# 0xWOLAND/halo2-prover

Hardware: AMD Instinct MI355X
Metric: MSM+NTT field-ops/s (higher is better)
Workload: dtype u32 limbs (256-bit modular)

## Files before the change

### halo2_prover_amd/csrc/h2_capi.hip

```cpp
#include "h2_internal.hpp"

#include <algorithm>
#include <cstdio>
#include <cstring>
#include <optional>

#include "h2_expr_program.hpp"
#include "h2_host.hpp"
#include "h2_ipa.hpp"
#include "h2_lookup.hpp"
#include "h2_ntt.hpp"
#include "h2_permutation.hpp"
#include "h2_poly.hpp"

using namespace h2;

namespace h2 {

Global g_h2;
std::recursive_mutex g_h2_mu;
TestKnobs g_knobs;
TestCounters g_counts;

int dev_fail(hipError_t e, const char* where) {
  char buf[256];
  snprintf(buf, sizeof buf, "%s: %s", where, hipGetErrorString(e));
  g_h2.last_error = buf;
  return H2_EDEVICE;
}

bool curve_ok(int c) { return c == H2_BN254 || c == H2_PALLAS || c == H2_VESTA; }

const CurveOps* ops_of(int curve) {
  switch (curve) {
    case H2_BN254: return curve_ops_bn254();
    case H2_PALLAS: return curve_ops_pallas();
    case H2_VESTA: return curve_ops_vesta();
  }
  return nullptr;
}

DevCtx* ctx_current() {
  if (!g_h2.ready || g_h2.ctx.empty()) return nullptr;
  if (g_h2.ctx.size() == 1) return &g_h2.ctx[0];
  int dev = -1;
  if (hipGetDevice(&dev) != hipSuccess) return nullptr;
  for (auto& c : g_h2.ctx)
    if (c.device == dev) return &c;
  return nullptr;
}
size_t ctx_index(const DevCtx* c) { return (size_t)(c - &g_h2.ctx[0]); }

int device_alloc(void** p, size_t bytes, const char* what) {
  hipError_t e = hipMalloc(p, bytes);
  if (e == hipSuccess) return H2_OK;
  (void)hipGetLastError();
  *p = nullptr;
  g_h2.last_error = std::string("hipMalloc(") + what + "): " + hipGetErrorString(e);
  return H2_ENOMEM;
}

ArenaLease::ArenaLease(Arena& arena, size_t want, hipStream_t stream) : a(arena), s(stream) { rc = acquire(want); }
int ArenaLease::acquire(size_t want) {
  clean_bytes = a.bytes < want ? 0 : a.clean_bytes;
  a.clean_bytes = 0;
  if (a.bytes < want) {
    g_counts.arena_growths++;
    if (a.p) {
      H2_TRY(hipDeviceSynchronize());
      (void)hipFree(a.p);
      a.p = nullptr;
      a.bytes = 0;
      a.used = false;
    }
    const size_t sz = want + (want >> 3);
    if (int st = device_alloc(&a.p, sz, "arena"); st != H2_OK) return st;
    a.bytes = sz;
  }
  if (!a.ev) H2_TRY(hipEventCreateWithFlags(&a.ev, hipEventDisableTiming));
  if (a.used && a.last != s) {
    g_counts.arena_waits++;
    H2_TRY(hipStreamWaitEvent(s, a.ev, 0));
  }
  return H2_OK;
}
int ArenaLease::release() {
  released = true;
  H2_TRY(hipEventRecord(a.ev, s));
  a.last = s;
  a.used = true;
  return H2_OK;
}
int ArenaLease::wait() {
  H2_TRY(hipStreamSynchronize(s));
  released = true;
  return H2_OK;
}
ArenaLease::~ArenaLease() noexcept {
  if (rc != H2_OK || released) return;
  if (hipEventRecord(a.ev, s) == hipSuccess) {
    a.last = s;
    a.used = true;
  } else {
    (void)hipGetLastError();
  }
}
static void arena_free(Arena& a) {
  if (a.p) (void)hipFree(a.p);
  if (a.ev) (void)hipEventDestroy(a.ev);
  a = Arena{};
}

static int register_device(DevCtx& src, int curve, const void* d_affine, size_t n, uint64_t* handle_out) {
  if (!curve_ok(curve) || !d_affine || !handle_out || n == 0) return H2_EINVAL;
  const CurveOps* ops = ops_of(curve);
  MsmGeom g = msm_geometry(n, ops->scalar_bits);
  if ((uint64_t)g.W * n >= (1ull << 31)) return H2_EINVAL;
  BasesEntry be{};
  be.curve = curve;
  be.n = n;
  be.geom = g;
  be.table_bytes = (size_t)g.W * n * 64;
  be.table.assign(g_h2.ctx.size(), nullptr);
  auto fail = [&](int rc) {
    for (size_t i = 0; i < be.table.size(); i++)
      if (be.table[i]) {
        DeviceGuard dg(g_h2.ctx[i].device);
        (void)hipFree(be.table[i]);
      }
    return rc;
  };
  for (size_t i = 0; i < g_h2.ctx.size(); i++) {
    DeviceGuard dg(g_h2.ctx[i].device);
    if (int rc = device_alloc(&be.table[i], be.table_bytes, "table"); rc != H2_OK) return fail(rc);
  }
  const size_t si = ctx_index(&src);
  {
    DeviceGuard dg(src.device);
    ArenaLease scan_ws(src.div_ws, sizeof(uint32_t), src.stream);
    if (scan_ws.rc != H2_OK) return fail(scan_ws.rc);
    uint32_t* d_bad = (uint32_t*)scan_ws.a.p;
    uint32_t bad = 0;
    ArenaLease table_ws(src.msm_ws.of(src.stream), be.table_bytes / 64 * MSM_TABLE_SCRATCH, src.stream);
    if (table_ws.rc != H2_OK) return fail(table_ws.rc);
    hipError_t e = hipMemsetAsync(d_bad, 0, 4, src.stream);
    if (e == hipSuccess) e = ops->table_build(d_affine, be.table[si], table_ws.a.p, (uint32_t)n, g, d_bad, src.stream);
    if (e == hipSuccess) e = hipMemcpyAsync(&bad, d_bad, 4, hipMemcpyDeviceToHost, src.stream);
    if (e == hipSuccess) e = hipStreamSynchronize(src.stream);
    if (e != hipSuccess) return fail(dev_fail(e, "msm_table_kernel"));
    (void)scan_ws.release();
    (void)table_ws.release();
    if (bad) {
      g_h2.last_error = "bases: " + std::to_string(bad) + " point(s) not on the curve";
      return fail(H2_EINVAL);
    }
    for (size_t i = 0; i < g_h2.ctx.size(); i++) {
      if (i == si) continue;
      e = hipMemcpyPeer(be.table[i], g_h2.ctx[i].device, be.table[si], src.device, be.table_bytes);
      if (e != hipSuccess) return fail(dev_fail(e, "hipMemcpyPeer(table)"));
    }
  }
  uint64_t h = g_h2.next_handle++;
  g_h2.bases[h] = be;
  *handle_out = h;
  return H2_OK;
}

int msm_common_checks(int curve, uint64_t handle, size_t first, size_t n, size_t m, const BasesEntry** be) {
  if (!g_h2.ready) return H2_ENOTINIT;
  if (!curve_ok(curve) || m == 0) return H2_EINVAL;
  auto it = g_h2.bases.find(handle);
  if (it == g_h2.bases.end()) return H2_EHANDLE;
  if (it->second.curve != curve) return H2_EINVAL;
  if (first > it->second.n || n > it->second.n - first) return H2_EINVAL;
  *be = &it->second;
  return H2_OK;
}

size_t msm_cols_per_launch(const MsmGeom& geom, size_t n) {
  const uint64_t per_col = (uint64_t)geom.W * n;
  const uint64_t by_entries = g_knobs.msm_max_entries / per_col;
  uint64_t by_keys = ((1ull << 31) - 1) / geom.B;
  if (geom.B > 4096) {
    const uint64_t by_bins = S2_MAX_H / msm_sort2_geom(n, geom).Hc;
    if (by_bins >= 1 && by_bins < by_keys) by_keys = by_bins;
  }
  return (size_t)(by_entries < by_keys ? by_entries : by_keys);
}

static int msm_guard_inspect(const MsmWorkspace& ws, char* ws_base, hipStream_t stream, size_t m, const char* what) {
  void* d_bad = nullptr;
  if (int rc = device_alloc(&d_bad, ws.n_regions * 4, "guard"); rc != H2_OK) return rc;
  DeviceBuffer owner(d_bad);
  std::vector<uint32_t> bad(ws.n_regions, 0);
  H2_TRY(hipMemsetAsync(d_bad, 0, ws.n_regions * 4, stream));
  if (g_knobs.msm_guard_poke)
    H2_TRY(hipMemsetAsync(ws_base + ws.regions[1].off + ws.regions[1].bytes, 0, 1, stream));
  hipLaunchKernelGGL(msm_guard_check_kernel, dim3(ws.n_regions), dim3(256), 0, stream, (const uint8_t*)ws_base, ws, (uint32_t*)d_bad);
  H2_TRY(hipMemcpyAsync(bad.data(), d_bad, ws.n_regions * 4, hipMemcpyDeviceToHost, stream));
  H2_TRY(hipStreamSynchronize(stream));
  g_counts.guard_launches++;
  for (uint32_t r = 0; r < ws.n_regions; r++)
    if (bad[r]) {
      if (!g_counts.guard_violations)
        g_counts.guard_first = std::string(ws.regions[r].name) + ": " + std::to_string(bad[r]) + " byte(s) behind the region, n=" +
                               std::to_string(ws.n) + " m=" + std::to_string(m) + what;
      g_counts.guard_violations++;
    }
  return H2_OK;
}

template <class Launch, class Finish>
static int msm_run_group(DevCtx& c, hipStream_t stream, const MsmGroupPlan& plan, const char* route, const char* label, size_t m,
                         const char* guard_what, Launch&& launch, Finish&& finish) {
  const MsmWorkspace& ws = plan.ws;
  ArenaLease lease(c.msm_ws.of(stream), ws.total, stream);
  if (lease.rc != H2_OK) return lease.rc;
  Arena& A = lease.a;
  if (const char* broken = plan.broken ? plan.broken : ws.total <= A.bytes ? nullptr : "ws.total <= arena_bytes") {
    g_h2.last_error = std::string(route) + " launch geometry: " + broken;
    return H2_EDEVICE;
  }
  const bool guard = g_knobs.msm_guard;
  if (guard) H2_TRY(hipMemsetAsync(A.p, MSM_GUARD_BYTE, ws.total, stream));
  const bool zeroed = !guard && lease.clean_bytes >= ws.zero_bytes && A.clean_off == ws.off_misc;
  if (int rc = launched(launch((char*)A.p, zeroed), label); rc != H2_OK) return rc;
  if (guard) {
    if (int rc = msm_guard_inspect(ws, (char*)A.p, stream, m, guard_what); rc != H2_OK) return rc;
  } else {
    A.clean_off = ws.off_misc;
    A.clean_bytes = ws.zero_bytes;
  }
  if (int rc = finish((char*)A.p); rc != H2_OK) return rc;
  return lease.release();
}

static std::pair<hipEvent_t, hipEvent_t> msm_prof_events(DevCtx& c, size_t n, size_t m) {
  if (!g_h2.profiling) return {nullptr, nullptr};
  if (c.prof_used == c.prof_events.size()) {
    hipEvent_t a, b;
    if (hipEventCreate(&a) == hipSuccess && hipEventCreate(&b) == hipSuccess) c.prof_events.push_back({a, b});
  }
  if (c.prof_used == c.prof_events.size()) return {nullptr, nullptr};
  c.prof_alg_bytes += (double)m * (double)n * 96.0 + (double)m * 96.0;
  return c.prof_events[c.prof_used++];
}

int msm_device_run(DevCtx& c, int curve, const BasesEntry& be, const void* d_scalars, size_t first_base, size_t n,
                   size_t col_stride, size_t m, void* d_out, bool affine_out, hipStream_t stream,
                   const BasesEntry* const* per_column) {
  if (msm_cols_per_launch(be.geom, n) == 0) return H2_EINVAL;
  const void* col_tables[MSM_MAX_MULTI];
  if (per_column) {
    if (m > MSM_MAX_MULTI) return H2_EINVAL;
    for (size_t j = 0; j < m; j++) {
      if (per_column[j]->n != be.n || per_column[j]->curve != be.curve) return H2_EINVAL;
      col_tables[j] = (const char*)per_column[j]->table[ctx_index(&c)] + first_base * 64;
    }
  }
  const size_t out_sz = affine_out ? 64 : 96;
  const CurveOps* ops = ops_of(curve);
  const char* table = (const char*)be.table[ctx_index(&c)] + first_base * 64;
  for (size_t j0 = 0; j0 < m;) {
    const MsmGroupPlan plan = msm_plan_group(be.geom, be.n, n, m - j0, col_stride, g_knobs.msm_guard, g_knobs.sort2_pack);
    const MsmWorkspace& ws = plan.ws;
    const size_t mm = plan.cols;
    if (per_column && mm < m) return H2_EINVAL;
    if (ws.E >= (1ull << 31) || ws.K >= (1ull << 31)) return H2_EINVAL;
    if (c.tail_wanted && !c.tail_event) H2_TRY(hipEventCreateWithFlags(&c.tail_event, hipEventDisableTiming));
    void* dst = (char*)d_out + j0 * out_sz;
    int rc = msm_run_group(
        c, stream, plan, "msm", "msm_launch", mm, ws.sort2 ? " two-level sort" : ws.staged ? " staged scatter" : " direct scatter",
        [&](char* ws_base, bool zeroed) {
          const auto [ev0, ev1] = msm_prof_events(c, n, mm);
          hipError_t e = ops->msm_launch(table, per_column ? col_tables : nullptr, (uint32_t)be.n,
                                         (const char*)d_scalars + j0 * col_stride * 32, n, col_stride, mm, be.geom, ws_base, ws, stream,
                                         ev0, ev1, (c.tail_wanted && !ev1) ? c.tail_event : nullptr, affine_out ? nullptr : dst, zeroed);
          c.tail_recorded = c.tail_wanted;
          c.tail_wait = ev1 ? ev1 : c.tail_event;
          return e;
        },
        [&](char* ws_base) {
          return affine_out ? launched(ops->to_affine(ws_base + ws.off_tree2, dst, (uint32_t)mm, stream), "msm finish kernel") : H2_OK;
        });
    if (rc != H2_OK) return rc;
    j0 += mm;
  }
  return H2_OK;
}

static int msm_points_run(DevCtx& c, int curve, const void* d_points, const void* d_scalars, size_t n, size_t col_stride,
                          size_t m, void* d_out, hipStream_t stream) {
  const CurveOps* ops = ops_of(curve);
  if (n < g_knobs.points_small_max) {
    const size_t blocks = (n + 15) / 16, work = MSM_SMALL_MAX * (blocks * (XYZZ29_WORDS * 4) + 4);
    for (size_t j0 = 0; j0 < m; j0 += MSM_SMALL_MAX) {
      const uint32_t count = (uint32_t)std::min<size_t>(MSM_SMALL_MAX, m - j0);
      ArenaLease lease(c.msm_ws.of(stream), work, stream);
      if (lease.rc != H2_OK) return lease.rc;
      const void* pts[MSM_SMALL_MAX];
      const void* sc[MSM_SMALL_MAX];
      uint32_t len[MSM_SMALL_MAX];
      for (uint32_t j = 0; j < count; j++) {
        pts[j] = d_points;
        sc[j] = (const char*)d_scalars + (j0 + j) * col_stride * 32;
        len[j] = (uint32_t)n;
      }
      if (int rc = launched(ops->msm_small(pts, sc, len, count, lease.a.p, (char*)d_out + j0 * 96, stream), "msm_small_kernel"); rc != H2_OK)
        return rc;
      if (int rc = lease.release(); rc != H2_OK) return rc;
    }
    return H2_OK;
  }
  const MsmGeom g = msm_points_geometry(n, ops->scalar_bits);
  for (size_t j0 = 0; j0 < m;) {
    const MsmGroupPlan plan = msm_points_plan_group(g, n, m - j0, col_stride, g_knobs.msm_guard);
    const size_t mm = plan.cols;
    if (mm == 0) return H2_EINVAL;
    int rc = msm_run_group(
        c, stream, plan, "msm points", "msm_points_launch", mm, " points front",
        [&](char* ws_base, bool zeroed) {
          return ops->msm_points_launch(d_points, (const char*)d_scalars + j0 * col_stride * 32, n, col_stride, mm, g, ws_base, plan.ws,
                                        stream, (char*)d_out + j0 * 96, zeroed);
        },
        [](char*) { return (int)H2_OK; });
    if (rc != H2_OK) return rc;
    j0 += mm;
  }
  return H2_OK;
}

static int get_twiddles(DevCtx& c, const CurveOps* ops, const uint64_t omega[4], uint32_t log_n, const uint64_t* scale,
                        const void** out) {
  for (auto& t : c.twiddles) {
    if (t.field == ops->scalar_field_id && t.log_n == log_n && memcmp(t.omega, omega, 32) == 0 && t.scaled == (scale != nullptr) &&
        (!scale || memcmp(t.scale, scale, 32) == 0)) {
      t.stamp = ++c.stamp;
      *out = t.tw;
      return H2_OK;
    }
  }
  if (c.twiddles.size() >= 16) {
    size_t victim = 0;
    for (size_t i = 1; i < c.twiddles.size(); i++)
      if (c.twiddles[i].stamp < c.twiddles[victim].stamp) victim = i;
    H2_TRY(hipDeviceSynchronize());
    (void)hipFree(c.twiddles[victim].tw);
    c.twiddles.erase(c.twiddles.begin() + victim);
  }
  TwiddleEntry te{};
  te.field = ops->scalar_field_id;
  te.log_n = log_n;
  memcpy(te.omega, omega, 32);
  te.scaled = scale != nullptr;
  if (scale) memcpy(te.scale, scale, 32);
  if (int rc = device_alloc(&te.tw, ops->ntt_table_bytes(log_n), "twiddles"); rc != H2_OK) return rc;
  DeviceBuffer owner(te.tw);
  hipError_t e = ops->ntt_twiddles(te.tw, omega, log_n, c.stream, scale);
  if (e == hipSuccess) e = hipStreamSynchronize(c.stream);
  if (e != hipSuccess) return dev_fail(e, "ntt_build_tables");
  (void)owner.release();
  te.stamp = ++c.stamp;
  c.twiddles.push_back(te);
  *out = te.tw;
  return H2_OK;
}

template <class Launch>
static int ntt_run(DevCtx& c, const CurveOps* ops, const uint64_t omega[4], uint32_t log_n, const uint64_t* table_scale, size_t m,
                   hipStream_t stream, const char* what, Launch&& launch) {
  const void* tw = nullptr;
  if (log_n > 0)
    if (int rc = get_twiddles(c, ops, omega, log_n, table_scale, &tw); rc != H2_OK) return rc;
  std::optional<ArenaLease> A;
  if (ntt_make_plan(log_n).npass > 1) {
    A.emplace(c.ntt_ws.of(stream), m * ((size_t)32 << log_n), stream);
    if (A->rc != H2_OK) return A->rc;
  }
  if (int rc = launched(launch(tw, A ? A->a.p : nullptr), what); rc != H2_OK) return rc;
  return A ? A->release() : H2_OK;
}

int ntt_enqueue(DevCtx& c, int curve, void* d_a, size_t m, const uint64_t omega[4], uint32_t log_n, hipStream_t stream,
                const uint64_t* scale) {
  const CurveOps* ops = ops_of(curve);
  if (!ops) return H2_EINVAL;
  return ntt_run(c, ops, omega, log_n, (scale && ops->ntt_scale_in_table(log_n)) ? scale : nullptr, m, stream, "ntt_launch",
                 [&](const void* tw, void* scratch) { return ops->ntt_launch(d_a, scratch, tw, log_n, m, stream, scale); });
}

int coeff_to_extended_enqueue(DevCtx& c, int curve, const void* d_coeff, size_t col_stride, uint32_t log_n, size_t m,
                              const uint64_t zeta[4], const uint64_t ext_omega[4], uint32_t ext_log_n, void* d_out,
                              hipStream_t stream) {
  const CurveOps* ops = ops_of(curve);
  if (!ops) return H2_EINVAL;
  return ntt_run(c, ops, ext_omega, ext_log_n, nullptr, m, stream, "ntt_extend_launch", [&](const void* tw, void* scratch) {
    return ops->ntt_extend_launch(d_coeff, col_stride, log_n, zeta, d_out, scratch, tw, ext_log_n, m, stream);
  });
}

int extended_to_coeff_enqueue(DevCtx& c, int curve, const void* d_ext, uint32_t ext_log_n, size_t m,
                              const uint64_t ext_omega_inv[4], const uint64_t scale[4], const uint64_t zeta_inv[4], const void* d_t,
                              size_t t_period, void* d_out, size_t out_len, size_t out_stride, hipStream_t stream) {
  const CurveOps* ops = ops_of(curve);
  if (!ops) return H2_EINVAL;
  if (m == 0 || out_len == 0) return H2_OK;
  return ntt_run(c, ops, ext_omega_inv, ext_log_n, ops->ntt_scale_in_table(ext_log_n) ? scale : nullptr, m, stream, "ntt_coeff_launch",
                 [&](const void* tw, void* scratch) {
                   return ops->ntt_coeff_launch(d_ext, d_t, t_period, scale, zeta_inv, d_out, out_len, out_stride, scratch, tw, ext_log_n,
                                                m, stream);
                 });
}

int poly_eval_enqueue(DevCtx& c, int curve, const void* const* d_polys, size_t n, const uint64_t* points, size_t q, void* d_out,
                      hipStream_t stream) {
  const CurveOps* ops = ops_of(curve);
  if (!ops || n == 0 || n > POLY_EVAL_MAX_N || q == 0) return H2_EINVAL;
  const size_t per_job = poly_eval_ws_bytes(1, n);
  const size_t group = std::min<size_t>({q, (size_t)65535, std::max<size_t>(1, POLY_EVAL_WS_CAP / per_job)});
  const size_t table_bytes = h2_align256(q * sizeof(PolyEvalJob));
  ArenaLease A(c.div_ws, table_bytes + poly_eval_ws_bytes(group, n), stream);
  if (A.rc != H2_OK) return A.rc;
  std::vector<PolyEvalJob> table(q);
  for (size_t t = 0; t < q; t++) {
    table[t].poly = d_polys[t];
    memcpy(table[t].point, points + 4 * t, 32);
  }
  H2_TRY(hipMemcpyAsync(A.a.p, table.data(), q * sizeof(PolyEvalJob), hipMemcpyHostToDevice, stream));
  const PolyEvalJob* d_jobs = (const PolyEvalJob*)A.a.p;
  void* ws = (char*)A.a.p + table_bytes;
  for (size_t t0 = 0; t0 < q; t0 += group) {
    const size_t cnt = std::min(group, q - t0);
    if (int rc = launched(ops->poly_eval(d_jobs + t0, (uint32_t)cnt, n, ws, (char*)d_out + 32 * t0, stream), "poly_eval kernels"); rc != H2_OK)
      return rc;
  }
  return A.release();
}

#define H2_BY_SCALAR_FIELD(curve, call)                          \
  ((curve) == H2_BN254    ? call<BN254_CURVE::Scalar>            \
   : (curve) == H2_PALLAS ? call<PALLAS_CURVE::Scalar>           \
                          : call<VESTA_CURVE::Scalar>)

template <class FP>
static void perm_fill_tables(const PermWorkspace& w, const void* const* d_values, const void* const* d_sigma, size_t n_cols, size_t m,
                             const uint64_t* beta, const uint64_t* gamma, const uint64_t omega[4], const uint64_t delta[4], char* out) {
  using H = HF<FP>;
  PermColumn* cols = (PermColumn*)(out + w.off_columns);
  PermChallenge* ch = (PermChallenge*)(out + w.off_challenges);
  const H d = H::from_mont_limbs(delta);
  for (size_t p = 0; p < m; p++) {
    H bd = H::from_mont_limbs(beta + 4 * p);
    memcpy(ch[p].beta, beta + 4 * p, 32);
    memcpy(ch[p].gamma, gamma + 4 * p, 32);
    for (size_t j = 0; j < n_cols; j++) {
      PermColumn& c = cols[p * n_cols + j];
      c.value = d_values[p * n_cols + j];
      c.sigma = d_sigma[j];
      uint64_t limbs[4];
      bd.mont_limbs(limbs);
      memcpy(c.beta_delta, limbs, 32);
      bd = bd * d;
    }
  }
  H pw = H::from_mont_limbs(omega);
  for (int r = 1; r < perm_run(); r <<= 1) pw = pw.sqr();
  for (int b = 0; b < PERM_POW_BITS; b++) {
    uint64_t limbs[4];
    pw.mont_limbs(limbs);
    memcpy(out + w.off_powers + 32 * (size_t)b, limbs, 32);
    pw = pw.sqr();
  }
}

int permutation_product_enqueue(DevCtx& c, int curve, const void* const* d_values, const void* const* d_sigma, size_t n_cols, size_t chunk_len,
                                size_t u, size_t m, const uint64_t* beta, const uint64_t* gamma, const uint64_t omega[4],
                                const uint64_t delta[4], void* d_z, size_t col_stride, hipStream_t stream) {
  const CurveOps* ops = ops_of(curve);
  if (!ops || n_cols == 0 || chunk_len == 0 || m == 0) return H2_EINVAL;
  const size_t S = (n_cols - 1) / chunk_len + 1;
  const size_t scan_group = std::min(m, PERM_SCAN_GROUP);
  const PermWorkspace ws = perm_workspace(u, n_cols, S, m, scan_group);
  if (const char* broken = perm_check(ws, u, n_cols, chunk_len, S, m, scan_group, col_stride, ws.total)) {
    g_h2.last_error = std::string("permutation launch geometry: ") + broken;
    return H2_EDEVICE;
  }
  ArenaLease A(c.div_ws, ws.total, stream);
  if (A.rc != H2_OK) return A.rc;
  if (const char* broken = perm_check(ws, u, n_cols, chunk_len, S, m, scan_group, col_stride, A.a.bytes)) {
    g_h2.last_error = std::string("permutation launch geometry: ") + broken;
    return H2_EDEVICE;
  }
  std::vector<char> tables(ws.off_scan);
  H2_BY_SCALAR_FIELD(curve, perm_fill_tables)(ws, d_values, d_sigma, n_cols, m, beta, gamma, omega, delta, tables.data());
  H2_TRY(hipMemcpyAsync(A.a.p, tables.data(), tables.size(), hipMemcpyHostToDevice, stream));
  for (size_t p0 = 0; p0 < m; p0 += PERM_RATIO_GROUP)
    if (int rc = launched(ops->perm_ratio(ws, (char*)A.a.p, p0, std::min(PERM_RATIO_GROUP, m - p0), u, n_cols, chunk_len, S, omega, d_z,
                                          col_stride, stream),
                          "perm_ratio_kernel");
        rc != H2_OK)
      return rc;
  for (size_t p0 = 0; u && p0 < m; p0 += scan_group)
    if (int rc = launched(ops->perm_scan(ws, (char*)A.a.p, p0, std::min(scan_group, m - p0), u, S, d_z, col_stride, stream),
                          "permutation scan kernels");
        rc != H2_OK)
      return rc;
  return A.release();
}

}

namespace {

struct Call {
  std::lock_guard<std::recursive_mutex> lk{g_h2_mu};
  DevCtx* c = nullptr;
  hipStream_t stream = nullptr;
  int rc = H2_OK;
  Call(void* stream_) {
    if (!g_h2.ready) { rc = H2_ENOTINIT; return; }
    c = ctx_current();
    if (!c) { rc = H2_EINVAL; g_h2.last_error = "no h2 context on the current HIP device"; return; }
    stream = stream_ ? (hipStream_t)stream_ : c->stream;
  }
};

int init_devices(int n, const int* ids) {
  if (g_h2.ready) {
    if ((size_t)n != g_h2.ctx.size()) return H2_EINVAL;
    for (int i = 0; i < n; i++)
      if (g_h2.ctx[i].device != ids[i]) return H2_EINVAL;
    return H2_OK;
  }
  int count = 0;
  hipError_t e = hipGetDeviceCount(&count);
  if (e != hipSuccess || count == 0) {
    (void)hipGetLastError();
    g_h2.last_error = "no HIP device available";
    return H2_EDEVICE;
  }
  for (int i = 0; i < n; i++)
    if (ids[i] < 0 || ids[i] >= count) return H2_EINVAL;
  int prev = 0;
  (void)hipGetDevice(&prev);
  g_h2.ctx.assign((size_t)n, DevCtx{});
  for (int i = 0; i < n; i++) {
    DevCtx& c = g_h2.ctx[i];
    c.device = ids[i];
    H2_TRY(hipSetDevice(ids[i]));
    H2_TRY(hipStreamCreateWithFlags(&c.stream, hipStreamDefault));
    for (int cv = 0; cv < 3; cv++) H2_TRY(ops_of(cv)->kernel_setup());
  }
  H2_TRY(hipSetDevice(n == 1 ? ids[0] : prev));
  g_h2.ready = true;
  return H2_OK;
}

template <class FP>
void jac_to_affine_host(const uint8_t* jac, size_t m, uint8_t* out) {
  using H = HF<FP>;
  std::vector<H> z(m), pre(m);
  H acc = H::one();
  for (size_t j = 0; j < m; j++) {
    z[j] = H::from_mont_limbs(jac + 96 * j + 64);
    pre[j] = acc;
    if (!z[j].is_zero()) acc *= z[j];
  }
  H inv = acc.inv();
  for (size_t j = m; j-- > 0;) {
    uint8_t* o = out + 64 * j;
    if (z[j].is_zero()) {
      memset(o, 0, 64);
      continue;
    }
    const H zi = inv * pre[j], zi2 = zi.sqr();
    inv *= z[j];
    const H x = H::from_mont_limbs(jac + 96 * j) * zi2, y = H::from_mont_limbs(jac + 96 * j + 32) * zi2 * zi;
    memcpy(o, x.v.v, 32);
    memcpy(o + 32, y.v.v, 32);
  }
}
void jac_to_affine_host(int curve, const uint8_t* jac, size_t m, uint8_t* out) {
  if (curve == H2_BN254) jac_to_affine_host<BN254_FQ>(jac, m, out);
  else if (curve == H2_PALLAS) jac_to_affine_host<PASTA_FP>(jac, m, out);
  else jac_to_affine_host<PASTA_FQ>(jac, m, out);
}

int msm_host(h2_curve_t curve, uint64_t handle, const uint64_t* const* cols, size_t n, size_t m, uint64_t* out,
                    bool affine_out) {
  const BasesEntry* be = nullptr;
  int rc = msm_common_checks((int)curve, handle, 0, n, m, &be);
  if (rc != H2_OK) return rc;
  if (!out || !cols) return H2_EINVAL;
  const size_t out_sz = affine_out ? 64 : 96;
  if (n == 0) {
    memset(out, 0, m * out_sz);
    return H2_OK;
  }
  for (size_t j = 0; j < m; j++)
    if (!cols[j]) return H2_EINVAL;
  const size_t G = g_h2.ctx.size();
  const size_t col_bytes = n * 32;
  if (m == 1 && G > 1 && n >= 4096 * G) {
    std::vector<uint64_t> partial(G * 12);
    std::vector<std::optional<ArenaLease>> stages(G);
    for (size_t g = 0; g < G; g++) {
      DevCtx& c = g_h2.ctx[g];
      DeviceGuard dg(c.device);
      const size_t lo = n * g / G, hi = n * (g + 1) / G, cnt = hi - lo;
      const size_t res_off = h2_align256(cnt * 32);
      if (int st = stages[g].emplace(c.stage, res_off + 96, c.stream).rc; st != H2_OK) return st;
      H2_TRY(hipMemcpyAsync(c.stage.p, (const char*)cols[0] + lo * 32, cnt * 32, hipMemcpyHostToDevice, c.stream));
      void* d_res = (char*)c.stage.p + res_off;
      rc = msm_device_run(c, (int)curve, *be, c.stage.p, lo, cnt, cnt, 1, d_res, false, c.stream);
      if (rc != H2_OK) return rc;
      H2_TRY(hipMemcpyAsync(&partial[12 * g], d_res, 96, hipMemcpyDeviceToHost, c.stream));
    }
    for (size_t g = 0; g < G; g++) {
      DeviceGuard dg(g_h2.ctx[g].device);
      if (int st = stages[g]->wait(); st != H2_OK) return st;
    }
    DevCtx& c = g_h2.ctx[0];
    DeviceGuard dg(c.device);
    const size_t res_off = h2_align256(G * 96);
    ArenaLease stage(c.stage, res_off + 96, c.stream);
    if (stage.rc != H2_OK) return stage.rc;
    H2_TRY(hipMemcpyAsync(c.stage.p, partial.data(), G * 96, hipMemcpyHostToDevice, c.stream));
    void* d_res = (char*)c.stage.p + res_off;
    if (int st = launched(ops_of((int)curve)->points_sum(c.stage.p, d_res, (uint32_t)G, 1, c.stream), "points_sum_kernel"); st != H2_OK)
      return st;
    if (affine_out) return H2_EINVAL;
    H2_TRY(hipMemcpyAsync(out, d_res, 96, hipMemcpyDeviceToHost, c.stream));
    return stage.wait();
  }
  std::vector<uint8_t> jac(affine_out ? m * 96 : 0);
  uint8_t* dst = affine_out ? jac.data() : (uint8_t*)out;
  std::vector<std::optional<ArenaLease>> stages(G);
  for (size_t g = 0; g < G && g < m; g++) {
    DevCtx& c = g_h2.ctx[g];
    DeviceGuard dg(c.device);
    const size_t mine = (m - g + G - 1) / G;
    const size_t res_off = h2_align256(mine * col_bytes);
    if (int st = stages[g].emplace(c.stage, res_off + mine * 96, c.stream).rc; st != H2_OK) return st;
    for (size_t i = 0; i < mine; i++)
      H2_TRY(hipMemcpyAsync((char*)c.stage.p + i * col_bytes, cols[g + i * G], col_bytes, hipMemcpyHostToDevice,
                            c.stream));
    void* d_res = (char*)c.stage.p + res_off;
    rc = msm_device_run(c, (int)curve, *be, c.stage.p, 0, n, n, mine, d_res, false, c.stream);
    if (rc != H2_OK) return rc;
    if (G == 1) {
      H2_TRY(hipMemcpyAsync(dst, d_res, mine * 96, hipMemcpyDeviceToHost, c.stream));
    } else {
      for (size_t i = 0; i < mine; i++)
        H2_TRY(hipMemcpyAsync(dst + (g + i * G) * 96, (char*)d_res + i * 96, 96, hipMemcpyDeviceToHost, c.stream));
    }
  }
  for (size_t g = 0; g < G && g < m; g++) {
    DeviceGuard dg(g_h2.ctx[g].device);
    if (int st = stages[g]->wait(); st != H2_OK) return st;
  }
  if (affine_out) jac_to_affine_host((int)curve, jac.data(), m, (uint8_t*)out);
  return H2_OK;
}

constexpr size_t EXPR_TABLE_CAP = (size_t)256 << 20;
constexpr size_t EXPR_MAX_COUNT = (size_t)1 << 20;
constexpr size_t EXPR_MAX_INSTANCES = (size_t)1 << 30;

template <class FP>
bool mont_canonical(const uint64_t* v) {
  for (int i = 3; i >= 0; i--) {
    const uint64_t pw = (uint64_t)FP::P(2 * i) | ((uint64_t)FP::P(2 * i + 1) << 32);
    if (v[i] != pw) return v[i] < pw;
  }
  return false;
}
template <class FP>
void expr_working_form(const uint64_t* api, uint64_t* out) {
  HF<FP> c = HF<FP>::from_mont_limbs(api);
// ... 387 lines not shown
  }
  return ntt_enqueue(*k.c, (int)curve, d_a, m, omega, log_n, k.stream, scale);
}

int h2_coeff_to_extended_device(h2_curve_t curve, const void* d_coeff, size_t col_stride, uint32_t log_n, size_t m,
                                const uint64_t zeta[4], const uint64_t ext_omega[4], uint32_t ext_log_n, void* d_out,
                                void* stream_) {
  Call k(stream_);
  if (k.rc != H2_OK) return k.rc;
  if (!curve_ok((int)curve) || !zeta || !ext_omega || ext_log_n > 30 || ext_log_n < log_n) return H2_EINVAL;
  const size_t n = (size_t)1 << log_n, en = (size_t)1 << ext_log_n;
  if (col_stride < n) return H2_EINVAL;
  if (m == 0) return H2_OK;
  if (!d_coeff || !d_out || m > 65535) return H2_EINVAL;
  const uintptr_t s0 = (uintptr_t)d_coeff, s1 = s0 + ((m - 1) * col_stride + n) * 32;
  const uintptr_t o0 = (uintptr_t)d_out, o1 = o0 + m * en * 32;
  if (s0 < o1 && o0 < s1) return H2_EINVAL;
  if (ext_log_n == 0) {
    H2_TRY(hipMemcpy2DAsync(d_out, 32, d_coeff, col_stride * 32, 32, m, hipMemcpyDeviceToDevice, k.stream));
    return H2_OK;
  }
  return coeff_to_extended_enqueue(*k.c, (int)curve, d_coeff, col_stride, log_n, m, zeta, ext_omega, ext_log_n, d_out, k.stream);
}

int h2_extended_to_coeff_device(h2_curve_t curve, const void* d_ext, uint32_t ext_log_n, size_t m, const uint64_t ext_omega_inv[4],
                                const uint64_t scale[4], const uint64_t zeta_inv[4], const void* d_t, size_t t_period, void* d_out,
                                size_t out_len, size_t out_stride, void* stream_) {
  Call k(stream_);
  if (k.rc != H2_OK) return k.rc;
  if (!curve_ok((int)curve) || ext_log_n > 30 || m > 65535) return H2_EINVAL;
  const size_t en = (size_t)1 << ext_log_n;
  if (out_len > en || out_stride < out_len || out_stride > ((size_t)1 << 40)) return H2_EINVAL;
  if (d_t && (t_period == 0 || (t_period & (t_period - 1)) || t_period > en)) return H2_EINVAL;
  if ((((uintptr_t)d_ext | (uintptr_t)d_out | (uintptr_t)d_t) & 15) != 0) return H2_EINVAL;
  if (m == 0 || out_len == 0) return H2_OK;
  if (!d_ext || !d_out || !ext_omega_inv || !scale || !zeta_inv) return H2_EINVAL;
  const uintptr_t s0 = (uintptr_t)d_ext, s1 = s0 + m * en * 32;
  const uintptr_t o0 = (uintptr_t)d_out, o1 = o0 + ((m - 1) * out_stride + out_len) * 32;
  if (s0 < o1 && o0 < s1) return H2_EINVAL;
  return extended_to_coeff_enqueue(*k.c, (int)curve, d_ext, ext_log_n, m, ext_omega_inv, scale, zeta_inv, d_t, t_period, d_out,
                                   out_len, out_stride, k.stream);
}

int h2_poly_scale_device(h2_curve_t curve, void* d_a, size_t n, size_t m, const uint64_t c[4], void* stream_) {
  Call k(stream_);
  if (k.rc != H2_OK) return k.rc;
  if (!curve_ok((int)curve) || !d_a || !c) return H2_EINVAL;
  if (n * m == 0) return H2_OK;
  return launched(ops_of((int)curve)->poly_scale(d_a, n * m, c, k.stream), "poly_scale_kernel");
}

int h2_poly_coset_device(h2_curve_t curve, void* d_a, size_t n, size_t m, const uint64_t g[4], void* stream_) {
  Call k(stream_);
  if (k.rc != H2_OK) return k.rc;
  if (!curve_ok((int)curve) || !d_a || !g) return H2_EINVAL;
  if (n * m == 0) return H2_OK;
  return launched(ops_of((int)curve)->poly_powers(d_a, n, m, g, k.stream), "poly_powers_kernel");
}

int h2_poly_mul_periodic_device(h2_curve_t curve, void* d_a, size_t n, size_t m, const void* d_t, size_t period,
                                void* stream_) {
  Call k(stream_);
  if (k.rc != H2_OK) return k.rc;
  if (!curve_ok((int)curve) || !d_a || !d_t || period == 0 || (period & (period - 1))) return H2_EINVAL;
  if (n * m == 0) return H2_OK;
  return launched(ops_of((int)curve)->poly_mul_periodic(d_a, n * m, d_t, period, k.stream), "poly_mul_periodic_kernel");
}

int h2_poly_inverse_device(h2_curve_t curve, void* d_a, size_t n, void* stream_) {
  Call k(stream_);
  if (k.rc != H2_OK) return k.rc;
  if (!curve_ok((int)curve) || !d_a) return H2_EINVAL;
  if (n == 0) return H2_OK;
  return launched(ops_of((int)curve)->poly_inverse(d_a, n, k.stream), "poly_inverse_kernel");
}

int h2_poly_divide_linear_device(h2_curve_t curve, const void* d_a, size_t n, const uint64_t z[4], void* d_q,
                                 void* stream_) {
  Call k(stream_);
  if (k.rc != H2_OK) return k.rc;
  if (!curve_ok((int)curve) || !d_a || !d_q || !z || d_a == d_q) return H2_EINVAL;
  if (n == 0) return H2_OK;
  ArenaLease A(k.c->div_ws, SCAN_WS_BYTES, k.stream);
  if (A.rc != H2_OK) return A.rc;
  if (int rc = launched(ops_of((int)curve)->poly_scan(0, &d_a, &d_q, z, 1, n, A.a.p, k.stream), "poly_scan kernels"); rc != H2_OK) return rc;
  return A.release();
}

int h2_poly_prefix_product_device(h2_curve_t curve, const void* d_a, size_t n, void* d_out, void* stream_) {
  Call k(stream_);
  if (k.rc != H2_OK) return k.rc;
  if (!curve_ok((int)curve) || !d_a || !d_out) return H2_EINVAL;
  if (n == 0) return H2_OK;
  ArenaLease A(k.c->div_ws, SCAN_WS_BYTES, k.stream);
  if (A.rc != H2_OK) return A.rc;
  if (int rc = launched(ops_of((int)curve)->poly_scan(1, &d_a, &d_out, nullptr, 1, n, A.a.p, k.stream), "poly_scan kernels"); rc != H2_OK) return rc;
  return A.release();
}

int h2_poly_eval_tile(void) { return POLY_EVAL_TILE; }

int h2_poly_eval_device(h2_curve_t curve, const void* const* d_polys, size_t n, const uint64_t* points, size_t q, void* d_out,
                        void* stream_) {
  Call k(stream_);
  if (k.rc != H2_OK) return k.rc;
  if (!curve_ok((int)curve) || n > POLY_EVAL_MAX_N) return H2_EINVAL;
  if (q == 0) return H2_OK;
  if (!d_polys || !points || !d_out) return H2_EINVAL;
  if (n == 0) {
    H2_TRY(hipMemsetAsync(d_out, 0, q * 32, k.stream));
    return H2_OK;
  }
  for (size_t t = 0; t < q; t++)
    if (!d_polys[t] || ((uintptr_t)d_polys[t] & 15)) return H2_EINVAL;
  return poly_eval_enqueue(*k.c, (int)curve, d_polys, n, points, q, d_out, k.stream);
}

int h2_poly_eval(h2_curve_t curve, const uint64_t* coeffs, size_t n, const uint64_t point[4], uint64_t out[4]) {
  Call k(nullptr);
  if (k.rc != H2_OK) return k.rc;
  if (!curve_ok((int)curve) || n > POLY_EVAL_MAX_N || !point || !out || (n > 0 && !coeffs)) return H2_EINVAL;
  if (n == 0) {
    memset(out, 0, 32);
    return H2_OK;
  }
  DevCtx& c = *k.c;
  const size_t off_res = h2_align256(n * 32);
  ArenaLease stage(c.stage, off_res + 32, c.stream);
  if (stage.rc != H2_OK) return stage.rc;
  char* base = (char*)c.stage.p;
  H2_TRY(hipMemcpyAsync(base, coeffs, n * 32, hipMemcpyHostToDevice, c.stream));
  const void* poly = base;
  if (int rc = poly_eval_enqueue(c, (int)curve, &poly, n, point, 1, base + off_res, c.stream); rc != H2_OK) return rc;
  H2_TRY(hipMemcpyAsync(out, base + off_res, 32, hipMemcpyDeviceToHost, c.stream));
  return stage.wait();
}

int h2_poly_lincomb_max_rounds(void) { return POLY_LINCOMB_MAX_ROUNDS; }

static_assert(sizeof(h2_lincomb_term_t) == sizeof(LincombTerm) && sizeof(h2_lincomb_job_t) == sizeof(LincombJob) &&
                  offsetof(h2_lincomb_term_t, coeff) == offsetof(LincombTerm, coeff) &&
                  offsetof(h2_lincomb_job_t, first_term) == offsetof(LincombJob, first_term),
              "the kernels read the C ABI's tables as they are");

static bool lincomb_overlaps(const h2_lincomb_job_t* jobs, size_t n_jobs, const h2_lincomb_term_t* terms, size_t n) {
  const uintptr_t len = (uintptr_t)n * 32;
  std::vector<std::pair<uintptr_t, size_t>> src, out;
  for (size_t j = 0; j < n_jobs; j++) {
    out.emplace_back((uintptr_t)jobs[j].d_out, j);
    for (uint32_t t = 0; t < jobs[j].n_terms; t++) src.emplace_back((uintptr_t)terms[jobs[j].first_term + t].d_poly, j);
  }
  std::sort(out.begin(), out.end());
  for (size_t a = 1; a < out.size(); a++)
    if (out[a].first - out[a - 1].first < len) return true;
  std::sort(src.begin(), src.end());
  src.erase(std::unique(src.begin(), src.end()), src.end());
  for (const auto& o : out) {
    auto it = std::lower_bound(src.begin(), src.end(), std::make_pair(o.first >= len ? o.first - len + 1 : (uintptr_t)0, (size_t)0));
    for (; it != src.end() && it->first < o.first + len; ++it) {
      if (it->second != o.second) return true;
      if (jobs[o.second].n_points > 0 || it->first != o.first) return true;
    }
  }
  return false;
}

int h2_poly_lincomb_device(h2_curve_t curve, const h2_lincomb_job_t* jobs, size_t n_jobs, const h2_lincomb_term_t* terms,
                           size_t n_terms, const uint64_t* low, size_t n_low, const uint64_t* points, size_t n_points, size_t n,
                           void* stream_) {
  Call k(stream_);
  if (k.rc != H2_OK) return k.rc;
  if (!curve_ok((int)curve) || n > POLY_LINCOMB_MAX_N) return H2_EINVAL;
  if (n_jobs == 0) return H2_OK;
  if (!jobs || n_jobs > ((size_t)1 << 31) || n_terms > ((size_t)1 << 31) || n_low > ((size_t)1 << 31)) return H2_EINVAL;
  size_t dividing = 0;
  for (size_t j = 0; j < n_jobs; j++) {
    const h2_lincomb_job_t& J = jobs[j];
    if ((uint64_t)J.first_term + J.n_terms > n_terms || (uint64_t)J.first_low + J.n_low > n_low ||
        (uint64_t)J.first_point + J.n_points > n_points)
      return H2_EINVAL;
    if (J.n_low > n || J.n_points > (uint32_t)POLY_LINCOMB_MAX_ROUNDS) return H2_EINVAL;
    if ((J.n_terms && !terms) || (J.n_low && !low) || (J.n_points && !points)) return H2_EINVAL;
    if (!J.d_out || ((uintptr_t)J.d_out & 15)) return H2_EINVAL;
    for (uint32_t t = 0; t < J.n_terms; t++) {
      const void* p = terms[J.first_term + t].d_poly;
      if (!p || ((uintptr_t)p & 15)) return H2_EINVAL;
    }
    dividing += J.n_points > 0;
  }
  if (n == 0) return H2_OK;
  if (lincomb_overlaps(jobs, n_jobs, terms, n)) return H2_EINVAL;

  const size_t col_bytes = h2_align256(n * 32);
  const size_t cols_cap = std::min(std::max<size_t>(1, POLY_LINCOMB_WS_CAP / col_bytes), std::max<size_t>(1, dividing));
  const size_t off_terms = h2_align256(n_jobs * sizeof(LincombJob));
  const size_t off_low = off_terms + h2_align256(n_terms * sizeof(LincombTerm));
  const size_t off_cols = off_low + h2_align256(n_low * 32);
  const size_t off_scan = off_cols + (dividing ? cols_cap * col_bytes : 0);
  ArenaLease A(k.c->div_ws, off_scan + (dividing ? SCAN_MAX_JOBS * SCAN_WS_BYTES : 0), k.stream);
  if (A.rc != H2_OK) return A.rc;
  char* base = (char*)A.a.p;

  std::vector<char> host(off_cols, 0);
  LincombJob* hj = (LincombJob*)host.data();
  std::vector<void*> scratch_of(n_jobs, nullptr);
  std::vector<size_t> group_end;
  for (size_t j = 0, g0 = 0, used = 0; j < n_jobs; j++) {
    const bool div = jobs[j].n_points > 0;
    if (j - g0 == 65535 || (div && used == cols_cap)) {
      group_end.push_back(j);
      g0 = j;
      used = 0;
    }
    memcpy(&hj[j], &jobs[j], sizeof(LincombJob));
    if (div) {
      scratch_of[j] = base + off_cols + used++ * col_bytes;
      if (jobs[j].n_points & 1) hj[j].out = scratch_of[j];
    }
  }
  group_end.push_back(n_jobs);
  if (n_terms) memcpy(host.data() + off_terms, terms, n_terms * sizeof(LincombTerm));
  if (n_low) memcpy(host.data() + off_low, low, n_low * 32);
  H2_TRY(hipMemcpyAsync(base, host.data(), off_cols, hipMemcpyHostToDevice, k.stream));

  const CurveOps* ops = ops_of((int)curve);
  for (size_t g = 0, j0 = 0; g < group_end.size(); j0 = group_end[g++]) {
    const size_t j1 = group_end[g];
    if (int rc = launched(ops->poly_lincomb((const LincombJob*)base + j0, (uint32_t)(j1 - j0), (const LincombTerm*)(base + off_terms),
                                            base + off_low, n, k.stream),
                          "poly_lincomb_kernel");
        rc != H2_OK)
      return rc;
    for (uint32_t r = 0; r < (uint32_t)POLY_LINCOMB_MAX_ROUNDS; r++) {
      const void* src[SCAN_MAX_JOBS];
      void* dst[SCAN_MAX_JOBS];
      uint64_t z[4 * SCAN_MAX_JOBS];
      uint32_t cnt = 0;
      bool any = false;
      auto flush = [&]() -> int {
        if (cnt == 0) return H2_OK;
        const int rc = launched(ops->poly_scan(0, src, dst, z, cnt, n, base + off_scan, k.stream), "poly_scan kernels");
        cnt = 0;
        return rc;
      };
      for (size_t j = j0; j < j1; j++) {
        const uint32_t P = jobs[j].n_points;
        if (P <= r) continue;
        any = true;
        src[cnt] = ((P - r) & 1) ? scratch_of[j] : jobs[j].d_out;
        dst[cnt] = ((P - r - 1) & 1) ? scratch_of[j] : jobs[j].d_out;
        memcpy(z + 4 * cnt, points + 4 * ((size_t)jobs[j].first_point + r), 32);
        if (++cnt == SCAN_MAX_JOBS)
          if (int rc = flush(); rc != H2_OK) return rc;
      }
      if (int rc = flush(); rc != H2_OK) return rc;
      if (!any) break;
    }
  }
  return A.release();
}

int h2_lookup_tile(void) { return (int)LOOKUP_TILE; }

static std::pair<uintptr_t, uintptr_t> lookup_range(const void* p, size_t rows, size_t stride, size_t m, size_t elem = 32) {
  const uintptr_t lo = (uintptr_t)p;
  if (rows == 0) return {lo, lo};
  return {lo, lo + ((m - 1) * stride + rows) * elem};
}
static bool lookup_overlap(const std::pair<uintptr_t, uintptr_t>& a, const std::pair<uintptr_t, uintptr_t>& b) {
  return a.first < b.second && b.first < a.second && a.first != a.second && b.first != b.second;
}

int h2_lookup_permute_device(h2_curve_t curve, const void* d_input, const void* d_table, size_t usable_rows, size_t col_stride,
                             size_t m, void* d_permuted_input, void* d_permuted_table, void* d_status, void* stream_) {
  Call k(stream_);
  if (k.rc != H2_OK) return k.rc;
  const size_t u = usable_rows;
  if (!curve_ok((int)curve) || u > LOOKUP_MAX_ROWS || col_stride < u || (col_stride && m > LOOKUP_MAX_CELLS / col_stride)) return H2_EINVAL;
  if ((((uintptr_t)d_input | (uintptr_t)d_table | (uintptr_t)d_permuted_input | (uintptr_t)d_permuted_table) & 15) || ((uintptr_t)d_status & 3))
    return H2_EINVAL;
  if (m == 0) return H2_OK;
  if (!d_status || (u > 0 && (!d_input || !d_table || !d_permuted_input || !d_permuted_table))) return H2_EINVAL;
  const auto in = lookup_range(d_input, u, col_stride, m), tab = lookup_range(d_table, u, col_stride, m);
  const auto pin = lookup_range(d_permuted_input, u, col_stride, m), ptab = lookup_range(d_permuted_table, u, col_stride, m);
  const auto st = lookup_range(d_status, 1, 1, m, 4);
  for (const auto* out : {&pin, &ptab, &st})
    if (lookup_overlap(*out, in) || lookup_overlap(*out, tab)) return H2_EINVAL;
  if (lookup_overlap(pin, ptab) || lookup_overlap(pin, st) || lookup_overlap(ptab, st)) return H2_EINVAL;
  const size_t group = u ? lookup_group(u, m) : m;
  for (size_t j0 = 0; u && j0 < m; j0 += group) {
    const size_t mm = std::min(group, m - j0);
    const LookupWorkspace ws = lookup_workspace(u, mm);
    if (const char* broken = lookup_check(ws, u, mm, col_stride, ws.total)) {
      g_h2.last_error = std::string("lookup launch geometry: ") + broken;
      return H2_EDEVICE;
    }
  }
  H2_TRY(hipMemsetAsync(d_status, 0, 4 * m, k.stream));
  if (u == 0) return H2_OK;
  const CurveOps* ops = ops_of((int)curve);
  for (size_t j0 = 0; j0 < m; j0 += group) {
    const size_t mm = std::min(group, m - j0);
    const LookupWorkspace ws = lookup_workspace(u, mm);
    ArenaLease A(k.c->msm_ws.of(k.stream), ws.total, k.stream);
    if (A.rc != H2_OK) return A.rc;
    if (const char* broken = lookup_check(ws, u, mm, col_stride, A.a.bytes)) {
      g_h2.last_error = std::string("lookup launch geometry: ") + broken;
      return H2_EDEVICE;
    }
    const size_t skip = j0 * col_stride * 32;
    if (int rc = launched(ops->lookup_permute((const char*)d_input + skip, (const char*)d_table + skip, col_stride, ws, (char*)A.a.p,
                                              (char*)d_permuted_input + skip, (char*)d_permuted_table + skip, (uint32_t*)d_status + j0,
                                              k.stream),
                          "lookup permute kernels");
        rc != H2_OK)
      return rc;
    if (int rc = A.release(); rc != H2_OK) return rc;
  }
  return H2_OK;
}

int h2_lookup_product_device(h2_curve_t curve, const void* d_input, const void* d_table, const void* d_permuted_input,
                             const void* d_permuted_table, size_t usable_rows, size_t col_stride, size_t m, const uint64_t beta[4],
                             const uint64_t gamma[4], void* d_z, void* stream_) {
  Call k(stream_);
  if (k.rc != H2_OK) return k.rc;
  const size_t u = usable_rows;
  if (!curve_ok((int)curve) || u > LOOKUP_MAX_ROWS || col_stride < u + 1 || m > LOOKUP_MAX_CELLS / col_stride) return H2_EINVAL;
  if (((uintptr_t)d_input | (uintptr_t)d_table | (uintptr_t)d_permuted_input | (uintptr_t)d_permuted_table | (uintptr_t)d_z) & 15) return H2_EINVAL;
  if (m == 0) return H2_OK;
  if (!d_z || !beta || !gamma || (u > 0 && (!d_input || !d_table || !d_permuted_input || !d_permuted_table))) return H2_EINVAL;
  const auto z = lookup_range(d_z, u + 1, col_stride, m);
  for (const void* src : {d_input, d_table, d_permuted_input, d_permuted_table})
    if (lookup_overlap(z, lookup_range(src, u, col_stride, m))) return H2_EINVAL;
  const CurveOps* ops = ops_of((int)curve);
  for (size_t j0 = 0; j0 < m; j0 += 65535) {
    const size_t skip = j0 * col_stride * 32;
    if (int rc = launched(ops->lookup_ratio((const char*)d_input + skip, (const char*)d_table + skip, (const char*)d_permuted_input + skip,
                                            (const char*)d_permuted_table + skip, u, col_stride, std::min<size_t>(65535, m - j0), beta,
                                            gamma, (char*)d_z + skip, k.stream),
                          "lookup_ratio_kernel");
        rc != H2_OK)
      return rc;
  }
  ArenaLease A(k.c->div_ws, SCAN_MAX_JOBS * SCAN_WS_BYTES, k.stream);
  if (A.rc != H2_OK) return A.rc;
  for (size_t j0 = 0; j0 < m; j0 += SCAN_MAX_JOBS) {
    const uint32_t cnt = (uint32_t)std::min<size_t>(SCAN_MAX_JOBS, m - j0);
    const void* src[SCAN_MAX_JOBS];
    void* dst[SCAN_MAX_JOBS];
    for (uint32_t j = 0; j < cnt; j++) src[j] = dst[j] = (char*)d_z + (j0 + j) * col_stride * 32;
    if (int rc = launched(ops->poly_scan(1, src, dst, nullptr, cnt, u + 1, A.a.p, k.stream), "poly_scan kernels"); rc != H2_OK) return rc;
  }
  return A.release();
}

int h2_permutation_tile(void) { return (int)perm_tile(); }

int h2_permutation_product_device(h2_curve_t curve, const void* const* d_values, const void* const* d_sigma, size_t n_cols, size_t chunk_len,
                                  size_t usable_rows, size_t m, const uint64_t* beta, const uint64_t* gamma, const uint64_t omega[4],
                                  const uint64_t delta[4], void* d_z, size_t col_stride, void* stream_) {
  Call k(stream_);
  if (k.rc != H2_OK) return k.rc;
  const size_t u = usable_rows;
  if (!curve_ok((int)curve) || (chunk_len == 0 && n_cols > 0) || u > PERM_MAX_ROWS || col_stride < u + 1) return H2_EINVAL;
  const size_t S = n_cols ? (n_cols - 1) / chunk_len + 1 : 0;
  if (S && m && (m > PERM_MAX_CELLS / S || m * S > PERM_MAX_CELLS / col_stride)) return H2_EINVAL;
  if (m == 0 || n_cols == 0) return H2_OK;
  if (!d_values || !d_sigma || !beta || !gamma || !omega || !delta || !d_z || ((uintptr_t)d_z & 15)) return H2_EINVAL;
  if (n_cols > ((size_t)1 << 31) || m > ((size_t)1 << 32) / n_cols) {
    g_h2.last_error = "permutation launch geometry: m n_cols <= 2^32";
    return H2_EDEVICE;
  }
  if (u > 0) {
    const auto z = lookup_range(d_z, u + 1, col_stride, m * S);
    for (size_t t = 0; t < m * n_cols + n_cols; t++) {
      const void* src = t < m * n_cols ? d_values[t] : d_sigma[t - m * n_cols];
      if (!src || ((uintptr_t)src & 15) || lookup_overlap(z, lookup_range(src, u, u, 1))) return H2_EINVAL;
    }
  }
  return permutation_product_enqueue(*k.c, (int)curve, d_values, d_sigma, n_cols, chunk_len, u, m, beta, gamma, omega, delta, d_z, col_stride,
                                     k.stream);
}

int h2_expr_compile(h2_curve_t curve, const h2_expr_node_t* nodes, size_t n_nodes, const uint64_t* consts, size_t n_consts,
                    uint32_t n_cols, uint32_t n_vars, uint64_t* handle_out) {
  std::lock_guard<std::recursive_mutex> lk(g_h2_mu);
  auto refuse = [](const char* rule) {
    g_h2.last_error = std::string("expr: ") + rule;
    return (int)H2_EINVAL;
  };
  if (!curve_ok((int)curve)) return refuse("unknown curve");
  if (!handle_out || !nodes || (n_consts && !consts)) return refuse("null pointer");
  if (n_nodes == 0 || n_nodes > EXPR_MAX_COUNT) return refuse("n_nodes must be 1 .. 2^20");
  if (n_consts > EXPR_MAX_COUNT || n_vars > EXPR_MAX_COUNT) return refuse("n_consts and n_vars may be at most 2^20");
  if (n_cols > (1u << 22)) return refuse("n_cols may be at most 2^22");
  ExprEntry e{};
  e.curve = (int)curve;
  try {
    H2_BY_SCALAR_FIELD((int)curve, expr_compile_t)(nodes, n_nodes, consts, n_consts, n_cols, n_vars, e);
  } catch (const product::Fail& f) {
    g_h2.last_error = f.what;
    return f.status;
  } catch (const std::exception& x) {
    g_h2.last_error = x.what();
    return H2_ENOMEM;
  }
  e.info.curve = (uint32_t)curve;
  const uint64_t h = g_h2.next_handle++;
  g_h2.exprs[h] = std::move(e);
  *handle_out = h;
  return H2_OK;
}

int h2_expr_release(uint64_t handle) {
  std::lock_guard<std::recursive_mutex> lk(g_h2_mu);
  auto it = g_h2.exprs.find(handle);
  if (it == g_h2.exprs.end()) return H2_EHANDLE;
  for (size_t i = 0; i < it->second.d_code.size() && i < g_h2.ctx.size(); i++) {
    if (!it->second.d_code[i]) continue;
    DeviceGuard dg(g_h2.ctx[i].device);
    (void)hipDeviceSynchronize();
    (void)hipFree(it->second.d_code[i]);
  }
  g_h2.exprs.erase(it);
  return H2_OK;
}

int h2_expr_info(uint64_t handle, h2_expr_info_t* out) {
  std::lock_guard<std::recursive_mutex> lk(g_h2_mu);
  if (!out) return H2_EINVAL;
  auto it = g_h2.exprs.find(handle);
  if (it == g_h2.exprs.end()) return H2_EHANDLE;
  *out = it->second.info;
  return H2_OK;
}

int h2_expr_dump(uint64_t handle, uint8_t* out, size_t cap, size_t* out_len) {
  std::lock_guard<std::recursive_mutex> lk(g_h2_mu);
  auto it = g_h2.exprs.find(handle);
  if (it == g_h2.exprs.end()) return H2_EHANDLE;
  const std::vector<uint8_t>& d = it->second.dump;
  if (out_len) *out_len = d.size();
  if (!out || cap < d.size()) return H2_EINVAL;
  memcpy(out, d.data(), d.size());
  return H2_OK;
}

int h2_expr_eval_device(uint64_t handle, const void* const* d_cols, const uint32_t* log_len, const uint64_t* vars, size_t m,
                        uint32_t log_rows, uint32_t rot_step, void* d_out, size_t out_stride, void* stream_) {
  Call k(stream_);
  if (k.rc != H2_OK) return k.rc;
  auto it = g_h2.exprs.find(handle);
  if (it == g_h2.exprs.end()) return H2_EHANDLE;
  ExprEntry& e = it->second;
  const size_t n_cols = e.info.n_cols, n_vars = e.info.n_vars, nconsts = e.table.size() / 4;
  if (log_rows > 28 || m > EXPR_MAX_INSTANCES) return H2_EINVAL;
  const size_t rows = (size_t)1 << log_rows;
  if (out_stride < rows || (m && out_stride > ((size_t)1 << 57) / m)) return H2_EINVAL;
  if (m == 0) return H2_OK;
  if (!d_out || ((uintptr_t)d_out & 15) || (n_cols && (!d_cols || !log_len)) || (n_vars && !vars)) return H2_EINVAL;
  for (size_t c = 0; c < n_cols; c++)
    if (log_len[c] > log_rows) return H2_EINVAL;
  const uintptr_t o0 = (uintptr_t)d_out, window = out_stride * 32, written = rows * 32, o1 = o0 + (m - 1) * window + written;
  for (size_t p = 0; p < m; p++)
    for (size_t c = 0; c < n_cols; c++) {
      const uintptr_t s0 = (uintptr_t)d_cols[p * n_cols + c], s1 = s0 + ((uintptr_t)32 << log_len[c]);
      if (!s0 || (s0 & 15)) return H2_EINVAL;
      if (s0 < o1 && o0 < s1) {
        const uintptr_t q = s0 > o0 ? (s0 - o0) / window : 0, w0 = o0 + q * window;
        if (s0 < w0 + written || (q + 1 < m && s1 > w0 + window)) return H2_EINVAL;
      }
    }
  for (size_t t = 0; t < m * n_vars; t++)
    if (!H2_BY_SCALAR_FIELD(e.curve, mont_canonical)(vars + 4 * t)) return H2_EINVAL;
  DevCtx& c = *k.c;
  const size_t ci = ctx_index(&c);
  const size_t group = std::min<size_t>({m, (size_t)65535, std::max<size_t>(1, EXPR_TABLE_CAP / (nconsts * 32))});
  std::vector<uint32_t> masks;
  std::vector<uint64_t> tables;
  try {
    masks.resize(n_cols);
    tables.resize(group * nconsts * 4);
    if (e.d_code.size() != g_h2.ctx.size()) e.d_code.assign(g_h2.ctx.size(), nullptr);
  } catch (const std::bad_alloc&) {
    g_h2.last_error = "expr: no host memory for the instances' constant tables";
    return H2_ENOMEM;
  }
  if (!e.d_code[ci]) {
    void* p = nullptr;
    if (int rc = device_alloc(&p, e.code.size() * 4, "expr code"); rc != H2_OK) return rc;
    DeviceBuffer owner(p);
    H2_TRY(hipMemcpyAsync(p, e.code.data(), e.code.size() * 4, hipMemcpyHostToDevice, c.stream));
    H2_TRY(hipStreamSynchronize(c.stream));
    e.d_code[ci] = owner.release();
  }
  const size_t mask_bytes = h2_align256(n_cols * 4 + 4), ptr_bytes = h2_align256(group * n_cols * sizeof(void*) + 8);
  ArenaLease A(c.div_ws, mask_bytes + ptr_bytes + group * nconsts * 32, k.stream);
  if (A.rc != H2_OK) return A.rc;
  uint32_t* d_masks = (uint32_t*)A.a.p;
  const void** d_ptrs = (const void**)((char*)A.a.p + mask_bytes);
  void* d_tables = (char*)A.a.p + mask_bytes + ptr_bytes;
  for (size_t j = 0; j < n_cols; j++) masks[j] = (1u << log_len[j]) - 1;
  if (n_cols) H2_TRY(hipMemcpyAsync(d_masks, masks.data(), n_cols * 4, hipMemcpyHostToDevice, k.stream));
  const CurveOps* ops = ops_of(e.curve);
  for (size_t p0 = 0; p0 < m; p0 += group) {
    const size_t cnt = std::min(group, m - p0);
    H2_BY_SCALAR_FIELD(e.curve, expr_fill_tables)(e, vars, p0, cnt, tables.data());
    if (n_cols) H2_TRY(hipMemcpyAsync(d_ptrs, d_cols + p0 * n_cols, cnt * n_cols * sizeof(void*), hipMemcpyHostToDevice, k.stream));
    H2_TRY(hipMemcpyAsync(d_tables, tables.data(), cnt * nconsts * 32, hipMemcpyHostToDevice, k.stream));
    if (int rc = launched(ops->expr_launch(e.d_code[ci], e.info.instructions, d_ptrs, (uint32_t)n_cols, d_masks, d_tables, (uint32_t)nconsts,
                                           (char*)d_out + p0 * out_stride * 32, out_stride, rot_step, (uint32_t)rows, (uint32_t)cnt,
                                           e.info.lds_bytes, k.stream),
                          "expr_kernel");
        rc != H2_OK)
      return rc;
  }
  return A.release();
}

int h2_chacha20_scalars_device(h2_curve_t curve, const uint8_t seed[32], uint64_t first_block, size_t n, void* d_out,
                               void* stream_) {
  Call k(stream_);
  if (k.rc != H2_OK) return k.rc;
  if (!curve_ok((int)curve) || !seed || !d_out) return H2_EINVAL;
  if (n == 0) return H2_OK;
  uint32_t key[8];
  for (int i = 0; i < 8; i++)
    key[i] = (uint32_t)seed[4 * i] | ((uint32_t)seed[4 * i + 1] << 8) | ((uint32_t)seed[4 * i + 2] << 16) |
             ((uint32_t)seed[4 * i + 3] << 24);
  return launched(ops_of((int)curve)->chacha20_scalars(d_out, n, first_block, key, k.stream), "chacha20_scalars_kernel");
}

static_assert(H2_IPA_MAX_K == IPA_MAX_K, "the header states the kernels' maximum");
static bool ipa_dev_ptr(const void* p) { return p && !((uintptr_t)p & 15); }

int h2_ipa_state_bytes(uint32_t k, size_t* out) {
  if (k == 0 || k > IPA_MAX_K || !out) return H2_EINVAL;
  *out = IpaLayout(k).total * 32;
  return H2_OK;
}

int h2_ipa_begin_device(h2_curve_t curve, uint32_t k_, const void* d_p, const uint64_t x3[4], void* d_state, void* stream_) {
  Call k(stream_);
  if (k.rc != H2_OK) return k.rc;
  if (!curve_ok((int)curve) || k_ == 0 || k_ > IPA_MAX_K || !ipa_dev_ptr(d_p) || !ipa_dev_ptr(d_state) || !x3) return H2_EINVAL;
  return launched(ops_of((int)curve)->ipa_begin(d_p, x3, k_, d_state, k.stream), "ipa_begin_kernel");
}

int h2_ipa_round_device(h2_curve_t curve, uint64_t bases, uint32_t k_, uint32_t j, void* d_state, const uint64_t* u_prev,
                        const uint64_t* u_prev_inv, const uint64_t z[4], const uint64_t l_blind[4], const uint64_t r_blind[4],
                        void* d_out_affine, void* stream_) {
  Call k(stream_);
  if (k.rc != H2_OK) return k.rc;
  if (!curve_ok((int)curve) || k_ == 0 || k_ > IPA_MAX_K || j >= k_) return H2_EINVAL;
  if (!ipa_dev_ptr(d_state) || !ipa_dev_ptr(d_out_affine) || !z || !l_blind || !r_blind) return H2_EINVAL;
  if (j == 0 ? (u_prev || u_prev_inv) : (!u_prev || !u_prev_inv)) return H2_EINVAL;
  const IpaLayout L(k_);
  const BasesEntry* be = nullptr;
  if (int rc = msm_common_checks((int)curve, bases, 0, L.col_stride, 2, &be); rc != H2_OK) return rc;
  if (be->n != L.col_stride) return H2_EINVAL;
  if (int rc = launched(ops_of((int)curve)->ipa_round(k_, j, d_state, u_prev, u_prev_inv, z, l_blind, r_blind, k.stream),
                        "ipa_round_kernel");
      rc != H2_OK)
    return rc;
  return msm_device_run(*k.c, (int)curve, *be, (const char*)d_state + L.col * 32, 0, L.col_stride, L.col_stride, 2, d_out_affine,
                        true, k.stream);
}

int h2_ipa_final_device(h2_curve_t curve, uint32_t k_, void* d_state, const uint64_t u_last[4], const uint64_t u_last_inv[4],
                        void* d_out, void* d_s_out, void* stream_) {
  Call k(stream_);
  if (k.rc != H2_OK) return k.rc;
  if (!curve_ok((int)curve) || k_ == 0 || k_ > IPA_MAX_K || !ipa_dev_ptr(d_state) || !ipa_dev_ptr(d_out) || !u_last || !u_last_inv)
    return H2_EINVAL;
  if (d_s_out && ((uintptr_t)d_s_out & 15)) return H2_EINVAL;
  return launched(ops_of((int)curve)->ipa_final(k_, d_state, u_last, u_last_inv, d_out, d_s_out, k.stream), "ipa_final_kernel");
}

int h2_ipa_challenge_products_device(h2_curve_t curve, const uint64_t* u, uint32_t k_, const uint64_t init[4], void* d_out,
                                     void* stream_) {
  Call k(stream_);
  if (k.rc != H2_OK) return k.rc;
  if (!curve_ok((int)curve) || k_ == 0 || k_ > IPA_MAX_K || !u || !init || !ipa_dev_ptr(d_out)) return H2_EINVAL;
  return launched(ops_of((int)curve)->ipa_s_products(u, k_, init, d_out, k.stream), "ipa_s_kernel");
}

int h2_poly_pointwise_device(h2_curve_t curve, int op, void* d_a, const void* d_b, size_t n, void* stream_) {
  Call k(stream_);
  if (k.rc != H2_OK) return k.rc;
  if (!curve_ok((int)curve) || !d_a || !d_b || op < 0 || op > 2) return H2_EINVAL;
  if (n == 0) return H2_OK;
  return launched(ops_of((int)curve)->poly_pointwise(d_a, d_b, n, op, k.stream), "poly_pointwise_kernel");
}

int h2_ntt_batch(h2_curve_t curve, uint64_t* const* cols, size_t m, const uint64_t omega[4], uint32_t log_n) {
  std::lock_guard<std::recursive_mutex> lk(g_h2_mu);
  if (!g_h2.ready) return H2_ENOTINIT;
  if (!curve_ok((int)curve) || !cols || !omega || m == 0 || log_n > 30) return H2_EINVAL;
  for (size_t j = 0; j < m; j++)
    if (!cols[j]) return H2_EINVAL;
  if (log_n == 0) return H2_OK;
  const size_t col_bytes = (size_t)32 << log_n;
  const size_t G = g_h2.ctx.size();
  std::vector<std::optional<ArenaLease>> stages(G);
  for (size_t g = 0; g < G && g < m; g++) {
    DevCtx& c = g_h2.ctx[g];
    DeviceGuard dg(c.device);
    const size_t mine = (m - g + G - 1) / G;
    if (int st = stages[g].emplace(c.stage, mine * col_bytes, c.stream).rc; st != H2_OK) return st;
    for (size_t i = 0; i < mine; i++)
      H2_TRY(hipMemcpyAsync((char*)c.stage.p + i * col_bytes, cols[g + i * G], col_bytes, hipMemcpyHostToDevice,
                            c.stream));
    int rc = ntt_enqueue(c, (int)curve, c.stage.p, mine, omega, log_n, c.stream);
    if (rc != H2_OK) return rc;
    for (size_t i = 0; i < mine; i++)
      H2_TRY(hipMemcpyAsync(cols[g + i * G], (char*)c.stage.p + i * col_bytes, col_bytes, hipMemcpyDeviceToHost,
                            c.stream));
  }
  for (size_t g = 0; g < G && g < m; g++) {
    DeviceGuard dg(g_h2.ctx[g].device);
    if (int st = stages[g]->wait(); st != H2_OK) return st;
  }
  return H2_OK;
}

int h2_fft_group_device(h2_curve_t curve, void* d_points_jac, const uint64_t omega[4], uint32_t log_n, void* stream_) {
  Call k(stream_);
  if (k.rc != H2_OK) return k.rc;
  if (!curve_ok((int)curve) || !d_points_jac || !omega || log_n > 26) return H2_EINVAL;
  if (log_n == 0) return H2_OK;
  const CurveOps* ops = ops_of((int)curve);
  ArenaLease A(k.c->msm_ws.of(k.stream), ops->group_fft_scratch(log_n), k.stream);
  if (A.rc != H2_OK) return A.rc;
  if (int rc = launched(ops->group_fft(d_points_jac, d_points_jac, A.a.p, omega, log_n, g_knobs.gfft_lanes, k.stream), "group fft kernels"); rc != H2_OK) return rc;
  return A.release();
}

int h2_fft_group(h2_curve_t curve, uint64_t* points_jac, const uint64_t omega[4], uint32_t log_n) {
  std::lock_guard<std::recursive_mutex> lk(g_h2_mu);
  if (!g_h2.ready) return H2_ENOTINIT;
  if (!curve_ok((int)curve) || !points_jac || !omega || log_n > 26) return H2_EINVAL;
  if (log_n == 0) return H2_OK;
  DevCtx& c = g_h2.ctx[0];
  DeviceGuard dg(c.device);
  const size_t bytes = ((size_t)96) << log_n;
  ArenaLease stage(c.stage, bytes, c.stream);
  if (stage.rc != H2_OK) return stage.rc;
  H2_TRY(hipMemcpyAsync(c.stage.p, points_jac, bytes, hipMemcpyHostToDevice, c.stream));
  int rc = h2_fft_group_device(curve, c.stage.p, omega, log_n, c.stream);
  if (rc != H2_OK) return rc;
  H2_TRY(hipMemcpyAsync(points_jac, c.stage.p, bytes, hipMemcpyDeviceToHost, c.stream));
  return stage.wait();
}

int h2_g_to_lagrange_device(h2_curve_t curve, const void* d_g_affine, uint32_t log_n, const uint64_t omega_inv[4],
                            const uint64_t scale[4], void* d_out_affine, void* stream_) {
  Call k(stream_);
  if (k.rc != H2_OK) return k.rc;
  if (!curve_ok((int)curve) || !d_g_affine || !d_out_affine || !omega_inv || !scale || log_n > 26) return H2_EINVAL;
  const uintptr_t in = (uintptr_t)d_g_affine, out = (uintptr_t)d_out_affine, bytes = (uintptr_t)64 << log_n;
  if ((in & 15) || (out & 15)) return H2_EINVAL;
  if (in != out && in < out + bytes && out < in + bytes) return H2_EINVAL;
  const CurveOps* ops = ops_of((int)curve);
  ArenaLease A(k.c->msm_ws.of(k.stream), ops->group_fft_scratch(log_n), k.stream);
  if (A.rc != H2_OK) return A.rc;
  if (int rc = launched(ops->g_to_lagrange(d_g_affine, d_out_affine, A.a.p, omega_inv, scale, log_n, g_knobs.gfft_lanes, k.stream),
                        "g_to_lagrange kernels");
      rc != H2_OK)
    return rc;
  return A.release();
}

int h2_g_to_lagrange(h2_curve_t curve, const uint64_t* g_affine, uint32_t log_n, const uint64_t omega_inv[4],
                     const uint64_t scale[4], uint64_t* out_affine) {
  std::lock_guard<std::recursive_mutex> lk(g_h2_mu);
  if (!g_h2.ready) return H2_ENOTINIT;
  if (!curve_ok((int)curve) || !g_affine || !out_affine || !omega_inv || !scale || log_n > 26) return H2_EINVAL;
  DevCtx& c = g_h2.ctx[0];
  DeviceGuard dg(c.device);
  const size_t bytes = ((size_t)64) << log_n;
  ArenaLease stage(c.stage, bytes, c.stream);
  if (stage.rc != H2_OK) return stage.rc;
  H2_TRY(hipMemcpyAsync(c.stage.p, g_affine, bytes, hipMemcpyHostToDevice, c.stream));
  int rc = h2_g_to_lagrange_device(curve, c.stage.p, log_n, omega_inv, scale, c.stage.p, c.stream);
  if (rc != H2_OK) return rc;
  H2_TRY(hipMemcpyAsync(out_affine, c.stage.p, bytes, hipMemcpyDeviceToHost, c.stream));
  return stage.wait();
}

int h2_ntt(h2_curve_t curve, uint64_t* a, const uint64_t omega[4], uint32_t log_n) {
  uint64_t* cols[1] = {a};
  return h2_ntt_batch(curve, cols, 1, omega, log_n);
}

}
```

### halo2_prover_amd/csrc/h2_curve_impl.hip

```cpp
#include "h2_curve_ops.hpp"
#include "h2_msm.hpp"
#include "h2_decompress.hpp"
#include "h2_ntt.hpp"
#include "h2_ntt29.hpp"
#include "h2_tune.hpp"
#include "h2_poly.hpp"
#include "h2_group_fft.hpp"
#include "h2_lookup.hpp"
#include "h2_permutation.hpp"
#include "h2_expr_kernel.hpp"
#include "h2_ipa.hpp"

#include <cstring>

#ifndef H2_CURVE_ID
#error "compile with -DH2_CURVE_ID=0 (bn254), 1 (pallas) or 2 (vesta)"
#endif

namespace h2 {
namespace {

#if H2_CURVE_ID == 0
using CV = BN254_CURVE;
#elif H2_CURVE_ID == 1
using CV = PALLAS_CURVE;
#else
using CV = VESTA_CURVE;
#endif
using FS = typename CV::Scalar;
using FB = typename CV::Base;

hipError_t kernel_setup() {
  hipError_t e = msm_kernel_setup<CV>();
  if (e != hipSuccess) return e;
  if ((e = msm_points_kernel_setup<CV>()) != hipSuccess) return e;
  return ntt29_kernel_setup<FS>();
}
hipError_t table_build(const void* d_bases, void* d_table, void* d_scratch, uint32_t n, const MsmGeom& g, uint32_t* d_bad, hipStream_t s) {
  hipLaunchKernelGGL(msm_table_kernel<CV>, dim3((n + 255) / 256), dim3(256), 0, s, (const U128*)d_bases,
                     (U128*)d_table, (uint32_t*)d_scratch, n, g, d_bad);
  return hipGetLastError();
}
hipError_t msm_launch_(const void* d_table, const void* const* per_column, uint32_t n_bases, const void* d_scalars, size_t n, size_t col_stride, size_t m,
                       const MsmGeom& g, char* ws_base, const MsmWorkspace& ws, hipStream_t s, hipEvent_t ev_start,
                       hipEvent_t ev_stop, hipEvent_t ev_tail, void* d_out_jac, bool zeroed) {
  return msm_launch<CV>((const U128*)d_table, (const U128* const*)per_column, n_bases, (const U128*)d_scalars, n, col_stride, m, g, ws_base, ws, s, ev_start,
                        ev_stop, ev_tail, (U128*)d_out_jac, zeroed);
}
hipError_t msm_points_launch_(const void* d_points, const void* d_scalars, size_t n, size_t col_stride, size_t m, const MsmGeom& g,
                              char* ws_base, const MsmWorkspace& ws, hipStream_t s, void* d_out_jac, bool zeroed) {
  return msm_points_launch<CV>((const U128*)d_points, (const U128*)d_scalars, n, col_stride, m, g, ws_base, ws, s, (U128*)d_out_jac, zeroed);
}
hipError_t srs_powers(void* d_out_affine, const uint64_t s_mont[4], uint32_t n, hipStream_t s) {
  Fe<FS> sv;
  memcpy(sv.v, s_mont, 32);
  hipLaunchKernelGGL(srs_powers_kernel<CV>, dim3((n + 255) / 256), dim3(256), 0, s, (U128*)d_out_affine, sv, n);
  return hipGetLastError();
}
hipError_t fixed_base_mul(void* d_out_affine, const void* d_scalars, uint32_t n, hipStream_t s) {
  hipLaunchKernelGGL(fixed_base_mul_kernel<CV>, dim3((n + 255) / 256), dim3(256), 0, s, (U128*)d_out_affine,
                     (const U128*)d_scalars, n);
  return hipGetLastError();
}
hipError_t to_affine(const void* d_xyzz, void* d_out, uint32_t m, hipStream_t s) {
  hipLaunchKernelGGL(msm_to_affine_kernel<CV>, dim3((m + 63) / 64), dim3(64), 0, s, (const uint32_t*)d_xyzz,
                     (U128*)d_out, m);
  return hipGetLastError();
}
hipError_t msm_small(const void* const* d_points, const void* const* d_scalars, const uint32_t* m, uint32_t count, void* d_work,
                     void* d_out_jac, hipStream_t s) {
  if (count == 0 || count > MSM_SMALL_MAX) return hipErrorInvalidValue;
  MsmSmallBatch J{};
  uint32_t mmax = 0;
  for (uint32_t j = 0; j < count; j++) {
    J.points[j] = (const U128*)d_points[j];
    J.scalars[j] = (const U128*)d_scalars[j];
    J.m[j] = m[j];
    mmax = std::max(mmax, m[j]);
  }
  const uint32_t blocks = (mmax + 15) / 16;
  if (blocks == 0) return hipErrorInvalidValue;
  uint32_t* part = (uint32_t*)d_work;
  uint32_t* counter = part + (size_t)count * blocks * XYZZ29_WORDS;
  hipError_t e = hipMemsetAsync(counter, 0, 4 * count, s);
  if (e != hipSuccess) return e;
  hipLaunchKernelGGL(msm_small_kernel<CV>, dim3(blocks, count), dim3(64), 0, s, J, part, counter, (U128*)d_out_jac);
  return hipGetLastError();
}
hipError_t points_sum(const void* d_in_jac, void* d_out_jac, uint32_t groups, uint32_t count, hipStream_t s) {
  hipLaunchKernelGGL(points_sum_kernel<CV>, dim3(count), dim3(64), 0, s, (const U128*)d_in_jac,
                     (U128*)d_out_jac, groups, count);
  return hipGetLastError();
}
#if H2_CURVE_ID == 0
hipError_t points_decompress(const void* d_compressed, void* d_out_affine, void* d_status, uint32_t n, hipStream_t s) {
  hipLaunchKernelGGL(points_decompress_kernel<CV>, dim3((n + 63) / 64), dim3(64), 0, s, (const uint32_t*)d_compressed,
                     (U128*)d_out_affine, (uint8_t*)d_status, n);
  return hipGetLastError();
}
int selftest_decompress(const uint8_t in[32], uint64_t out_affine[8]) {
  uint32_t w[8];
  for (int i = 0; i < 8; i++)
    w[i] = (uint32_t)in[4 * i] | ((uint32_t)in[4 * i + 1] << 8) | ((uint32_t)in[4 * i + 2] << 16) | ((uint32_t)in[4 * i + 3] << 24);
  Fe<FB> x, y;
  const uint8_t st = g1_decompress<CV>(w, x, y);
  memcpy(out_affine, x.v, 32);
  memcpy(out_affine + 4, y.v, 32);
  return st;
}
#else
constexpr auto points_decompress = nullptr;
constexpr auto selftest_decompress = nullptr;
#endif
size_t ntt_table_bytes(uint32_t log_n) { return ntt29_tables(log_n).total; }
bool ntt_scale_in_table(uint32_t log_n) { return ntt29_scale_in_table(log_n); }
hipError_t ntt_twiddles(void* d_tw, const uint64_t omega[4], uint32_t log_n, hipStream_t s, const uint64_t* scale) {
  Fe<FS> w, sc;
  memcpy(w.v, omega, 32);
  if (scale) memcpy(sc.v, scale, 32);
  return ntt29_build_tables<FS>(d_tw, w, log_n, s, scale ? &sc : nullptr);
}
hipError_t ntt_launch_(void* d_data, void* d_scratch, const void* d_tw, uint32_t log_n, size_t m, hipStream_t s,
                       const uint64_t* scale) {
  Fe<FS> sc;
  if (scale) memcpy(sc.v, scale, 32);
  return ntt29_launch<FS>((U128*)d_data, (U128*)d_scratch, d_tw, log_n, m, s, scale ? &sc : nullptr);
}
hipError_t ntt_extend_launch_(const void* d_src, size_t src_stride, uint32_t log_src, const uint64_t zeta[4], void* d_out,
                              void* d_scratch, const void* d_tw, uint32_t log_n, size_t m, hipStream_t s) {
  Fe<FS> z;
  memcpy(z.v, zeta, 32);
  return ntt29_extend_launch<FS>((const U128*)d_src, src_stride, log_src, z, (U128*)d_out, (U128*)d_scratch, d_tw, log_n, m, s);
}
hipError_t ntt_coeff_launch_(const void* d_src, const void* d_t, size_t t_period, const uint64_t scale[4], const uint64_t zeta_inv[4],
                             void* d_out, size_t out_len, size_t out_stride, void* d_scratch, const void* d_tw, uint32_t log_n,
                             size_t m, hipStream_t s) {
  Fe<FS> sc, zi;
  memcpy(sc.v, scale, 32);
  memcpy(zi.v, zeta_inv, 32);
  return ntt29_coeff_launch<FS>((const U128*)d_src, (const U128*)d_t, t_period, sc, zi, (U128*)d_out, out_len, out_stride,
                                (U128*)d_scratch, d_tw, log_n, m, s);
}
size_t group_fft_scratch(uint32_t log_n) { return gfft_scratch_bytes(log_n); }
hipError_t group_fft(const void* d_in_jac, void* d_out_jac, void* d_scratch, const uint64_t omega[4], uint32_t log_n, int lanes,
                     hipStream_t s) {
  Fe<FS> w;
  memcpy(w.v, omega, 32);
  return gfft_launch<CV>((const U128*)d_in_jac, (U128*)d_out_jac, d_scratch, w, log_n, s, lanes);
}
hipError_t g_to_lagrange(const void* d_in_affine, void* d_out_affine, void* d_scratch, const uint64_t omega[4],
                         const uint64_t scale[4], uint32_t log_n, int lanes, hipStream_t s) {
  Fe<FS> w, c;
  memcpy(w.v, omega, 32);
  memcpy(c.v, scale, 32);
  return gfft_to_lagrange_launch<CV>((const U128*)d_in_affine, (U128*)d_out_affine, d_scratch, w, c, log_n, s, lanes);
}
void selftest_glv_split(const uint64_t k_canonical[4], uint32_t out[10]) {
  Fe<FS> k;
  memcpy(k.v, k_canonical, 32);
  const GlvScalar r = glv_split<FS>(k);
  memcpy(out, r.k1, 4 * GLV_WORDS);
  memcpy(out + GLV_WORDS, r.k2, 4 * GLV_WORDS);
}
void selftest_glv_constants(uint64_t lambda[4], uint64_t beta[4]) {
  uint32_t l[8], b[8];
  for (int i = 0; i < 8; i++) {
    l[i] = Glv<FS>::LAMBDA(i);
    b[i] = Glv<FS>::BETA(i);
  }
  memcpy(lambda, l, 32);
  memcpy(beta, b, 32);
}
hipError_t poly_scale(void* d_a, size_t total, const uint64_t c[4], hipStream_t s) {
  Fe<FS> cv;
  memcpy(cv.v, c, 32);
  hipLaunchKernelGGL(poly_scale_kernel<FS>, dim3(poly_grid(total)), dim3(256), 0, s, (U128*)d_a, total, cv);
  return hipGetLastError();
}
hipError_t poly_powers(void* d_a, size_t n, size_t m, const uint64_t g[4], hipStream_t s) {
  Fe<FS> gv;
  memcpy(gv.v, g, 32);
  const size_t threads = (n + POLY_RUN - 1) / POLY_RUN;
  hipLaunchKernelGGL(poly_powers_kernel<FS>, dim3((unsigned)((threads + 255) / 256), (unsigned)m), dim3(256), 0, s,
                     (U128*)d_a, n, gv);
  return hipGetLastError();
}
hipError_t poly_mul_periodic(void* d_a, size_t total, const void* d_t, size_t period, hipStream_t s) {
  hipLaunchKernelGGL(poly_mul_periodic_kernel<FS>, dim3(poly_grid(total)), dim3(256), 0, s, (U128*)d_a, total,
                     (const U128*)d_t, period - 1);
  return hipGetLastError();
}
hipError_t poly_inverse(void* d_a, size_t total, hipStream_t s) {
  hipLaunchKernelGGL(poly_inverse_kernel<FS>, dim3(poly_grid(total)), dim3(256), 0, s, (U128*)d_a, total);
  return hipGetLastError();
}
hipError_t poly_scan(int mode, const void* const* d_a, void* const* d_out, const uint64_t* z, uint32_t jobs, size_t n,
                     void* d_ws, hipStream_t s) {
  if (jobs == 0 || jobs > SCAN_MAX_JOBS || n == 0) return hipErrorInvalidValue;
  uint32_t L = (uint32_t)((n + SCAN_CHUNKS - 1) / SCAN_CHUNKS);
  if (L < 16) L = 16;
  const uint32_t C = (uint32_t)((n + L - 1) / L);
  ScanBatch<FS> B{};
  for (uint32_t j = 0; j < jobs; j++) {
    B.a[j] = (const U128*)d_a[j];
    B.out[j] = (U128*)d_out[j];
    if (mode == 0) {
      memcpy(B.z[j].v, z + 4 * j, 32);
      B.w[j] = fe_pow_u64(B.z[j], (uint64_t)L);
    }
  }
  U128* H = (U128*)d_ws;
  U128* G = H + 2 * (size_t)jobs * SCAN_CHUNKS;
  hipLaunchKernelGGL(poly_scan_chunk_kernel<FS>, dim3((C + 63) / 64, jobs), dim3(64), 0, s, B, mode, n, L, C, H);
  hipLaunchKernelGGL(poly_scan_block_kernel<FS>, dim3(jobs), dim3(SCAN_BLOCK_THREADS), 0, s, B, mode, C, H, G);
  hipLaunchKernelGGL(poly_scan_apply_kernel<FS>, dim3((C + 63) / 64, jobs), dim3(64), 0, s, B, mode, n, L, C, G);
  return hipGetLastError();
}
hipError_t poly_eval(const PolyEvalJob* d_jobs, uint32_t jobs, size_t n, void* d_ws, void* d_out, hipStream_t s) {
  if (jobs == 0 || jobs > 65535 || n == 0 || n > POLY_EVAL_MAX_N) return hipErrorInvalidValue;
  const uint32_t tiles = (uint32_t)poly_eval_tiles(n);
  U128* partial = (U128*)d_ws;
  int32_t* powers = (int32_t*)((char*)d_ws + (size_t)jobs * tiles * 32);
  hipLaunchKernelGGL(poly_eval_powers_kernel<FS>, dim3((jobs + 63) / 64), dim3(64), 0, s, d_jobs, jobs, powers);
  hipLaunchKernelGGL(poly_eval_tile_kernel<FS>, dim3(tiles, jobs), dim3(POLY_EVAL_THREADS), 0, s, d_jobs, n,
                     (const int32_t*)powers, partial, tiles);
  hipLaunchKernelGGL(poly_eval_fold_kernel<FS>, dim3((jobs + 63) / 64), dim3(64), 0, s, jobs, (const int32_t*)powers,
                     (const U128*)partial, tiles, (U128*)d_out);
  return hipGetLastError();
}
hipError_t poly_lincomb(const LincombJob* d_jobs, uint32_t jobs, const LincombTerm* d_terms, const void* d_low, size_t n,
                        hipStream_t s) {
  if (jobs == 0 || jobs > 65535 || n == 0 || n > POLY_LINCOMB_MAX_N) return hipErrorInvalidValue;
  hipLaunchKernelGGL(poly_lincomb_kernel<FS>, dim3((unsigned)((n + POLY_LINCOMB_THREADS - 1) / POLY_LINCOMB_THREADS), jobs),
                     dim3(POLY_LINCOMB_THREADS), 0, s, d_jobs, d_terms, (const U128*)d_low, n);
  return hipGetLastError();
}
hipError_t lookup_permute(const void* d_input, const void* d_table, size_t col_stride, const LookupWorkspace& ws, char* ws_base,
                          void* d_permuted_input, void* d_permuted_table, uint32_t* d_status, hipStream_t s) {
  return lookup_permute_launch<FS>(d_input, d_table, col_stride, ws, ws_base, d_permuted_input, d_permuted_table, d_status, s);
}
hipError_t lookup_ratio(const void* d_input, const void* d_table, const void* d_permuted_input, const void* d_permuted_table, size_t u,
                        size_t col_stride, size_t m, const uint64_t beta[4], const uint64_t gamma[4], void* d_z, hipStream_t s) {
  return lookup_ratio_launch<FS>(d_input, d_table, d_permuted_input, d_permuted_table, u, col_stride, m, beta, gamma, d_z, s);
}
hipError_t perm_ratio(const PermWorkspace& w, char* base, size_t p0, size_t count, size_t u, size_t n_cols, size_t chunk_len, size_t S,
                      const uint64_t omega[4], void* d_z, size_t col_stride, hipStream_t s) {
  return perm_ratio_launch<FS>(w, base, p0, count, u, n_cols, chunk_len, S, omega, d_z, col_stride, s);
}
hipError_t perm_scan(const PermWorkspace& w, char* base, size_t p0, size_t count, size_t u, size_t S, void* d_z, size_t col_stride,
                     hipStream_t s) {
  return perm_scan_launch<FS>(w, base, p0, count, u, S, d_z, col_stride, s);
}
hipError_t expr_launch(const void* d_code, uint32_t ninstr, const void* const* d_cols, uint32_t ncols, const uint32_t* d_masks,
                       const void* d_consts, uint32_t nconsts, void* d_out, size_t out_stride, uint32_t step, uint32_t rows, uint32_t count,
                       size_t lds_bytes, hipStream_t s) {
  return pk::expr_kernel_launch<FS>((const pk::XInstr*)d_code, ninstr, (const U128* const*)d_cols, ncols, d_masks, (const U128*)d_consts,
                                    nconsts, (U128*)d_out, out_stride, step, rows, count, lds_bytes, s);
}
hipError_t chacha20_scalars(void* d_out, size_t n, uint64_t first_block, const uint32_t key[8], hipStream_t s) {
  ChaChaKey k;
  memcpy(k.w, key, 32);
  hipLaunchKernelGGL(chacha20_scalars_kernel<FS>, dim3((unsigned)((n + 255) / 256)), dim3(256), 0, s, (U128*)d_out, n,
                     first_block, k);
  return hipGetLastError();
}
hipError_t poly_pointwise(void* d_a, const void* d_b, size_t total, int op, hipStream_t s) {
  hipLaunchKernelGGL(poly_pointwise_kernel<FS>, dim3(poly_grid(total)), dim3(256), 0, s, (U128*)d_a,
                     (const U128*)d_b, total, op);
  return hipGetLastError();
}

template <bool PLAIN>
__global__ void __launch_bounds__(256) modmul_rate_kernel(uint32_t* out, int iters) {
  Fe29<FB> a, b;
#pragma unroll
  for (int i = 0; i < 9; i++) {
    a.v[i] = (int32_t)((0x1234567u * (i + 1) + threadIdx.x * 2654435761u) & L29_MASK);
    b.v[i] = (int32_t)((0x7654321u * (i + 3) + blockIdx.x * 40503u) & L29_MASK);
  }
  a.v[8] &= 0xFFFFF;
  b.v[8] &= 0xFFFFF;
  for (int k = 0; k < iters; k++) a = PLAIN ? fe29_mul_plain(a, b) : fe29_mul(a, b);
  uint32_t* o = out + 9 * (size_t)(blockIdx.x * blockDim.x + threadIdx.x);
#pragma unroll
  for (int i = 0; i < 9; i++) o[i] = (uint32_t)a.v[i];
}
hipError_t modmul_rate(int blocks, int iters, hipStream_t s, double* modmul_per_s) {
  void* buf = nullptr;
  hipError_t e = hipMalloc(&buf, (size_t)blocks * 256 * 9 * 4);
  if (e != hipSuccess) return e;
  hipEvent_t e0, e1;
  (void)hipEventCreate(&e0);
  (void)hipEventCreate(&e1);
  float best = 1e30f;
  for (int r = 0; r < 8 && e == hipSuccess; r++) {
    (void)hipEventRecord(e0, s);
    if (r < 4) hipLaunchKernelGGL(modmul_rate_kernel<false>, dim3(blocks), dim3(256), 0, s, (uint32_t*)buf, iters);
    else hipLaunchKernelGGL(modmul_rate_kernel<true>, dim3(blocks), dim3(256), 0, s, (uint32_t*)buf, iters);
    (void)hipEventRecord(e1, s);
    e = hipEventSynchronize(e1);
    float ms = 0;
    if (e == hipSuccess) e = hipEventElapsedTime(&ms, e0, e1);
    if ((r & 3) > 0 && ms < best) best = ms;
  }
  (void)hipEventDestroy(e0);
  (void)hipEventDestroy(e1);
  (void)hipFree(buf);
  if (e == hipSuccess) *modmul_per_s = (double)blocks * 256.0 * iters / (best * 1e-3);
  return e;
}

template <class FP>
int selftest_field_t(int op, const uint64_t* a_, const uint64_t* b_, uint64_t* out) {
  Fe<FP> a, b, r;
  memcpy(a.v, a_, 32);
  memcpy(b.v, b_, 32);
  switch (op) {
    case 9: r = fe29_to_api(fe29_mul(fe29_from_api(a), fe29_from_api(b))); break;
    case 10: r = fe29_to_api(fe29_add(fe29_from_api(a), fe29_from_api(b))); break;
    case 11: r = fe29_to_api(fe29_sub(fe29_from_api(a), fe29_from_api(b))); break;
    case 12: {
      const Fe29<FP> x = fe29_from_api(a), y = fe29_from_api(b);
      const Fe29<FP> d = fe29_sub(x, y);
      r = fe29_to_api(fe29_norm(fe29_sub(fe29_sub(fe29_sub(fe29_sqr(d), fe29_mul(x, y)), y), y)));
      break;
    }
    case 0: r = fe_add(a, b); break;
    case 1: r = fe_sub(a, b); break;
    case 2: r = fe_mul(a, b); break;
    case 3: r = fe_inv(a); break;
    case 4: r = fe_to_mont(a); break;
    case 5: r = fe_from_mont(a); break;
    case 6: r = fe_neg(a); break;
    default: return -1;
  }
  memcpy(out, r.v, 32);
  return 0;
}
int selftest_field(int which, int op, const uint64_t* a, const uint64_t* b, uint64_t* out) {
  return which == 0 ? selftest_field_t<FB>(op, a, b, out) : selftest_field_t<FS>(op, a, b, out);
}
template <class FP>
__global__ void selftest_field_kernel(int op, const U128* a_, const U128* b_, U128* out, uint32_t n) {
  const uint32_t i = blockIdx.x * blockDim.x + threadIdx.x;
  if (i >= n) return;
  Fe<FP> a = fe_load<FP>(a_ + 2 * (size_t)i), b = fe_load<FP>(b_ + 2 * (size_t)i), r;
  switch (op) {
    case 0: r = fe_add(a, b); break;
    case 1: r = fe_sub(a, b); break;
    case 2: r = fe_mul(a, b); break;
    case 3: r = fe_inv(a); break;
    case 4: r = fe_to_mont(a); break;
    case 5: r = fe_from_mont(a); break;
    case 7: r = fe_mul_cios(a, b); break;
// ... 135 lines not shown
```

### halo2_prover_amd/csrc/h2_curve_ops.hpp

```cpp
#pragma once
#include <hip/hip_runtime.h>
#include <stddef.h>
#include <stdint.h>

namespace h2 {

struct U128;
struct MsmGeom;
struct MsmWorkspace;
struct LookupWorkspace;
struct PermWorkspace;

struct PolyEvalJob {
  const void* poly;
  uint32_t point[8];
};

struct LincombTerm {
  const void* poly;
  uint32_t coeff[8];
};
struct LincombJob {
  void* out;
  uint32_t first_term, n_terms, first_low, n_low, first_point, n_points;
};
static_assert(sizeof(LincombTerm) == 40 && sizeof(LincombJob) == 32, "the C ABI's layout");

struct CurveOps {
  int curve_id;
  int scalar_field_id;
  uint32_t scalar_bits;
  hipError_t (*kernel_setup)();
  hipError_t (*table_build)(const void* d_bases, void* d_table, void* d_scratch, uint32_t n, const MsmGeom& g, uint32_t* d_bad, hipStream_t s);
  hipError_t (*msm_launch)(const void* d_table, const void* const* per_column_tables, uint32_t n_bases, const void* d_scalars, size_t n, size_t col_stride, size_t m,
                           const MsmGeom& g, char* ws_base, const MsmWorkspace& ws, hipStream_t s,
                           hipEvent_t ev_start, hipEvent_t ev_stop, hipEvent_t ev_tail,
                           void* d_out_jac ,
                           bool zeroed );
  hipError_t (*msm_points_launch)(const void* d_points_affine, const void* d_scalars, size_t n, size_t col_stride, size_t m,
                                  const MsmGeom& g, char* ws_base, const MsmWorkspace& ws, hipStream_t s, void* d_out_jac,
                                  bool zeroed);
  hipError_t (*srs_powers)(void* d_out_affine, const uint64_t s_mont[4], uint32_t n, hipStream_t s);
  hipError_t (*fixed_base_mul)(void* d_out_affine, const void* d_scalars, uint32_t n, hipStream_t s);
  hipError_t (*msm_small)(const void* const* d_points_affine, const void* const* d_scalars, const uint32_t* m, uint32_t count,
                          void* d_work, void* d_out_jac, hipStream_t s);
  hipError_t (*to_affine)(const void* d_xyzz, void* d_out, uint32_t m, hipStream_t s);
  hipError_t (*points_sum)(const void* d_in_jac, void* d_out_jac, uint32_t groups, uint32_t count, hipStream_t s);
  hipError_t (*points_decompress)(const void* d_compressed, void* d_out_affine, void* d_status, uint32_t n, hipStream_t s);
  int (*selftest_decompress)(const uint8_t in[32], uint64_t out_affine[8]);
  size_t (*ntt_table_bytes)(uint32_t log_n);
  bool (*ntt_scale_in_table)(uint32_t log_n);
  hipError_t (*ntt_twiddles)(void* d_tables, const uint64_t omega[4], uint32_t log_n, hipStream_t s, const uint64_t* scale );
  hipError_t (*ntt_launch)(void* d_data, void* d_scratch, const void* d_tw, uint32_t log_n, size_t m,
                           hipStream_t s, const uint64_t* scale );
  hipError_t (*ntt_extend_launch)(const void* d_src, size_t src_stride, uint32_t log_src, const uint64_t zeta[4], void* d_out,
                                  void* d_scratch, const void* d_tw, uint32_t log_n, size_t m, hipStream_t s);
  hipError_t (*ntt_coeff_launch)(const void* d_src, const void* d_t, size_t t_period, const uint64_t scale[4],
                                 const uint64_t zeta_inv[4], void* d_out, size_t out_len, size_t out_stride, void* d_scratch,
                                 const void* d_tw, uint32_t log_n, size_t m, hipStream_t s);
  size_t (*group_fft_scratch)(uint32_t log_n);
  hipError_t (*group_fft)(const void* d_in_jac, void* d_out_jac, void* d_scratch, const uint64_t omega[4], uint32_t log_n,
                          int lanes, hipStream_t s);
  hipError_t (*g_to_lagrange)(const void* d_in_affine, void* d_out_affine, void* d_scratch, const uint64_t omega[4],
                              const uint64_t scale[4], uint32_t log_n, int lanes, hipStream_t s);
  void (*selftest_glv_split)(const uint64_t k_canonical[4], uint32_t out[10]);
  void (*selftest_glv_constants)(uint64_t lambda[4], uint64_t beta[4]);
  int glv_bits;
  hipError_t (*poly_scale)(void* d_a, size_t total, const uint64_t c[4], hipStream_t s);
  hipError_t (*poly_powers)(void* d_a, size_t n, size_t m, const uint64_t g[4], hipStream_t s);
  hipError_t (*poly_mul_periodic)(void* d_a, size_t total, const void* d_t, size_t period, hipStream_t s);
  hipError_t (*poly_pointwise)(void* d_a, const void* d_b, size_t total, int op, hipStream_t s);
  hipError_t (*poly_inverse)(void* d_a, size_t total, hipStream_t s);
  hipError_t (*poly_scan)(int mode, const void* const* d_a, void* const* d_out, const uint64_t* z, uint32_t jobs, size_t n,
                          void* d_ws, hipStream_t s);
  hipError_t (*poly_eval)(const PolyEvalJob* d_jobs, uint32_t jobs, size_t n, void* d_ws, void* d_out, hipStream_t s);
  hipError_t (*poly_lincomb)(const LincombJob* d_jobs, uint32_t jobs, const LincombTerm* d_terms, const void* d_low, size_t n,
                             hipStream_t s);
  hipError_t (*lookup_permute)(const void* d_input, const void* d_table, size_t col_stride, const LookupWorkspace& ws, char* ws_base,
                               void* d_permuted_input, void* d_permuted_table, uint32_t* d_status, hipStream_t s);
  hipError_t (*lookup_ratio)(const void* d_input, const void* d_table, const void* d_permuted_input, const void* d_permuted_table,
                             size_t u, size_t col_stride, size_t m, const uint64_t beta[4], const uint64_t gamma[4], void* d_z,
                             hipStream_t s);
  hipError_t (*perm_ratio)(const PermWorkspace& w, char* base, size_t p0, size_t count, size_t u, size_t n_cols, size_t chunk_len,
                           size_t S, const uint64_t omega[4], void* d_z, size_t col_stride, hipStream_t s);
  hipError_t (*perm_scan)(const PermWorkspace& w, char* base, size_t p0, size_t count, size_t u, size_t S, void* d_z, size_t col_stride,
                          hipStream_t s);
  hipError_t (*expr_launch)(const void* d_code, uint32_t ninstr, const void* const* d_cols, uint32_t ncols, const uint32_t* d_masks,
                            const void* d_consts, uint32_t nconsts, void* d_out, size_t out_stride, uint32_t step, uint32_t rows,
                            uint32_t count, size_t lds_bytes, hipStream_t s);
  hipError_t (*chacha20_scalars)(void* d_out, size_t n, uint64_t first_block, const uint32_t key[8], hipStream_t s);
  hipError_t (*ipa_begin)(const void* d_p, const uint64_t x3[4], uint32_t k, void* d_state, hipStream_t s);
  hipError_t (*ipa_round)(uint32_t k, uint32_t j, void* d_state, const uint64_t* u_prev, const uint64_t* u_prev_inv,
                          const uint64_t z[4], const uint64_t l_blind[4], const uint64_t r_blind[4], hipStream_t s);
  hipError_t (*ipa_final)(uint32_t k, void* d_state, const uint64_t u[4], const uint64_t uinv[4], void* d_out, void* d_s_out,
                          hipStream_t s);
  hipError_t (*ipa_s_products)(const uint64_t* u, uint32_t k, const uint64_t init[4], void* d_out, hipStream_t s);
  int (*selftest_field)(int which , int op, const uint64_t* a,
                        const uint64_t* b, uint64_t* out);
  int (*selftest_curve)(int op, const uint64_t* p, const uint64_t* q, uint64_t* out);
  hipError_t (*selftest_field_device)(int which, int op, const void* d_a, const void* d_b, void* d_out, uint32_t n,
                                      hipStream_t s);
  hipError_t (*selftest_curve_device)(int op, const void* d_p, const void* d_q, void* d_out, uint32_t n, hipStream_t s);
  int (*selftest_digits)(const uint64_t* scalar_mont, size_t n_for_geometry, uint32_t* out, uint32_t cap);
  hipError_t (*modmul_rate)(int blocks, int iters, hipStream_t s, double* modmul_per_s);
};

const CurveOps* curve_ops_bn254();
const CurveOps* curve_ops_pallas();
const CurveOps* curve_ops_vesta();

}
```

### halo2_prover_amd/csrc/h2_internal.hpp

```cpp
#pragma once
#include <hip/hip_runtime.h>

#include <map>
#include <memory>
#include <mutex>
#include <string>
#include <vector>

#include "../../include/h2hip.h"
#include "h2_curve_ops.hpp"
#include "h2_msm.hpp"

namespace h2 {

struct Arena {
  void* p = nullptr;
  size_t bytes = 0;
  hipEvent_t ev = nullptr;
  hipStream_t last = nullptr;
  bool used = false;
  size_t clean_off = 0, clean_bytes = 0;
};

constexpr int H2_ARENA_SLOTS = 4;
struct ArenaSet {
  Arena slot[H2_ARENA_SLOTS];
  hipStream_t owner[H2_ARENA_SLOTS] = {};
  bool owned[H2_ARENA_SLOTS] = {};
  uint64_t used_at[H2_ARENA_SLOTS] = {};
  uint64_t clock = 0, takeovers = 0;
  Arena& of(hipStream_t s) {
    int pick = -1;
    for (int i = 0; i < H2_ARENA_SLOTS && pick < 0; i++)
      if (owned[i] && owner[i] == s) pick = i;
    for (int i = 0; i < H2_ARENA_SLOTS && pick < 0; i++)
      if (!owned[i]) pick = i;
    if (pick < 0) {
      pick = 0;
      for (int i = 1; i < H2_ARENA_SLOTS; i++)
        if (used_at[i] < used_at[pick]) pick = i;
      takeovers++;
    }
    owned[pick] = true;
    owner[pick] = s;
    used_at[pick] = ++clock;
    return slot[pick];
  }
};

struct TwiddleEntry {
  int field;
  uint32_t log_n;
  uint64_t omega[4];
  bool scaled;
  uint64_t scale[4];
  void* tw;
  uint64_t stamp;
};

struct DevCtx {
  int device = -1;
  hipStream_t stream = nullptr;
  hipStream_t side_stream = nullptr;
  hipEvent_t side_ev[3] = {nullptr, nullptr, nullptr};
  ArenaSet msm_ws, ntt_ws;
  Arena stage, div_ws;
  hipEvent_t shard_ev = nullptr;
  hipEvent_t tail_event = nullptr;
  hipEvent_t tail_wait = nullptr;
  bool tail_recorded = false, tail_wanted = false;
  std::vector<TwiddleEntry> twiddles;
  uint64_t stamp = 0;
  std::vector<std::pair<hipEvent_t, hipEvent_t>> prof_events;
  size_t prof_used = 0;
  double prof_alg_bytes = 0;
};

struct BasesEntry {
  int curve;
  size_t n;
  MsmGeom geom;
  std::vector<void*> table;
  size_t table_bytes;
};

struct ExprEntry {
  int curve;
  h2_expr_info_t info;
  std::vector<uint32_t> code;
  std::vector<uint64_t> table;
  std::vector<uint32_t> var_slot;
  std::vector<uint8_t> dump;
  std::vector<void*> d_code;
};

struct Global {
  bool ready = false;
  std::vector<DevCtx> ctx;
  std::map<uint64_t, BasesEntry> bases;
  std::map<uint64_t, ExprEntry> exprs;
  uint64_t next_handle = 1;
  bool profiling = false;
  std::string last_error;
};

extern Global g_h2;
extern std::recursive_mutex g_h2_mu;

struct TestKnobs {
  uint64_t msm_max_entries = (1ull << 31) - 1;
  bool msm_guard = false, msm_guard_poke = false;
  bool sort2_pack = true;
  size_t points_small_max = MSM_POINTS_SMALL_MAX;
  int gfft_lanes = 0;
};
struct TestCounters {
  uint64_t guard_launches = 0, guard_violations = 0;
  std::string guard_first;
  uint64_t arena_growths = 0, arena_waits = 0;
};
extern TestKnobs g_knobs;
extern TestCounters g_counts;

struct DeviceGuard {
  int prev = -1;
  bool switched = false;
  explicit DeviceGuard(int device) {
    if (hipGetDevice(&prev) == hipSuccess && prev != device) switched = hipSetDevice(device) == hipSuccess;
  }
  ~DeviceGuard() {
    if (switched) (void)hipSetDevice(prev);
  }
};

int dev_fail(hipError_t e, const char* where);
inline int launched(hipError_t e, const char* what) { return e == hipSuccess ? H2_OK : dev_fail(e, what); }
const CurveOps* ops_of(int curve);
bool curve_ok(int c);
DevCtx* ctx_current();
size_t ctx_index(const DevCtx* c);

int device_alloc(void** p, size_t bytes, const char* what);
struct HipFree { void operator()(void* p) const { (void)hipFree(p); } };
using DeviceBuffer = std::unique_ptr<void, HipFree>;

struct ArenaLease {
  Arena& a;
  hipStream_t s;
  size_t clean_bytes = 0;
  int rc;
  ArenaLease(Arena& arena, size_t want, hipStream_t stream);
  ArenaLease(const ArenaLease&) = delete;
  ~ArenaLease() noexcept;
  int release();
  int wait();
 private:
  bool released = false;
  int acquire(size_t want);
};

int msm_device_run(DevCtx& c, int curve, const BasesEntry& be, const void* d_scalars, size_t first_base, size_t n,
                   size_t col_stride, size_t m, void* d_out, bool affine_out, hipStream_t stream,
                   const BasesEntry* const* per_column = nullptr);
size_t msm_cols_per_launch(const MsmGeom& geom, size_t n);
struct MsmGroupPlan {
  size_t cols;
  MsmWorkspace ws;
  const char* broken;
};
inline MsmGroupPlan msm_plan_group(const MsmGeom& g, size_t n_bases, size_t n, size_t m, size_t col_stride, bool guard, bool pack) {
  MsmGroupPlan p{};
  p.cols = std::min(m, msm_cols_per_launch(g, n));
  if (p.cols == 0) return p;
  p.ws = msm_workspace(n, p.cols, g, guard ? 256u : 0u, n_bases, pack);
  p.broken = msm_check(p.ws, g, n, p.cols, col_stride, (uint32_t)n_bases, p.ws.total);
  return p;
}
inline MsmGroupPlan msm_points_plan_group(const MsmGeom& g, size_t n, size_t m, size_t col_stride, bool guard) {
  MsmGroupPlan p{};
  p.cols = std::min(m, msm_points_cols_per_launch(g, n));
  if (p.cols == 0) return p;
  p.ws = msm_points_workspace(n, p.cols, g, guard ? 256u : 0u);
  p.broken = msm_points_check(p.ws, g, n, p.cols, col_stride, p.ws.total);
  return p;
}
int ntt_enqueue(DevCtx& c, int curve, void* d_a, size_t m, const uint64_t omega[4], uint32_t log_n, hipStream_t stream,
                const uint64_t* scale = nullptr);
int coeff_to_extended_enqueue(DevCtx& c, int curve, const void* d_coeff, size_t col_stride, uint32_t log_n, size_t m,
                              const uint64_t zeta[4], const uint64_t ext_omega[4], uint32_t ext_log_n, void* d_out,
                              hipStream_t stream);
int poly_eval_enqueue(DevCtx& c, int curve, const void* const* d_polys, size_t n, const uint64_t* points, size_t q, void* d_out,
                      hipStream_t stream);
int extended_to_coeff_enqueue(DevCtx& c, int curve, const void* d_ext, uint32_t ext_log_n, size_t m,
                              const uint64_t ext_omega_inv[4], const uint64_t scale[4], const uint64_t zeta_inv[4], const void* d_t,
                              size_t t_period, void* d_out, size_t out_len, size_t out_stride, hipStream_t stream);
int permutation_product_enqueue(DevCtx& c, int curve, const void* const* d_values, const void* const* d_sigma, size_t n_cols,
                                size_t chunk_len, size_t u, size_t m, const uint64_t* beta, const uint64_t* gamma, const uint64_t omega[4],
                                const uint64_t delta[4], void* d_z, size_t col_stride, hipStream_t stream);
int msm_common_checks(int curve, uint64_t handle, size_t first, size_t n, size_t m, const BasesEntry** be);

#define H2_TRY(call)                                        \
  do {                                                      \
    hipError_t _e = (call);                                 \
    if (_e != hipSuccess) return ::h2::dev_fail(_e, #call); \
  } while (0)

}
```

### halo2_prover_amd/csrc/h2_msm.hpp

```cpp
#pragma once
#include "h2_curve29.hpp"
#include "h2_curve_quad.hpp"
#include "h2_tune.hpp"
#include <hip/hip_ext.h>
#include <algorithm>
#include <cstdlib>

namespace h2 {

#ifdef H2_TAIL_STAMPS
__device__ unsigned long long* h2_stamps;
#define H2_STAMP(slot)                                                                                              \
  do {                                                                                                              \
    if (threadIdx.x == 0) h2_stamps[((size_t)blockIdx.y * gridDim.x + blockIdx.x) * 16 + (slot)] = wall_clock64(); \
  } while (0)
#else
#define H2_STAMP(slot)
#endif

constexpr uint32_t MSM_SIGN = 0x80000000u;
constexpr uint32_t MSM_MAX_WINDOWS = 48;
constexpr uint32_t MSM_HOT_SPAN = 256;
constexpr uint32_t MSM_HOT_SEG = 128;
constexpr uint32_t MSM_NOT_HOT = 0xFFFFFFFFu;
// ... 968 lines not shown
  using FB = typename CV::Base;
  Fe<FS> k = fe_from_mont(fe_pow_u64(s, (uint64_t)i));
  Affine<CV> g;
#pragma unroll
  for (int j = 0; j < 8; j++) {
    g.x.v[j] = CV::GX(j);
    g.y.v[j] = CV::GY(j);
  }
  Xyzz<CV> r = Xyzz<CV>::identity();
  for (int bit = 255; bit >= 0; bit--) {
    r = xyzz_double(r);
    if ((k.v[bit >> 5] >> (bit & 31)) & 1) r = xyzz_add_affine(r, g);
  }
  Affine<CV> a = xyzz_to_affine(r);
  fe_store<FB>(out + 4 * (size_t)i, a.x);
  fe_store<FB>(out + 4 * (size_t)i + 2, a.y);
}

template <class CV>
__global__ void __launch_bounds__(256)
fixed_base_mul_kernel(U128* __restrict__ out, const U128* __restrict__ scalars, uint32_t n) {
  const uint32_t i = blockIdx.x * blockDim.x + threadIdx.x;
  if (i >= n) return;
  using FS = typename CV::Scalar;
  using FB = typename CV::Base;
  Fe<FS> k = fe_from_mont(fe_load<FS>(scalars + 2 * (size_t)i));
  Affine<CV> g;
#pragma unroll
  for (int j = 0; j < 8; j++) {
    g.x.v[j] = CV::GX(j);
    g.y.v[j] = CV::GY(j);
  }
  Xyzz<CV> r = Xyzz<CV>::identity();
  for (int bit = 255; bit >= 0; bit--) {
    r = xyzz_double(r);
    if ((k.v[bit >> 5] >> (bit & 31)) & 1) r = xyzz_add_affine(r, g);
  }
  Affine<CV> a = xyzz_to_affine(r);
  fe_store<FB>(out + 4 * (size_t)i, a.x);
  fe_store<FB>(out + 4 * (size_t)i + 2, a.y);
}

constexpr uint32_t MSM_WS_REGIONS = 32;
constexpr uint8_t MSM_GUARD_BYTE = 0xA5;
struct MsmRegion {
  const char* name;
  size_t off, bytes;
};
struct MsmWorkspace {
  size_t n, m;
  size_t K;
  size_t E;
  size_t nblk;
  uint32_t T;
  size_t nchunks;
  uint32_t log_g;
  uint32_t tile;
  uint32_t staged;
  size_t stage_lds;
  MsmStagePack pack;
  uint32_t sort2;
  Sort2Geom s2;
  uint32_t lb;
  uint32_t rc;
  size_t off_counts, off_gcounts, off_offsets, off_tile_base, off_tile_hist, off_blocksums, off_ref, off_key, off_misc, off_bsum,
      off_head, off_tail, off_xsum, off_rc, off_part, off_done, off_tree2, off_hot_slot, off_hot_tasks, off_hot_part, off_hot_arrive, total;
  size_t off_cstart, off_group_base, off_mid_ref, off_mid_lo;
  size_t off_points;
  size_t zero_bytes;
  uint32_t max_tasks;
  uint32_t guard;
  uint32_t n_regions;
  MsmRegion regions[MSM_WS_REGIONS];
};
inline size_t h2_align256(size_t x) { return (x + 255) & ~(size_t)255; }

inline bool msm_use_sort2(size_t n, size_t m, const MsmGeom& g) {
  const int forced = tune_int("H2_TUNE_SORT2", -1);
  const Sort2Geom s = msm_sort2_geom(n, g);
  const bool fits = g.B >= S2_MAX_F / 8 && s.F <= S2_MAX_F && (size_t)s.Hc * m <= S2_MAX_H;
  if (forced >= 0) return forced != 0 && fits;
  return fits && g.B > 4096;
}

struct MsmPointsShape {
  size_t m;
  uint32_t W;
};
inline MsmWorkspace msm_workspace(size_t n, size_t m, const MsmGeom& g, uint32_t guard = 0, size_t n_bases = 0,
                                  bool allow_pack = true, const MsmPointsShape* pts = nullptr) {
  if (!n_bases) n_bases = n;
  MsmWorkspace ws{};
  ws.n = n;
  ws.m = m;
  ws.guard = guard;
  ws.K = m * g.B;
  ws.E = m * g.W * n;
  ws.nblk = (ws.K + SCAN_BLOCK - 1) / SCAN_BLOCK;
  const uint64_t t_max = (uint64_t)tune_int("H2_TUNE_TMAX", 64);
  uint64_t T = t_max;
  {
    uint64_t best = ~0ull;
    for (uint64_t w = MSM_CHUNK_WAVES; w >= 2; w--) {
      uint64_t t = (ws.E + w * 65536 - 1) / (w * 65536);
      if (t < 8) t = 8;
      if (t > t_max) continue;
      const uint64_t cost = w * t * (w == 2 ? 21 : 20);
      if (cost < best) { best = cost; T = t; }
    }
  }
  ws.T = (uint32_t)T;
  ws.nchunks = (ws.E + T - 1) / T;
  {
    const size_t fine = std::min<size_t>((ws.E + 7) / 8, (size_t)MSM_CHUNK_WAVES * 65536 + 1);
    if (ws.nchunks < fine) ws.nchunks = fine;
  }
  const double span = (double)g.W * (double)n / (double)g.B / (double)T + 1.0;
  uint32_t lq = 0;
  while ((1u << lq) < span && lq < 4) lq++;
  while (lq > 0 && (ws.K << lq) > 40960) lq--;
  lq = (uint32_t)tune_int("H2_TUNE_LQ", (int)lq);
  uint32_t lg = lq + 2;
  ws.log_g = lg;
  ws.sort2 = msm_use_sort2(n, m, g) ? 1u : 0u;
  ws.s2 = msm_sort2_geom(n, g, allow_pack ? n_bases : 0);
  size_t tile = (n * (pts ? pts->m : m) + 1023) / 1024;
  const size_t dense = (size_t)2 * g.B / g.W;
  if (tile < dense) tile = dense;
  if (tile < 256) tile = 256;
  tile *= (size_t)tune_int("H2_TUNE_TILE_MUL", 2);
  if (tile > n) tile = n;
  ws.staged = 0;
  ws.stage_lds = 0;
  ws.pack = MsmStagePack{};
  if (!ws.sort2 && !pts) {
    const size_t cap = MSM_STAGE_LDS_CAP;
    auto pack_of = [&](size_t t) {
      MsmStagePack pk = msm_stage_pack(g, t);
      if (!allow_pack) pk.on = 0;
      return pk;
    };
    if (g.B <= 65536 && n * m >= 8192 && msm_stage_need(g, dense, pack_of(dense).on != 0) <= cap) {
      for (size_t rounds = 1; rounds <= 2; rounds++) {
        const size_t tpc = 256 * rounds / m;
        size_t t = tpc ? (n + tpc - 1) / tpc : (n * m + 256 * rounds - 1) / (256 * rounds);
        if (t < dense) t = dense;
        if (t < 256) t = 256;
        if (t > n) t = n;
        const MsmStagePack pk = pack_of(t);
        if (msm_stage_need(g, t, pk.on != 0) <= cap) {
          tile = t;
          ws.staged = 1;
          ws.stage_lds = msm_stage_need(g, t, pk.on != 0);
          ws.pack = pk;
          break;
        }
      }
    }
  }
  ws.tile = (uint32_t)tile;
  ws.lb = (g.c - 1) / 2;
  ws.rc = (1u << (g.c - 1 - ws.lb)) + (1u << ws.lb);
  size_t o = 0;
  auto region = [&](const char* name, size_t bytes) {
    const size_t at = o;
    if (ws.n_regions < MSM_WS_REGIONS) ws.regions[ws.n_regions++] = MsmRegion{name, at, bytes};
    o = h2_align256(o + bytes) + (guard ? h2_align256(guard) : 0);
    return at;
  };
  const size_t tiles = (n + ws.tile - 1) / ws.tile;
  if (ws.sort2) {
    const size_t H = (size_t)ws.s2.Hc * m, t2 = (size_t)ws.s2.tiles * m;
    ws.zero_bytes = 256 + H * 4;
    ws.off_misc = region("zeroed: misc + coarse counters", ws.zero_bytes);
    ws.off_gcounts = ws.off_misc + 256;
    ws.off_counts = ws.off_gcounts;
    ws.off_cstart = region("coarse bin starts", (H + 1) * 4);
    ws.off_offsets = region("offsets", (ws.K + 1) * 4);
    ws.off_tile_base = region("tile bases", t2 * ws.s2.Hc * 4);
    ws.off_tile_hist = region("tile counts", t2 * ws.s2.Hc * 4);
    ws.off_group_base = region("group bases", (size_t)ws.s2.groups * m * ws.s2.Hc * 4);
    ws.off_mid_ref = region("coarse-sorted entries", ws.E * 4);
    ws.off_mid_lo = region("coarse-sorted low key bits", ws.s2.pack_shift ? 0 : ws.E);
    ws.off_blocksums = ws.off_cstart;
  } else {
    ws.zero_bytes = 256 + h2_align256(ws.K * 4) + MSM_XCDS * ws.K * 4;
    ws.off_misc = region("zeroed: misc + counts + group counters", ws.zero_bytes);
    ws.off_counts = ws.off_misc + 256;
    ws.off_gcounts = ws.off_counts + h2_align256(ws.K * 4);
    ws.off_offsets = region("offsets", (ws.K + 1) * 4);
    ws.off_tile_base = region("tile bases", tiles * ws.K * 4);
    ws.off_tile_hist = region("tile counts", ws.staged ? tiles * ws.K * 4 : 0);
    ws.off_blocksums = region("scan block sums", (ws.nblk + 1) * 4);
  }
  ws.off_ref = region("sorted entries", ws.E * 4 + 16);
  ws.off_key = region("chunk first keys", (ws.nchunks + 1) * 4);
  ws.off_bsum = region("bucket sums", ws.K * (XYZZ29_WORDS * 4));
  ws.off_head = region("chunk heads", ws.nchunks * (XYZZ29_WORDS * 4));
  ws.off_tail = region("chunk tails", ws.nchunks * (XYZZ29_WORDS * 4));
  ws.off_xsum = region("bucket point sums", ws.K * (XYZZ29_WORDS * 4));
  ws.off_rc = region("row / column sums", m * ws.rc * (XYZZ29_WORDS * 4));
  ws.off_part = region("final partials", m * MSM_FINAL_MAX_BLOCKS * (XYZZ29_WORDS * 4));
  ws.off_done = region("final counters", m * 4);
  ws.off_tree2 = region("results", m * (XYZZ29_WORDS * 4));
  ws.max_tasks = (uint32_t)(ws.nchunks / MSM_HOT_SEG + 2 * (ws.nchunks / MSM_HOT_SPAN) + 16);
  ws.off_hot_slot = region("hot slots", ws.K * 4);
  ws.off_hot_tasks = region("hot tasks", (size_t)ws.max_tasks * 8);
  ws.off_hot_part = region("hot partials", (size_t)ws.max_tasks * (XYZZ29_WORDS * 4));
  ws.off_hot_arrive = region("hot arrivals", (size_t)ws.max_tasks * 4);
  ws.off_points = pts ? region("packed points", n * 64) : 0;
  ws.total = o;
  return ws;
}

#define MSM_REQUIRE(cond) \
  do {                    \
    if (!(cond)) return #cond; \
  } while (0)
inline const char* msm_check(const MsmWorkspace& ws, const MsmGeom& g, size_t n, size_t m, size_t col_stride,
                             uint32_t n_bases, size_t arena_bytes) {
  auto bytes_at = [&](size_t off) -> size_t {
    for (uint32_t r = 0; r < ws.n_regions; r++)
      if (off >= ws.regions[r].off && off < ws.regions[r].off + ws.regions[r].bytes)
        return ws.regions[r].off + ws.regions[r].bytes - off;
    return 0;
  };
  MSM_REQUIRE(ws.n == n && ws.m == m);
  MSM_REQUIRE(n >= 1 && m >= 1 && n <= n_bases);
  MSM_REQUIRE(m == 1 || col_stride >= n);
  MSM_REQUIRE(ws.n_regions < MSM_WS_REGIONS);
  MSM_REQUIRE(ws.total <= arena_bytes);
  for (uint32_t r = 0; r + 1 < ws.n_regions; r++)
    MSM_REQUIRE(ws.regions[r].off + ws.regions[r].bytes + ws.guard <= ws.regions[r + 1].off);
  MSM_REQUIRE(ws.regions[ws.n_regions - 1].off + ws.regions[ws.n_regions - 1].bytes + ws.guard <= ws.total);
  MSM_REQUIRE(g.W >= 1 && g.W <= MSM_MAX_WINDOWS && g.B == (1u << (g.c - 1)) && g.c <= MSM_MAX_C);
  MSM_REQUIRE(ws.sort2 || g.c <= MSM_MAX_C_ONE_LEVEL);
  MSM_REQUIRE((uint64_t)g.W * n_bases < (1ull << 31));
  MSM_REQUIRE(ws.K == m * (size_t)g.B && ws.E == m * (size_t)g.W * n);
  MSM_REQUIRE(ws.E < (1ull << 31) && ws.K < (1ull << 31));
  MSM_REQUIRE(bytes_at(ws.off_misc) >= ws.zero_bytes && ws.zero_bytes >= 256);
  MSM_REQUIRE(ws.zero_bytes % 16 == 0 && ws.off_misc % 16 == 0 && ws.zero_bytes / 16 < (1ull << 32));
  MSM_REQUIRE(bytes_at(ws.off_offsets) >= (ws.K + 1) * 4);
  if (ws.sort2) {
    const Sort2Geom& s = ws.s2;
    const size_t H = (size_t)s.Hc * m;
    MSM_REQUIRE(s.F * s.Hc == g.B && s.F == (1u << s.lo_bits) && s.F <= S2_MAX_F && s.Hc <= S2_MAX_HC && H <= S2_MAX_H);
    MSM_REQUIRE(s.tile >= 1 && s.tile <= S2_THREADS && (size_t)s.tile * g.W <= S2_STAGE);
    MSM_REQUIRE((size_t)s.tiles * s.tile >= n && (size_t)(s.tiles - 1) * s.tile < n);
    MSM_REQUIRE(s.tiles <= 0x7FFFFFFFu && m <= 65535);
    MSM_REQUIRE(ws.off_gcounts == ws.off_misc + 256 && ws.zero_bytes >= 256 + H * 4);
    MSM_REQUIRE(bytes_at(ws.off_cstart) >= (H + 1) * 4);
    MSM_REQUIRE(bytes_at(ws.off_tile_base) >= (size_t)s.tiles * m * s.Hc * 4);
    MSM_REQUIRE(bytes_at(ws.off_tile_hist) >= (size_t)s.tiles * m * s.Hc * 4);
    MSM_REQUIRE(bytes_at(ws.off_mid_ref) >= ws.E * 4 && (s.pack_shift || bytes_at(ws.off_mid_lo) >= ws.E));
    MSM_REQUIRE(s.group >= 1 && s.group <= S2_GROUP && (size_t)s.groups * s.group >= s.tiles && bytes_at(ws.off_group_base) >= (size_t)s.groups * m * s.Hc * 4);
    MSM_REQUIRE(!s.pack_shift || (((uint64_t)g.W * n_bases <= (1ull << s.pack_shift)) && s.pack_shift + s.lo_bits <= 31));
    MSM_REQUIRE((size_t)s.Hc * 8 <= 64 * 1024);
    MSM_REQUIRE(msm_sort2_lds_scatter(s, g) <= 160 * 1024 - 512 && msm_sort2_lds_fine() + 4 * S2_MAX_F * 4 <= 160 * 1024 - 512);
  } else {
    const size_t tiles = (n + ws.tile - 1) / ws.tile;
    MSM_REQUIRE(ws.tile >= 1 && tiles * m < (1ull << 31) - MSM_XCDS);
    MSM_REQUIRE(msm_tile_grid((uint32_t)tiles, (uint32_t)m) >= tiles * m);
    MSM_REQUIRE((size_t)g.B * 4 <= 128 * 1024);
    MSM_REQUIRE(ws.off_counts == ws.off_misc + 256 && ws.off_gcounts >= ws.off_counts + ws.K * 4);
    MSM_REQUIRE(ws.off_gcounts + MSM_XCDS * ws.K * 4 <= ws.off_misc + ws.zero_bytes);
    MSM_REQUIRE(bytes_at(ws.off_tile_base) >= tiles * ws.K * 4);
    if (ws.staged) {
      MSM_REQUIRE(bytes_at(ws.off_tile_hist) >= tiles * ws.K * 4);
      MSM_REQUIRE(g.B <= 65536);
      MSM_REQUIRE(ws.stage_lds >= (size_t)8 * g.B + (size_t)(ws.pack.on ? 4 : 6) * ws.tile * g.W && ws.stage_lds <= MSM_STAGE_LDS_CAP);
      MSM_REQUIRE(!ws.pack.on || (g.B <= (1ull << ws.pack.bbits) && ws.tile <= (1ull << ws.pack.ibits) && g.W <= (1ull << ws.pack.wbits) &&
                                  ws.pack.bbits + ws.pack.ibits + ws.pack.wbits <= 31));
      MSM_REQUIRE(m > 256 || tiles * m <= 512);
    }
    if (ws.K > SCAN_LDS_MAX) {
      MSM_REQUIRE(ws.nblk * SCAN_BLOCK >= ws.K && ws.nblk < (1ull << 31));
      MSM_REQUIRE(bytes_at(ws.off_blocksums) >= (ws.nblk + 1) * 4);
    }
  }
  MSM_REQUIRE(bytes_at(ws.off_ref) >= ((ws.E + 3) & ~(size_t)3) * 4);
  MSM_REQUIRE(ws.T >= 8 && ws.nchunks >= (ws.E + ws.T - 1) / ws.T);
  MSM_REQUIRE(ws.nchunks >= std::min<size_t>((ws.E + 7) / 8, (size_t)MSM_CHUNK_WAVES * 65536 + 1));
  MSM_REQUIRE((ws.nchunks + 255) / 256 < (1ull << 31));
  MSM_REQUIRE(bytes_at(ws.off_key) >= ws.nchunks * 4);
  MSM_REQUIRE(bytes_at(ws.off_head) >= ws.nchunks * (XYZZ29_WORDS * 4) && bytes_at(ws.off_tail) >= ws.nchunks * (XYZZ29_WORDS * 4));
  MSM_REQUIRE(bytes_at(ws.off_bsum) >= ws.K * (XYZZ29_WORDS * 4) && bytes_at(ws.off_xsum) >= ws.K * (XYZZ29_WORDS * 4));
  MSM_REQUIRE(ws.log_g >= 2 && ws.log_g <= 6 && ((ws.K << ws.log_g) + 255) / 256 < (1ull << 31));
  MSM_REQUIRE(ws.lb < g.c && ws.rc == (1u << (g.c - 1 - ws.lb)) + (1u << ws.lb));
  MSM_REQUIRE(bytes_at(ws.off_rc) >= m * ws.rc * (XYZZ29_WORDS * 4));
  MSM_REQUIRE(msm_final_blocks(g.c - 1, ws.lb) <= MSM_FINAL_MAX_BLOCKS);
  MSM_REQUIRE(bytes_at(ws.off_part) >= m * MSM_FINAL_MAX_BLOCKS * (XYZZ29_WORDS * 4));
  MSM_REQUIRE(bytes_at(ws.off_done) >= m * 4 && bytes_at(ws.off_tree2) >= m * (XYZZ29_WORDS * 4));
  MSM_REQUIRE(bytes_at(ws.off_hot_slot) >= ws.K * 4);
  MSM_REQUIRE(bytes_at(ws.off_hot_tasks) >= (size_t)ws.max_tasks * 8);
  MSM_REQUIRE(bytes_at(ws.off_hot_part) >= (size_t)ws.max_tasks * (XYZZ29_WORDS * 4));
  MSM_REQUIRE(bytes_at(ws.off_hot_arrive) >= (size_t)ws.max_tasks * 4);
  MSM_REQUIRE(ws.max_tasks >= 1 && msm_fixup_task_blocks(ws.max_tasks) >= 1);
  MSM_REQUIRE(((ws.K << ws.log_g) + 255) / 256 + msm_fixup_task_blocks(ws.max_tasks) < (1ull << 31));
  MSM_REQUIRE(m <= 65535);
  return nullptr;
}
#undef MSM_REQUIRE

static __global__ void __launch_bounds__(256)
msm_guard_check_kernel(const uint8_t* __restrict__ arena, MsmWorkspace ws, uint32_t* __restrict__ bad ) {
  const uint32_t r = blockIdx.x;
  const size_t from = ws.regions[r].off + ws.regions[r].bytes;
  const size_t to = r + 1 < ws.n_regions ? ws.regions[r + 1].off : ws.total;
  uint32_t c = 0;
  for (size_t i = from + threadIdx.x; i < to; i += blockDim.x) c += arena[i] != MSM_GUARD_BYTE;
  if (c) atomicAdd(&bad[r], c);
}

template <class CV>
inline hipError_t msm_kernel_setup() {
  hipError_t e;
  const int lds = (int)((1u << (MSM_MAX_C_ONE_LEVEL - 1)) * 4);
  if ((e = hipFuncSetAttribute((const void*)msm_digits_kernel<CV>, hipFuncAttributeMaxDynamicSharedMemorySize, lds)) != hipSuccess) return e;
  if ((e = hipFuncSetAttribute((const void*)msm_scatter_kernel<CV>, hipFuncAttributeMaxDynamicSharedMemorySize, lds)) != hipSuccess) return e;
  if ((e = hipFuncSetAttribute((const void*)msm_scatter_staged_kernel<CV, true>, hipFuncAttributeMaxDynamicSharedMemorySize, (int)MSM_STAGE_LDS_CAP)) != hipSuccess) return e;
  if ((e = hipFuncSetAttribute((const void*)msm_scatter_staged_kernel<CV, false>, hipFuncAttributeMaxDynamicSharedMemorySize, (int)MSM_STAGE_LDS_CAP)) != hipSuccess) return e;
  if ((e = hipFuncSetAttribute((const void*)msm2_scatter_kernel<CV>, hipFuncAttributeMaxDynamicSharedMemorySize, 160 * 1024 - 512)) != hipSuccess) return e;
  if ((e = hipFuncSetAttribute((const void*)msm2_fine_kernel, hipFuncAttributeMaxDynamicSharedMemorySize, (int)msm_sort2_lds_fine())) != hipSuccess) return e;
  return hipFuncSetAttribute((const void*)scan_lds_kernel, hipFuncAttributeMaxDynamicSharedMemorySize, (int)(SCAN_LDS_MAX * 4));
}

inline void msm_launch_scan(char* ws_base, const MsmWorkspace& ws, hipStream_t stream) {
  uint32_t* counts = (uint32_t*)(ws_base + ws.off_counts);
  uint32_t* gcounts = (uint32_t*)(ws_base + ws.off_gcounts);
  uint32_t* offsets = (uint32_t*)(ws_base + ws.off_offsets);
  uint32_t* blocksums = (uint32_t*)(ws_base + ws.off_blocksums);
  uint32_t* misc = (uint32_t*)(ws_base + ws.off_misc);
  if (ws.K <= SCAN_LDS_MAX) {
    uint32_t per = (uint32_t)((ws.K + 1023) / 1024);
    per |= 1u;
    hipLaunchKernelGGL(scan_lds_kernel, dim3(1), dim3(1024), ws.K * 4, stream, gcounts, offsets, (uint32_t)ws.K, per);
  } else {
    hipLaunchKernelGGL(msm_group_fold_kernel, dim3((unsigned)((ws.K + 255) / 256)), dim3(256), 0, stream, gcounts, counts, ws.K);
    hipLaunchKernelGGL(scan_reduce_kernel, dim3((unsigned)ws.nblk), dim3(256), 0, stream, counts, blocksums, ws.K);
    hipLaunchKernelGGL(scan_blocksums_kernel, dim3(1), dim3(1024), 0, stream, blocksums, (uint32_t)ws.nblk, misc + 1);
    hipLaunchKernelGGL(scan_apply_kernel, dim3((unsigned)ws.nblk), dim3(256), 0, stream, counts, blocksums, offsets,
                       ws.K);
  }
}

inline MsmKeysArgs msm_keys_args(char* ws_base, const MsmWorkspace& ws) {
  MsmKeysArgs a{};
  a.chunk_first = (uint32_t*)(ws_base + ws.off_key);
  a.hot_slot = (uint32_t*)(ws_base + ws.off_hot_slot);
  a.tasks = (uint32_t*)(ws_base + ws.off_hot_tasks);
  a.hot_arrive = (uint32_t*)(ws_base + ws.off_hot_arrive);
  a.task_count = (uint32_t*)(ws_base + ws.off_misc);
  a.max_tasks = ws.max_tasks;
  a.T_host = ws.T;
  return a;
}

template <class CV>
inline hipError_t msm_launch_back(const U128* table, const U128** d_tables, uint32_t log_b, size_t m, const MsmGeom& g,
                                  char* ws_base, const MsmWorkspace& ws, const MsmKeysArgs& keys_args, bool keys_merged,
                                  hipStream_t stream, hipEvent_t ev_start, hipEvent_t ev_stop, hipEvent_t ev_tail, U128* d_out_jac) {
  uint32_t* offsets = (uint32_t*)(ws_base + ws.off_offsets);
  uint32_t* sref = (uint32_t*)(ws_base + ws.off_ref);
  uint32_t* chunk_first = (uint32_t*)(ws_base + ws.off_key);
  uint32_t* misc = (uint32_t*)(ws_base + ws.off_misc);
  uint32_t* bsum = (uint32_t*)(ws_base + ws.off_bsum);
  uint32_t* head = (uint32_t*)(ws_base + ws.off_head);
  uint32_t* tail = (uint32_t*)(ws_base + ws.off_tail);
  uint32_t* xsum = (uint32_t*)(ws_base + ws.off_xsum);
  uint32_t* rc = (uint32_t*)(ws_base + ws.off_rc);
  uint32_t* tree2 = (uint32_t*)(ws_base + ws.off_tree2);
  uint32_t* hot_slot = (uint32_t*)(ws_base + ws.off_hot_slot);
  uint32_t* hot_tasks = (uint32_t*)(ws_base + ws.off_hot_tasks);
  uint32_t* hot_part = (uint32_t*)(ws_base + ws.off_hot_part);
  uint32_t* hot_arrive = (uint32_t*)(ws_base + ws.off_hot_arrive);
  if (!keys_merged)
    hipLaunchKernelGGL(msm_keys_kernel, dim3((unsigned)((ws.K + MSM_KEYS_THREADS - 1) / MSM_KEYS_THREADS)), dim3(MSM_KEYS_THREADS), 0,
                       stream, (const uint32_t*)offsets, ws.K, keys_args);
  hipEvent_t ev_end = ev_stop ? ev_stop : ev_tail;
  if (ev_start || ev_end)
    hipExtLaunchKernelGGL(msm_chunk_kernel<CV>, dim3((unsigned)((ws.nchunks + 255) / 256)), dim3(256), 0, stream, ev_start, ev_end,
                          0, table, (const U128* const*)d_tables, log_b, (const uint32_t*)sref, (const uint32_t*)chunk_first,
                          (const uint32_t*)offsets, ws.K, ws.T, bsum, head, tail);
  else
    hipLaunchKernelGGL(msm_chunk_kernel<CV>, dim3((unsigned)((ws.nchunks + 255) / 256)), dim3(256), 0, stream, table,
                       (const U128* const*)d_tables, log_b, sref, chunk_first, offsets, ws.K, ws.T, bsum, head, tail);
  if (ev_stop && ev_tail) (void)hipEventRecord(ev_tail, stream);
  const size_t fix_threads = ws.K << ws.log_g;
  const uint32_t task_blocks = msm_fixup_task_blocks(ws.max_tasks);
  hipLaunchKernelGGL(msm_fixup_kernel<CV>, dim3((unsigned)((fix_threads + 255) / 256) + task_blocks), dim3(256), 0, stream, offsets,
                     ws.K, ws.T, ws.log_g, bsum, head, tail, hot_slot, hot_tasks, misc, ws.max_tasks, task_blocks, hot_part,
                     hot_arrive, xsum);
  uint32_t* part = (uint32_t*)(ws_base + ws.off_part);
  uint32_t* done = (uint32_t*)(ws_base + ws.off_done);
  hipLaunchKernelGGL(msm_rowcol_kernel<CV>, dim3(ws.rc, (unsigned)m), dim3(64 * msm_rowcol_waves(g.c - 1, ws.lb, m)), 0, stream,
                     xsum, rc, done, g.c - 1, ws.lb, (U128*)misc, (uint32_t)(ws.zero_bytes / 16));
  hipLaunchKernelGGL(msm_final_kernel<CV>, dim3(msm_final_blocks(g.c - 1, ws.lb), (unsigned)m), dim3(64), 0, stream, rc, part,
                     done, tree2, d_out_jac, g.c - 1, ws.lb);
  return hipGetLastError();
}

template <class CV>
inline hipError_t msm_launch(const U128* table, const U128* const* per_column ,
                             uint32_t n_bases, const U128* d_scalars, size_t n, size_t col_stride,
                             size_t m, const MsmGeom& g, char* ws_base, const MsmWorkspace& ws, hipStream_t stream,
                             hipEvent_t ev_start = nullptr, hipEvent_t ev_stop = nullptr, hipEvent_t ev_tail = nullptr,
                             U128* d_out_jac = nullptr ,
                             bool zeroed = false ) {
  uint32_t* gcounts = (uint32_t*)(ws_base + ws.off_gcounts);
  uint32_t* offsets = (uint32_t*)(ws_base + ws.off_offsets);
  uint32_t* tile_base = (uint32_t*)(ws_base + ws.off_tile_base);
  uint32_t* sref = (uint32_t*)(ws_base + ws.off_ref);
  uint32_t* misc = (uint32_t*)(ws_base + ws.off_misc);
  hipError_t e;
  if (per_column && m > MSM_MAX_MULTI) return hipErrorInvalidValue;
  if (!zeroed && (e = hipMemsetAsync(misc, 0, ws.zero_bytes, stream)) != hipSuccess) return e;
  uint32_t* tile_hist = (ws.staged || ws.sort2) ? (uint32_t*)(ws_base + ws.off_tile_hist) : nullptr;
  const U128** d_tables = nullptr;
  uint32_t log_b = 0;
  MsmKeysArgs keys_args = msm_keys_args(ws_base, ws);
  if (per_column) {
    d_tables = (const U128**)(misc + 16);
    keys_args.n_tables = (uint32_t)m;
    keys_args.tables_dst = d_tables;
    for (size_t j = 0; j < m; j++) keys_args.tables.t[j] = per_column[j];
    while ((1u << log_b) < g.B) log_b++;
  }
  bool keys_merged = false;
  if (ws.sort2) {
    const Sort2Geom& s2 = ws.s2;
    const uint32_t H = s2.Hc * (uint32_t)m;
    uint32_t* cstart = (uint32_t*)(ws_base + ws.off_cstart);
    uint32_t* mid_ref = (uint32_t*)(ws_base + ws.off_mid_ref);
    uint8_t* mid_lo = (uint8_t*)(ws_base + ws.off_mid_lo);
    uint32_t* group_base = (uint32_t*)(ws_base + ws.off_group_base);
    hipLaunchKernelGGL(msm2_count_kernel<CV>, dim3(s2.groups, (unsigned)m), dim3(S2_THREADS), (size_t)s2.Hc * 8, stream, d_scalars,
                       gcounts, tile_base, tile_hist, group_base, (uint32_t)n, col_stride, s2, g);
    hipLaunchKernelGGL(msm2_coarse_scan_kernel, dim3(1), dim3(1024), 0, stream, gcounts, cstart, H, offsets + ws.K);
    hipLaunchKernelGGL(msm2_scatter_kernel<CV>, dim3(s2.tiles, (unsigned)m), dim3(S2_THREADS), msm_sort2_lds_scatter(s2, g), stream,
                       d_scalars, cstart, tile_base, tile_hist, group_base, mid_ref, mid_lo, (uint32_t)n, col_stride, n_bases, s2, g);
    hipLaunchKernelGGL(msm2_fine_kernel, dim3(H), dim3(S2_THREADS), msm_sort2_lds_fine(), stream, cstart, mid_ref, mid_lo, sref,
                       offsets, s2.F, s2.lo_bits, s2.pack_shift);
  } else {
    const size_t lds = (size_t)g.B * 4;
    const uint32_t tiles = (uint32_t)((n + ws.tile - 1) / ws.tile);
    const uint32_t sort_grid = msm_tile_grid(tiles, (uint32_t)m);
    hipLaunchKernelGGL(msm_digits_kernel<CV>, dim3(sort_grid), dim3(MSM_SORT_THREADS), lds, stream, d_scalars, gcounts,
                       tile_base, tile_hist, (uint32_t)n, col_stride, ws.tile, tiles, (uint32_t)m, g);
    msm_launch_scan(ws_base, ws, stream);
    if (ws.staged) {
      const size_t per = (ws.K + (size_t)tiles * m - 1) / ((size_t)tiles * m);
      keys_merged = per <= MSM_SORT_THREADS && ws.stage_lds >= (size_t)4 * (MSM_SORT_THREADS + 1);
      MsmKeysArgs ka = keys_args;
      const uint32_t grid = sort_grid;
      if (keys_merged) ka.keys_per_block = (uint32_t)per;
      auto scatter = [&](auto kernel) {
        hipLaunchKernelGGL(kernel, dim3(grid), dim3(MSM_SORT_THREADS), ws.stage_lds, stream, d_scalars, (const uint32_t*)offsets,
                           (const uint32_t*)gcounts, (const uint32_t*)tile_base, (const uint32_t*)tile_hist, sref, (uint32_t)n,
                           col_stride, n_bases, ws.tile, tiles, (uint32_t)m, g, (uint32_t)(ws.tile * g.W), ws.pack, ka);
      };
      if (ws.pack.on) scatter(msm_scatter_staged_kernel<CV, true>);
      else scatter(msm_scatter_staged_kernel<CV, false>);
    } else
      hipLaunchKernelGGL(msm_scatter_kernel<CV>, dim3(sort_grid), dim3(MSM_SORT_THREADS), lds, stream, d_scalars, offsets,
                         gcounts, tile_base, sref, (uint32_t)n, col_stride, n_bases, ws.tile, tiles, (uint32_t)m, g);
  }
  return msm_launch_back<CV>(table, d_tables, log_b, m, g, ws_base, ws, keys_args, keys_merged, stream, ev_start, ev_stop, ev_tail,
                             d_out_jac);
}

}
#include "h2_msm_points.hpp"
```

### halo2_prover_amd/csrc/h2_msm_points.hpp

```cpp
#pragma once
#include "h2_msm.hpp"

namespace h2 {

constexpr size_t MSM_POINTS_LDS_CAP = (size_t)4 << (MSM_MAX_C_ONE_LEVEL - 1);
constexpr uint32_t MSM_POINTS_MAX_C = 11;
constexpr uint32_t MSM_POINTS_MIN_C = 6;
constexpr size_t MSM_POINTS_MAX_N = (size_t)1 << 26;

inline MsmGeom msm_points_geometry(size_t n, uint32_t nbits) {
  uint32_t lg = 0;
  while (((size_t)1 << (lg + 1)) <= n) lg++;
  int c = std::max(8, (int)lg - 9);
  c = tune_int("H2_TUNE_POINTS_C", c);
  if (c < (int)MSM_POINTS_MIN_C) c = (int)MSM_POINTS_MIN_C;
  if (c > (int)MSM_POINTS_MAX_C) c = (int)MSM_POINTS_MAX_C;
  MsmGeom g{};
  g.nbits = nbits;
  const uint32_t total = nbits + 1;
  g.W = (total + c - 1) / c;
  const uint32_t base = total / g.W, extra = total % g.W;
  g.wbase = base;
  g.wextra = extra;
  uint32_t o = 0;
  for (uint32_t w = 0; w < g.W; w++) {
    g.off[w] = (uint8_t)o;
    g.width[w] = (uint8_t)(base + (w < extra ? 1 : 0));
    o += g.width[w];
  }
  g.c = base + (extra ? 1 : 0);
  g.B = 1u << (g.c - 1);
  return g;
}
inline MsmGeom msm_points_virtual(const MsmGeom& g) {
  MsmGeom v{};
  v.c = g.c;
  v.W = 1;
  v.B = g.B;
  v.nbits = g.nbits;
  v.wbase = g.c;
  v.wextra = 0;
  v.off[0] = 0;
  v.width[0] = (uint8_t)g.c;
  return v;
}
inline MsmWorkspace msm_points_workspace(size_t n, size_t m, const MsmGeom& g, uint32_t guard = 0) {
  const MsmPointsShape shape{m, g.W};
  return msm_workspace(n, m * g.W, msm_points_virtual(g), guard, n, true, &shape);
}
inline size_t msm_points_cols_per_launch(const MsmGeom& g, size_t n) {
  const uint64_t by_entries = ((1ull << 31) - 1) / ((uint64_t)g.W * n);
  const uint64_t by_keys = std::min<uint64_t>(((1ull << 31) - 1) / ((uint64_t)g.W * g.B), 65535u / g.W);
  return (size_t)std::min(by_entries, by_keys);
}

template <class CV>
__global__ void __launch_bounds__(256)
msm_points_pack_kernel(const U128* __restrict__ points, U128* __restrict__ packed, uint32_t n) {
  const uint32_t i = blockIdx.x * blockDim.x + threadIdx.x;
  if (i >= n) return;
  affine29_store_table<CV>(packed + 4 * (size_t)i, affine_load<CV>(points + 4 * (size_t)i));
}

template <class CV>
__global__ void __launch_bounds__(1024)
msm_points_digits_kernel(const U128* __restrict__ scalars, uint32_t* __restrict__ gcounts, uint32_t* __restrict__ tile_base,
                         uint32_t n, size_t col_stride , uint32_t tile, uint32_t tiles, uint32_t m, MsmGeom g) {
  using S = typename CV::Scalar;
  extern __shared__ uint32_t hist[];
  const MsmTileId id = msm_tile_id(tiles, m);
  if (!id.live) return;
  const uint32_t WB = g.W * g.B, log_b = g.c - 1;
  for (uint32_t b = threadIdx.x; b < WB; b += blockDim.x) hist[b] = 0;
  __syncthreads();
  const uint32_t lo = id.tile * tile, hi = min(lo + tile, n);
  for (uint32_t i = lo + threadIdx.x; i < hi; i += blockDim.x) {
    MsmDigits dg(fe_from_mont(fe_load<S>(scalars + 2 * (col_stride * id.col + i))).v);
    for (uint32_t w = 0; w < g.W; w++) {
      const uint32_t enc = dg.next(g, w);
      if (enc) atomicAdd(&hist[(w << log_b) + (enc & ~MSM_SIGN) - 1], 1u);
    }
  }
  __syncthreads();
  const size_t K = (size_t)m * WB;
  uint32_t* gc = gcounts + (size_t)id.group * K + (size_t)id.col * WB;
  for (uint32_t idx = threadIdx.x; idx < WB; idx += blockDim.x) {
    const uint32_t h = hist[idx], w = idx >> log_b, b = idx & (g.B - 1);
    const size_t vcol = (size_t)id.col * g.W + w;
    tile_base[(vcol * tiles + id.tile) * g.B + b] = h ? atomicAdd(&gc[idx], h) : 0u;
  }
}

template <class CV>
__global__ void __launch_bounds__(1024)
msm_points_scatter_kernel(const U128* __restrict__ scalars, const uint32_t* __restrict__ offsets,
                          const uint32_t* __restrict__ gcounts, const uint32_t* __restrict__ tile_base,
                          uint32_t* __restrict__ sorted_ref, uint32_t n, size_t col_stride , uint32_t tile,
                          uint32_t tiles, uint32_t m, MsmGeom g) {
  using S = typename CV::Scalar;
  extern __shared__ uint32_t hist[];
  const MsmTileId id = msm_tile_id(tiles, m);
  if (!id.live) return;
  const uint32_t WB = g.W * g.B, log_b = g.c - 1;
  const size_t K = (size_t)m * WB;
  const uint32_t* gc = gcounts + (size_t)id.col * WB;
  const uint32_t* of = offsets + (size_t)id.col * WB;
  for (uint32_t idx = threadIdx.x; idx < WB; idx += blockDim.x) {
    const uint32_t w = idx >> log_b, b = idx & (g.B - 1);
    const size_t vcol = (size_t)id.col * g.W + w;
    uint32_t at = of[idx] + tile_base[(vcol * tiles + id.tile) * g.B + b];
    for (uint32_t x = 0; x < id.group; x++) at += gc[x * K + idx];
    hist[idx] = at;
  }
  __syncthreads();
  const uint32_t lo = id.tile * tile, hi = min(lo + tile, n);
  for (uint32_t i = lo + threadIdx.x; i < hi; i += blockDim.x) {
    MsmDigits dg(fe_from_mont(fe_load<S>(scalars + 2 * (col_stride * id.col + i))).v);
    for (uint32_t w = 0; w < g.W; w++) {
      const uint32_t enc = dg.next(g, w);
      if (enc) {
        const uint32_t pos = atomicAdd(&hist[(w << log_b) + (enc & ~MSM_SIGN) - 1], 1u);
        sorted_ref[pos] = i | (enc & MSM_SIGN);
      }
    }
  }
}

template <class CV>
__global__ void __launch_bounds__(64)
msm_points_combine_kernel(const uint32_t* __restrict__ results ,
                          U128* __restrict__ out_jac, uint32_t m, MsmGeom g) {
  __builtin_amdgcn_s_setprio(3);
  using P = Xyzz29<CV>;
  using F = Fe29<typename CV::Base>;
  using B = typename CV::Base;
  const uint32_t col = blockIdx.x * 16 + (threadIdx.x >> 2), q = threadIdx.x & 3u;
  const bool live = col < m;
  P acc = P::identity();
#pragma nounroll
  for (uint32_t w = g.W; w-- > 0;) {
    const uint32_t width = g.wbase + (w < g.wextra ? 1u : 0u);
#pragma nounroll
    for (uint32_t k = 0; k < width; k++) acc = xyzz29_double_quad(acc);
    const P r = live ? xyzz29_load<CV>(results + XYZZ29_WORDS * ((size_t)col * g.W + w)) : P::identity();
    acc = xyzz29_add_quad(acc, r);
  }
  const F one = fe29_one<CV>();
  const F prod = fe29_mul(quad_select(q, acc.x, acc.y, acc.zz, acc.zz), quad_select(q, acc.zz, acc.zzz, one, one));
  Fe<B> v = fe29_to_api(prod);
  if (acc.is_identity()) v = Fe<B>::zero();
  if (live && q < 3) fe_store<B>(out_jac + 6 * (size_t)col + 2 * q, v);
}

#define MSM_REQUIRE(cond) \
  do {                    \
    if (!(cond)) return #cond; \
  } while (0)
inline const char* msm_points_check(const MsmWorkspace& ws, const MsmGeom& g, size_t n, size_t m, size_t col_stride,
                                    size_t arena_bytes) {
  MSM_REQUIRE(n >= 1 && m >= 1 && n <= MSM_POINTS_MAX_N);
  MSM_REQUIRE(col_stride >= n);
  MSM_REQUIRE(g.c >= MSM_POINTS_MIN_C && g.c <= MSM_POINTS_MAX_C && g.W >= 1 && g.W <= MSM_MAX_WINDOWS);
  MSM_REQUIRE(g.B == (1u << (g.c - 1)) && g.wbase >= 1 && g.wbase + (g.wextra ? 1u : 0u) == g.c && g.wextra < g.W);
  MSM_REQUIRE(g.wbase * g.W + g.wextra == g.nbits + 1);
  MSM_REQUIRE((uint64_t)m * g.W <= 65535);
  const MsmGeom v = msm_points_virtual(g);
  if (const char* broken = msm_check(ws, v, n, m * g.W, col_stride, (uint32_t)n, arena_bytes)) return broken;
  MSM_REQUIRE(!ws.sort2 && !ws.staged);
  MSM_REQUIRE((size_t)g.W * g.B * 4 <= MSM_POINTS_LDS_CAP);
  MSM_REQUIRE(n < (1ull << 31));
  MSM_REQUIRE(ws.K == m * (size_t)g.W * g.B && ws.E == m * (size_t)g.W * n);
  const size_t tiles = (n + ws.tile - 1) / ws.tile;
  MSM_REQUIRE(ws.tile >= 1 && tiles * ws.tile >= n && tiles * m < (1ull << 31) - MSM_XCDS);
  MSM_REQUIRE(msm_tile_grid((uint32_t)tiles, (uint32_t)m) >= tiles * m);
  MSM_REQUIRE((m - 1) * col_stride + n <= (1ull << 40));
  auto bytes_at = [&](size_t off) -> size_t {
    for (uint32_t r = 0; r < ws.n_regions; r++)
      if (off >= ws.regions[r].off && off < ws.regions[r].off + ws.regions[r].bytes)
        return ws.regions[r].off + ws.regions[r].bytes - off;
    return 0;
  };
  MSM_REQUIRE(bytes_at(ws.off_points) >= n * 64 && ws.off_points % 16 == 0);
  MSM_REQUIRE(bytes_at(ws.off_tile_base) >= tiles * m * g.W * g.B * 4);
  MSM_REQUIRE(ws.off_gcounts + MSM_XCDS * m * (size_t)g.W * g.B * 4 <= ws.off_misc + ws.zero_bytes);
  MSM_REQUIRE(bytes_at(ws.off_tree2) >= m * g.W * (XYZZ29_WORDS * 4));
  MSM_REQUIRE((n + 255) / 256 < (1ull << 31) && (m + 15) / 16 < (1ull << 31));
  return nullptr;
}
#undef MSM_REQUIRE

template <class CV>
inline hipError_t msm_points_kernel_setup() {
  hipError_t e;
  if ((e = hipFuncSetAttribute((const void*)msm_points_digits_kernel<CV>, hipFuncAttributeMaxDynamicSharedMemorySize, (int)MSM_POINTS_LDS_CAP)) != hipSuccess) return e;
  return hipFuncSetAttribute((const void*)msm_points_scatter_kernel<CV>, hipFuncAttributeMaxDynamicSharedMemorySize, (int)MSM_POINTS_LDS_CAP);
}

template <class CV>
inline hipError_t msm_points_launch(const U128* d_points, const U128* d_scalars, size_t n, size_t col_stride, size_t m,
                                    const MsmGeom& g, char* ws_base, const MsmWorkspace& ws, hipStream_t stream, U128* d_out_jac,
                                    bool zeroed) {
  uint32_t* gcounts = (uint32_t*)(ws_base + ws.off_gcounts);
  uint32_t* offsets = (uint32_t*)(ws_base + ws.off_offsets);
  uint32_t* tile_base = (uint32_t*)(ws_base + ws.off_tile_base);
  uint32_t* sref = (uint32_t*)(ws_base + ws.off_ref);
  U128* packed = (U128*)(ws_base + ws.off_points);
  hipError_t e;
  if (!zeroed && (e = hipMemsetAsync(ws_base + ws.off_misc, 0, ws.zero_bytes, stream)) != hipSuccess) return e;
  hipLaunchKernelGGL(msm_points_pack_kernel<CV>, dim3((unsigned)((n + 255) / 256)), dim3(256), 0, stream, d_points, packed, (uint32_t)n);
  const size_t lds = (size_t)g.W * g.B * 4;
  const uint32_t tiles = (uint32_t)((n + ws.tile - 1) / ws.tile);
  const uint32_t sort_grid = msm_tile_grid(tiles, (uint32_t)m);
  hipLaunchKernelGGL(msm_points_digits_kernel<CV>, dim3(sort_grid), dim3(MSM_SORT_THREADS), lds, stream, d_scalars, gcounts,
                     tile_base, (uint32_t)n, col_stride, ws.tile, tiles, (uint32_t)m, g);
  msm_launch_scan(ws_base, ws, stream);
  hipLaunchKernelGGL(msm_points_scatter_kernel<CV>, dim3(sort_grid), dim3(MSM_SORT_THREADS), lds, stream, d_scalars,
                     (const uint32_t*)offsets, (const uint32_t*)gcounts, (const uint32_t*)tile_base, sref, (uint32_t)n, col_stride,
                     ws.tile, tiles, (uint32_t)m, g);
  const MsmGeom v = msm_points_virtual(g);
  if ((e = msm_launch_back<CV>(packed, nullptr, 0, m * g.W, v, ws_base, ws, msm_keys_args(ws_base, ws), false, stream, nullptr,
                               nullptr, nullptr, nullptr)) != hipSuccess)
    return e;
  hipLaunchKernelGGL(msm_points_combine_kernel<CV>, dim3((unsigned)((m + 15) / 16)), dim3(64), 0, stream,
                     (const uint32_t*)(ws_base + ws.off_tree2), d_out_jac, (uint32_t)m, g);
  return hipGetLastError();
}

}
```

### halo2_prover_amd/csrc/h2_selftest.hip

```cpp
#include "h2_internal.hpp"
#include "h2_field29_chain.hpp"

#include <cstdio>

#include "../../include/h2hip_selftest.h"

using namespace h2;

extern "C" int h2_selftest_field_op(int field, int op, const uint64_t a[4], const uint64_t b[4], uint64_t out[4]) {
  if (!a || !b || !out) return H2_EINVAL;
  int rc = -1;
  switch (field) {
    case 0: rc = curve_ops_bn254()->selftest_field(0, op, a, b, out); break;
    case 1: rc = curve_ops_bn254()->selftest_field(1, op, a, b, out); break;
    case 2: rc = curve_ops_pallas()->selftest_field(0, op, a, b, out); break;
    case 3: rc = curve_ops_pallas()->selftest_field(1, op, a, b, out); break;
  }
  return rc == 0 ? H2_OK : H2_EINVAL;
}
template <class FP>
H2_HD void selftest_fe29_run(int op, const int32_t* in, int32_t* out) {
  Fe29<FP> a[4];
  for (int k = 0; k < 4; k++)
    for (int l = 0; l < 9; l++) a[k].v[l] = in[9 * k + l];
  Fe29<FP> r;
  switch (op) {
    case 0: r = fe29_mul(a[0], a[1]); break;
    case 1: r = fe29_sqr(a[0]); break;
    case 2: r = fe29_mul_sub(a[0], a[1], a[2], a[3]); break;
    default: r = fe29_mul_up(a[0], a[1]); break;
  }
  for (int l = 0; l < 9; l++) out[l] = r.v[l];
}
template <class FP>
__global__ void __launch_bounds__(64) selftest_fe29_kernel(int op, const int32_t* __restrict__ in, int32_t* __restrict__ out,
                                                           uint32_t n) {
  const uint32_t i = blockIdx.x * blockDim.x + threadIdx.x;
  if (i >= n) return;
  selftest_fe29_run<FP>(op, in + 36 * (size_t)i, out + 9 * (size_t)i);
}
extern "C" int h2_selftest_fe29_op(int field, int op, const int32_t in[36], int32_t out[9]) {
  if (!in || !out || op < 0 || op > 3) return H2_EINVAL;
  switch (field) {
    case 0: selftest_fe29_run<BN254_FQ>(op, in, out); return H2_OK;
    case 1: selftest_fe29_run<BN254_FR>(op, in, out); return H2_OK;
    case 2: selftest_fe29_run<PASTA_FP>(op, in, out); return H2_OK;
    case 3: selftest_fe29_run<PASTA_FQ>(op, in, out); return H2_OK;
  }
  return H2_EINVAL;
}
extern "C" int h2_selftest_fe29_op_device(int field, int op, const int32_t* in, int32_t* out, size_t n) {
  std::lock_guard<std::recursive_mutex> lk(g_h2_mu);
  if (!g_h2.ready) return H2_ENOTINIT;
  if (!in || !out || n == 0 || n > (1u << 20) || field < 0 || field > 3 || op < 0 || op > 3) return H2_EINVAL;
  DevCtx& g_ctx = g_h2.ctx[0];
  DeviceGuard dg(g_ctx.device);
  const size_t in_bytes = n * 36 * 4, out_bytes = n * 9 * 4;
  ArenaLease stage(g_ctx.stage, in_bytes + out_bytes, g_ctx.stream);
  if (stage.rc != H2_OK) return stage.rc;
  int32_t* d_in = (int32_t*)g_ctx.stage.p;
  int32_t* d_out = (int32_t*)((char*)g_ctx.stage.p + in_bytes);
  H2_TRY(hipMemcpyAsync(d_in, in, in_bytes, hipMemcpyHostToDevice, g_ctx.stream));
  const dim3 grid((unsigned)((n + 63) / 64)), block(64);
  switch (field) {
    case 0: hipLaunchKernelGGL(selftest_fe29_kernel<BN254_FQ>, grid, block, 0, g_ctx.stream, op, d_in, d_out, (uint32_t)n); break;
    case 1: hipLaunchKernelGGL(selftest_fe29_kernel<BN254_FR>, grid, block, 0, g_ctx.stream, op, d_in, d_out, (uint32_t)n); break;
    case 2: hipLaunchKernelGGL(selftest_fe29_kernel<PASTA_FP>, grid, block, 0, g_ctx.stream, op, d_in, d_out, (uint32_t)n); break;
    default: hipLaunchKernelGGL(selftest_fe29_kernel<PASTA_FQ>, grid, block, 0, g_ctx.stream, op, d_in, d_out, (uint32_t)n); break;
  }
  if (int rc = launched(hipGetLastError(), "selftest_fe29_kernel"); rc != H2_OK) return rc;
  H2_TRY(hipMemcpyAsync(out, d_out, out_bytes, hipMemcpyDeviceToHost, g_ctx.stream));
  return stage.wait();
}
template <class FP>
__global__ void __launch_bounds__(64) selftest_fe29_chain_kernel(int op, const int32_t* __restrict__ in, int32_t* __restrict__ out_cpp,
                                                                 int32_t* __restrict__ out_chain, uint32_t n) {
  const uint32_t i = blockIdx.x * blockDim.x + threadIdx.x;
  if (i >= n) return;
  Fe29<FP> a[4];
  for (int k = 0; k < 4; k++)
    for (int l = 0; l < 9; l++) a[k].v[l] = in[36 * (size_t)i + 9 * k + l];
  Fe29<FP> r, c;
  switch (op) {
    case 0: r = fe29_mul(a[0], a[1]); c = Fe29Chain::mul(a[0], a[1]); break;
    case 1: r = fe29_sqr(a[0]); c = Fe29Chain::sqr(a[0]); break;
    case 2: r = fe29_mul_sub(a[0], a[1], a[2], a[3]); c = Fe29Chain::mul_sub(a[0], a[1], a[2], a[3]); break;
    default: r = fe29_mul_up(a[0], a[1]); c = Fe29Chain::mul_up(a[0], a[1]); break;
  }
  for (int l = 0; l < 9; l++) {
    out_cpp[9 * (size_t)i + l] = r.v[l];
    out_chain[9 * (size_t)i + l] = c.v[l];
  }
}
extern "C" int h2_selftest_fe29_chain_device(int field, int op, const int32_t* in, int32_t* out_cpp, int32_t* out_chain, size_t n) {
  std::lock_guard<std::recursive_mutex> lk(g_h2_mu);
  if (!g_h2.ready) return H2_ENOTINIT;
  if (!in || !out_cpp || !out_chain || n == 0 || n > (1u << 20) || field < 2 || field > 3 || op < 0 || op > 3) return H2_EINVAL;
  static_assert(chain29::covers<PASTA_FP>() && chain29::covers<PASTA_FQ>(), "the Pasta fields take the chain form");
  DevCtx& g_ctx = g_h2.ctx[0];
  DeviceGuard dg(g_ctx.device);
  const size_t in_bytes = n * 36 * 4, out_bytes = n * 9 * 4;
  ArenaLease stage(g_ctx.stage, in_bytes + 2 * out_bytes, g_ctx.stream);
  if (stage.rc != H2_OK) return stage.rc;
  int32_t* d_in = (int32_t*)g_ctx.stage.p;
  int32_t* d_cpp = (int32_t*)((char*)g_ctx.stage.p + in_bytes);
  int32_t* d_chain = (int32_t*)((char*)g_ctx.stage.p + in_bytes + out_bytes);
  H2_TRY(hipMemcpyAsync(d_in, in, in_bytes, hipMemcpyHostToDevice, g_ctx.stream));
  const dim3 grid((unsigned)((n + 63) / 64)), block(64);
  if (field == 2)
    hipLaunchKernelGGL(selftest_fe29_chain_kernel<PASTA_FP>, grid, block, 0, g_ctx.stream, op, d_in, d_cpp, d_chain, (uint32_t)n);
  else
    hipLaunchKernelGGL(selftest_fe29_chain_kernel<PASTA_FQ>, grid, block, 0, g_ctx.stream, op, d_in, d_cpp, d_chain, (uint32_t)n);
  if (int rc = launched(hipGetLastError(), "selftest_fe29_chain_kernel"); rc != H2_OK) return rc;
  H2_TRY(hipMemcpyAsync(out_cpp, d_cpp, out_bytes, hipMemcpyDeviceToHost, g_ctx.stream));
  H2_TRY(hipMemcpyAsync(out_chain, d_chain, out_bytes, hipMemcpyDeviceToHost, g_ctx.stream));
  return stage.wait();
}
extern "C" int h2_selftest_curve_op(int curve, int op, const uint64_t p[8], const uint64_t q[8], uint64_t out[8]) {
  const CurveOps* ops = ops_of(curve);
  if (!ops || !p || !q || !out) return H2_EINVAL;
  return ops->selftest_curve(op, p, q, out) == 0 ? H2_OK : H2_EINVAL;
}
extern "C" int h2_selftest_digits(int curve, const uint64_t scalar[4], size_t n_for_geometry, uint32_t* out,
                                  uint32_t cap) {
  const CurveOps* ops = ops_of(curve);
  if (!ops || !scalar || !out) return H2_EINVAL;
  return ops->selftest_digits(scalar, n_for_geometry, out, cap);
}
extern "C" int h2_selftest_curve_op_device(int curve, int op, const uint64_t* p, const uint64_t* q, uint64_t* out,
                                           size_t n) {
  std::lock_guard<std::recursive_mutex> lk(g_h2_mu);
  if (!g_h2.ready) return H2_ENOTINIT;
  const CurveOps* ops = ops_of(curve);
  if (!ops || !p || !q || !out || n == 0 || n > (1u << 20)) return H2_EINVAL;
  DevCtx& g_ctx = g_h2.ctx[0];
  DeviceGuard dg(g_ctx.device);
  ArenaLease stage(g_ctx.stage, 3 * n * 64, g_ctx.stream);
  if (stage.rc != H2_OK) return stage.rc;
  char* d = (char*)g_ctx.stage.p;
  H2_TRY(hipMemcpyAsync(d, p, n * 64, hipMemcpyHostToDevice, g_ctx.stream));
  H2_TRY(hipMemcpyAsync(d + n * 64, q, n * 64, hipMemcpyHostToDevice, g_ctx.stream));
  if (int rc = launched(ops->selftest_curve_device(op, d, d + n * 64, d + 2 * n * 64, (uint32_t)n, g_ctx.stream), "selftest_curve_kernel");
      rc != H2_OK)
    return rc;
  H2_TRY(hipMemcpyAsync(out, d + 2 * n * 64, n * 64, hipMemcpyDeviceToHost, g_ctx.stream));
  return stage.wait();
}

extern "C" int h2_selftest_field_op_device(int field, int op, const uint64_t* a, const uint64_t* b, uint64_t* out,
                                           size_t n) {
  std::lock_guard<std::recursive_mutex> lk(g_h2_mu);
  if (!g_h2.ready) return H2_ENOTINIT;
  if (!a || !b || !out || n == 0 || n > (1u << 24) || field < 0 || field > 3) return H2_EINVAL;
  const CurveOps* ops = field < 2 ? curve_ops_bn254() : curve_ops_pallas();
  const int which = field & 1;
  DevCtx& g_ctx = g_h2.ctx[0];
  DeviceGuard dg(g_ctx.device);
  ArenaLease stage(g_ctx.stage, 3 * n * 32, g_ctx.stream);
  if (stage.rc != H2_OK) return stage.rc;
  char* d = (char*)g_ctx.stage.p;
  H2_TRY(hipMemcpyAsync(d, a, n * 32, hipMemcpyHostToDevice, g_ctx.stream));
  H2_TRY(hipMemcpyAsync(d + n * 32, b, n * 32, hipMemcpyHostToDevice, g_ctx.stream));
  if (int rc = launched(ops->selftest_field_device(which, op, d, d + n * 32, d + 2 * n * 32, (uint32_t)n, g_ctx.stream), "selftest_field_kernel");
      rc != H2_OK)
    return rc;
  H2_TRY(hipMemcpyAsync(out, d + 2 * n * 32, n * 32, hipMemcpyDeviceToHost, g_ctx.stream));
  return stage.wait();
}

extern "C" int h2_selftest_msm_guard(int on) {
  std::lock_guard<std::recursive_mutex> lk(g_h2_mu);
  g_knobs.msm_guard = on != 0;
  g_knobs.msm_guard_poke = on == 2;
  g_knobs.sort2_pack = on != 3;
  g_counts.guard_launches = g_counts.guard_violations = 0;
  g_counts.guard_first.clear();
  return H2_OK;
}
extern "C" int h2_selftest_msm_guard_report(uint64_t out[2], char* first, size_t cap) {
  std::lock_guard<std::recursive_mutex> lk(g_h2_mu);
  if (!out) return H2_EINVAL;
  out[0] = g_counts.guard_launches;
  out[1] = g_counts.guard_violations;
  if (first && cap) {
    snprintf(first, cap, "%s", g_counts.guard_first.c_str());
  }
  return H2_OK;
}
extern "C" int h2_selftest_msm_check(int curve, size_t n_bases, size_t n, size_t m, size_t col_stride, int guard, uint64_t out[8]) {
  std::lock_guard<std::recursive_mutex> lk(g_h2_mu);
  const CurveOps* ops = ops_of(curve);
  if (!ops || n == 0 || m == 0 || n > n_bases) return H2_EINVAL;
  const MsmGeom g = msm_geometry(n_bases, ops->scalar_bits);
  const MsmGroupPlan plan = msm_plan_group(g, n_bases, n, m, col_stride, guard != 0, true);
  if (plan.cols == 0) return H2_EINVAL;
  if (m > plan.cols && col_stride < n) { g_h2.last_error = "msm launch geometry: col_stride >= n"; return H2_EINVAL; }
  const MsmWorkspace& ws = plan.ws;
  if (out) {
    out[0] = g.c; out[1] = g.W; out[2] = g.B; out[3] = ws.sort2 ? ws.s2.tile : ws.tile;
    out[4] = ws.staged; out[5] = ws.sort2; out[6] = ws.T; out[7] = ws.n_regions;
  }
  if (plan.broken) {
    g_h2.last_error = std::string("msm launch geometry: ") + plan.broken;
    return H2_EINVAL;
  }
  return H2_OK;
}
extern "C" int h2_selftest_msm_points_check(int curve, size_t n, size_t m, size_t col_stride, int guard, uint64_t out[8]) {
  std::lock_guard<std::recursive_mutex> lk(g_h2_mu);
  if (!curve_ok(curve) || !out || n == 0 || m == 0 || n > MSM_POINTS_MAX_N) return H2_EINVAL;
  if (col_stride < n) { g_h2.last_error = "msm points launch geometry: col_stride >= n"; return H2_EINVAL; }
  const MsmGeom g = msm_points_geometry(n, ops_of(curve)->scalar_bits);
  const MsmGroupPlan plan = msm_points_plan_group(g, n, m, col_stride, guard != 0);
  if (plan.cols == 0) return H2_EINVAL;
  const MsmWorkspace& ws = plan.ws;
  out[0] = g.c; out[1] = g.W; out[2] = g.B; out[3] = ws.tile; out[4] = (uint64_t)g.W * g.B * 4; out[5] = plan.cols;
  out[6] = ws.T; out[7] = ws.n_regions;
  if (plan.broken) {
    g_h2.last_error = std::string("msm points launch geometry: ") + plan.broken;
    return H2_EDEVICE;
  }
  return H2_OK;
}
extern "C" int h2_selftest_set_msm_points_small_max(size_t n) {
  std::lock_guard<std::recursive_mutex> lk(g_h2_mu);
  g_knobs.points_small_max = n == SIZE_MAX ? MSM_POINTS_SMALL_MAX : n;
  return H2_OK;
}
extern "C" int h2_selftest_set_gfft_lanes(int lanes) {
  std::lock_guard<std::recursive_mutex> lk(g_h2_mu);
  if (lanes != 0 && lanes != 1 && lanes != 4) return H2_EINVAL;
  g_knobs.gfft_lanes = lanes;
  return H2_OK;
}
extern "C" int h2_selftest_glv_split(int curve, const uint64_t k[4], uint32_t out[10]) {
  const CurveOps* ops = ops_of(curve);
  if (!ops || !k || !out) return H2_EINVAL;
  ops->selftest_glv_split(k, out);
  return H2_OK;
}
extern "C" int h2_selftest_glv_constants(int curve, uint64_t lambda[4], uint64_t beta[4], uint32_t* glv_bits) {
  const CurveOps* ops = ops_of(curve);
  if (!ops || !lambda || !beta || !glv_bits) return H2_EINVAL;
  ops->selftest_glv_constants(lambda, beta);
  *glv_bits = (uint32_t)ops->glv_bits;
  return H2_OK;
}
extern "C" int h2_selftest_msm_front(int curve, size_t n_bases, size_t n, size_t m, int pack, uint64_t out[12]) {
  std::lock_guard<std::recursive_mutex> lk(g_h2_mu);
  const CurveOps* ops = ops_of(curve);
  if (!ops || !out || n == 0 || m == 0 || n > n_bases || n_bases >= (1ull << 31)) return H2_EINVAL;
  const MsmGeom g = msm_geometry(n_bases, ops->scalar_bits);
  const MsmGroupPlan plan = msm_plan_group(g, n_bases, n, m, n, false, pack != 0);
  if (plan.cols < m) return H2_EINVAL;
  const MsmWorkspace& ws = plan.ws;
  const char* broken = plan.broken;
  if (broken) g_h2.last_error = std::string("msm launch geometry: ") + broken;
  out[0] = ws.sort2 ? ws.s2.tile : ws.tile; out[1] = ws.staged; out[2] = ws.stage_lds; out[3] = ws.pack.on;
  out[4] = ws.pack.bbits; out[5] = ws.pack.ibits; out[6] = ws.pack.wbits; out[7] = broken ? 0 : 1;
  out[8] = msm_effective_t((uint32_t)ws.E, ws.T); out[9] = MSM_HOT_SPAN; out[10] = MSM_HOT_SEG; out[11] = ws.max_tasks;
  return H2_OK;
}
extern "C" int h2_selftest_arena_stats(uint64_t out[4]) {
  std::lock_guard<std::recursive_mutex> lk(g_h2_mu);
  DevCtx* c = g_h2.ready ? ctx_current() : nullptr;
  if (!c || !out) return H2_EINVAL;
  out[0] = g_counts.arena_growths;
  out[1] = g_counts.arena_waits;
  out[2] = c->msm_ws.takeovers;
  out[3] = c->ntt_ws.takeovers;
  return H2_OK;
}
extern "C" int h2_selftest_msm_tiles(uint32_t tiles, uint32_t m) {
  if (tiles == 0 || m == 0 || (uint64_t)tiles * m > (1u << 24)) return H2_EINVAL;
  const uint32_t grid = msm_tile_grid(tiles, m);
  std::vector<uint8_t> seen((size_t)tiles * m, 0);
  size_t live = 0;
  for (uint32_t b = 0; b < grid; b++) {
    const MsmTileId t = msm_tile_id_of(b, tiles, m);
    if (!t.live) continue;
    if (t.col >= m || t.tile >= tiles || t.group >= MSM_XCDS || seen[(size_t)t.col * tiles + t.tile]) return H2_EINVAL;
    seen[(size_t)t.col * tiles + t.tile] = 1;
    live++;
  }
  return live == (size_t)tiles * m ? H2_OK : H2_EINVAL;
}

extern "C" int h2_selftest_set_msm_max_entries(uint64_t limit) {
  std::lock_guard<std::recursive_mutex> lk(g_h2_mu);
  g_knobs.msm_max_entries = (limit > 0 && limit < (1ull << 31) - 1) ? limit : (1ull << 31) - 1;
  return H2_OK;
}

extern "C" int h2_selftest_modmul_rate(int curve, int waves_per_simd, int iters, double* modmul_per_s) {
  std::lock_guard<std::recursive_mutex> lk(g_h2_mu);
  if (!g_h2.ready) return H2_ENOTINIT;
  const CurveOps* ops = ops_of(curve);
  if (!ops || !modmul_per_s || waves_per_simd < 1 || waves_per_simd > 8 || iters < 1 || iters > (1 << 20)) return H2_EINVAL;
  DevCtx* c = ctx_current();
  if (!c) return H2_EINVAL;
  hipDeviceProp_t prop;
  H2_TRY(hipGetDeviceProperties(&prop, c->device));
  return launched(ops->modmul_rate(prop.multiProcessorCount * waves_per_simd, iters, c->stream, modmul_per_s), "modmul_rate_kernel");
}
```

### halo2_prover_amd/lib.py

```python
import ctypes
import os

_HERE = os.path.dirname(os.path.abspath(__file__))
LIB_PATH = os.path.join(_HERE, "libh2hip.so")

H2_BN254, H2_PALLAS, H2_VESTA = 0, 1, 2
CURVES = {"bn254": H2_BN254, "pallas": H2_PALLAS, "vesta": H2_VESTA}

H2_OK = 0
STATUS_NAMES = {0: "H2_OK", -1: "H2_EINVAL", -2: "H2_ENOMEM", -3: "H2_EDEVICE", -4: "H2_EHANDLE", -5: "H2_ENOTINIT",
                -6: "H2_EPROOF"}

_P, _Z, _I, _U32, _U64 = ctypes.c_void_p, ctypes.c_size_t, ctypes.c_int, ctypes.c_uint32, ctypes.c_uint64


class Profile(ctypes.Structure):
    _fields_ = [("launches", _U64), ("kernel_ms", ctypes.c_double), ("algorithmic_bytes", ctypes.c_double)]


class MsmPlan(ctypes.Structure):
    _fields_ = [("window_bits", _U32), ("windows", _U32), ("buckets", _U32), ("table_bytes", _U64)]


class MsmPointsPlan(ctypes.Structure):
    _fields_ = [("window_bits", _U32), ("windows", _U32), ("buckets", _U32), ("route", _U32), ("scalar_bits", _U32),
                ("lds_bytes", _U32), ("lds_limit", _U32), ("reserved", _U32), ("crossover", _U64), ("max_n", _U64),
                ("width", ctypes.c_uint8 * 48), ("offset", ctypes.c_uint8 * 48)]


class ExprInfo(ctypes.Structure):
    _fields_ = [(name, _U32) for name in ("curve", "instructions", "products", "column_reads", "slots", "constants",
                                          "reductions", "n_cols", "n_vars", "lds_bytes")] + [
        ("min_rot", ctypes.c_int32), ("max_rot", ctypes.c_int32)]


SYMBOLS = {
    "h2_init": (_I, [_I]),
    "h2_init_devices": (_I, [_I, _P]),
    "h2_device_count": (_I, []),
    "h2_shutdown": (_I, []),
    "h2_strerror": (ctypes.c_char_p, [_I]),
    "h2_last_device_error": (ctypes.c_char_p, []),
    "h2_version": (_I, []),
    "h2_bases_register": (_I, [_I, _P, _Z, ctypes.POINTER(_U64)]),
    "h2_bases_register_device": (_I, [_I, _P, _Z, ctypes.POINTER(_U64)]),
    "h2_bases_release": (_I, [_U64]),
    "h2_bases_len": (ctypes.c_int64, [_U64]),
    "h2_msm": (_I, [_I, _U64, _P, _Z, _P]),
    "h2_msm_batch": (_I, [_I, _U64, _P, _Z, _Z, _P]),
    "h2_msm_device": (_I, [_I, _U64, _P, _Z, _Z, _P, _P]),
    "h2_msm_device_range": (_I, [_I, _U64, _P, _Z, _Z, _Z, _Z, _P, _P]),
    "h2_points_sum_device": (_I, [_I, _P, _Z, _Z, _P, _P]),
    "h2_points_decompress_device": (_I, [_I, _P, _Z, _P, _P, _P]),
    "h2_stream_wait_msm_tail": (_I, [_P]),
    "h2_msm_device_multi": (_I, [_I, _P, _P, _Z, _Z, _Z, _Z, _P, _P]),
    "h2_msm_points_device": (_I, [_I, _P, _P, _Z, _Z, _Z, _P, _P]),
    "h2_msm_points": (_I, [_I, _P, _P, _Z, _P]),
    "h2_msm_points_plan": (_I, [_I, _Z, ctypes.POINTER(MsmPointsPlan)]),
    "h2_ntt": (_I, [_I, _P, _P, _U32]),
    "h2_ntt_batch": (_I, [_I, _P, _Z, _P, _U32]),
    "h2_ntt_device": (_I, [_I, _P, _Z, _P, _U32, _P]),
    "h2_fft_group": (_I, [_I, _P, _P, _U32]),
    "h2_fft_group_device": (_I, [_I, _P, _P, _U32, _P]),
    "h2_g_to_lagrange_device": (_I, [_I, _P, _U32, _P, _P, _P, _P]),
    "h2_g_to_lagrange": (_I, [_I, _P, _U32, _P, _P, _P]),
    "h2_params_downsize": (_I, [_P, _Z, _U32, _P, _Z, ctypes.POINTER(_Z)]),
    "h2_ntt_scaled_device": (_I, [_I, _P, _Z, _P, _U32, _P, _P]),
    "h2_coeff_to_extended_device": (_I, [_I, _P, _Z, _U32, _Z, _P, _P, _U32, _P, _P]),
    "h2_extended_to_coeff_device": (_I, [_I, _P, _U32, _Z, _P, _P, _P, _P, _Z, _P, _Z, _Z, _P]),
    "h2_poly_scale_device": (_I, [_I, _P, _Z, _Z, _P, _P]),
    "h2_poly_coset_device": (_I, [_I, _P, _Z, _Z, _P, _P]),
    "h2_poly_mul_periodic_device": (_I, [_I, _P, _Z, _Z, _P, _Z, _P]),
    "h2_poly_pointwise_device": (_I, [_I, _I, _P, _P, _Z, _P]),
    "h2_poly_divide_linear_device": (_I, [_I, _P, _Z, _P, _P, _P]),
    "h2_poly_prefix_product_device": (_I, [_I, _P, _Z, _P, _P]),
    "h2_poly_eval_device": (_I, [_I, _P, _Z, _P, _Z, _P, _P]),
    "h2_poly_eval": (_I, [_I, _P, _Z, _P, _P]),
    "h2_poly_eval_tile": (_I, []),
    "h2_poly_lincomb_device": (_I, [_I, _P, _Z, _P, _Z, _P, _Z, _P, _Z, _Z, _P]),
    "h2_poly_lincomb_max_rounds": (_I, []),
    "h2_ipa_state_bytes": (_I, [_U32, ctypes.POINTER(_Z)]),
    "h2_ipa_begin_device": (_I, [_I, _U32, _P, _P, _P, _P]),
    "h2_ipa_round_device": (_I, [_I, _U64, _U32, _U32, _P, _P, _P, _P, _P, _P, _P, _P]),
    "h2_ipa_final_device": (_I, [_I, _U32, _P, _P, _P, _P, _P, _P]),
    "h2_ipa_challenge_products_device": (_I, [_I, _P, _U32, _P, _P, _P]),
    "h2_lookup_permute_device": (_I, [_I, _P, _P, _Z, _Z, _Z, _P, _P, _P, _P]),
    "h2_lookup_product_device": (_I, [_I, _P, _P, _P, _P, _Z, _Z, _Z, _P, _P, _P, _P]),
    "h2_lookup_tile": (_I, []),
    "h2_permutation_product_device": (_I, [_I, _P, _P, _Z, _Z, _Z, _Z, _P, _P, _P, _P, _P, _Z, _P]),
    "h2_permutation_tile": (_I, []),
    "h2_expr_compile": (_I, [_I, _P, _Z, _P, _Z, _U32, _U32, ctypes.POINTER(_U64)]),
    "h2_expr_release": (_I, [_U64]),
    "h2_expr_info": (_I, [_U64, ctypes.POINTER(ExprInfo)]),
    "h2_expr_dump": (_I, [_U64, _P, _Z, ctypes.POINTER(_Z)]),
    "h2_expr_eval_device": (_I, [_U64, _P, _P, _P, _Z, _U32, _U32, _P, _Z, _P]),
    "h2_chacha20_scalars_device": (_I, [_I, _P, _U64, _Z, _P, _P]),
    "h2_poly_inverse_device": (_I, [_I, _P, _Z, _P]),
    "h2_msm_plan": (_I, [_U64, ctypes.POINTER(MsmPlan)]),
    "h2_srs_generate": (_I, [_I, _P, _Z, _P, _P]),
    "h2_fixed_base_mul": (_I, [_I, _P, _Z, _P, _P]),
    "h2_setup": (_I, [_U32, _P, _P, _P, _Z, ctypes.POINTER(_Z)]),
    "h2_generate_proof": (_I, [_P, _Z, ctypes.c_char_p, _I, _P, _P, _P, _Z, ctypes.POINTER(_Z)]),
    "h2_generate_proofs": (_I, [_P, _Z, _Z, _P, _I, _P, _P, _P, _Z, _P, ctypes.POINTER(_Z)]),
    "h2_verify_proof": (_I, [_P, _Z, _P, _Z, ctypes.c_char_p, _I, ctypes.POINTER(_I)]),
    "h2_verify_proofs": (_I, [_P, _Z, _Z, _P, _P, _P, _I, _P, _P, _P, ctypes.POINTER(_I)]),
    "h2_simulate": (_I, [ctypes.c_char_p, _I, _P, _Z, ctypes.POINTER(_Z)]),
    "h2_circuit_count": (_I, []),
    "h2_params_cache_clear": (_I, []),
    "h2_key_cache": (_I, [_I]),
    "h2_profile_enable": (_I, [_I]),
    "h2_profile_read": (_I, [ctypes.POINTER(Profile)]),
    "h2_selftest_commit_launches": (_U64, []),
    "h2_selftest_set_prove_group": (_I, [_Z]),
    "h2_selftest_msm_points_check": (_I, [_I, _Z, _Z, _Z, _I, _P]),
    "h2_selftest_set_msm_points_small_max": (_I, [_Z]),
    "h2_selftest_set_gfft_lanes": (_I, [_I]),
    "h2_selftest_glv_split": (_I, [_I, _P, _P]),
    "h2_selftest_glv_constants": (_I, [_I, _P, _P, ctypes.POINTER(_U32)]),
}
SELFTEST_SYMBOLS = {
    "h2_selftest_field_op": (_I, [_I, _I, _P, _P, _P]),
    "h2_selftest_curve_op": (_I, [_I, _I, _P, _P, _P]),
    "h2_selftest_digits": (_I, [_I, _P, _Z, _P, _U32]),
    "h2_selftest_field_op_device": (_I, [_I, _I, _P, _P, _P, _Z]),
    "h2_selftest_curve_op_device": (_I, [_I, _I, _P, _P, _P, _Z]),
    "h2_selftest_set_msm_max_entries": (_I, [_U64]),
    "h2_selftest_modmul_rate": (_I, [_I, _I, _I, ctypes.POINTER(ctypes.c_double)]),
    "h2_selftest_host": (_I, [_I, _P, _Z, _P, _Z, ctypes.POINTER(_Z)]),
    "h2_selftest_sharded_commits": (_U64, []),
    "h2_selftest_set_shard_min_rows": (_I, [_Z]),
    "h2_selftest_msm_check": (_I, [_I, _Z, _Z, _Z, _Z, _I, _P]),
    "h2_selftest_msm_front": (_I, [_I, _Z, _Z, _Z, _I, _P]),
    "h2_selftest_msm_tiles": (_I, [_U32, _U32]),
    "h2_selftest_msm_guard": (_I, [_I]),
    "h2_selftest_msm_guard_report": (_I, [_P, _P, _Z]),
    "h2_selftest_arena_stats": (_I, [_P]),
    "h2_selftest_fe29_op": (_I, [_I, _I, _P, _P]),
    "h2_selftest_fe29_op_device": (_I, [_I, _I, _P, _P, _Z]),
    "h2_selftest_fe29_chain_device": (_I, [_I, _I, _P, _P, _P, _Z]),
    "h2_selftest_pairing_checks": (_U64, []),
    "h2_selftest_expr_run": (_I, [_P, _Z, _P, _P, _U32, _U32, _U32, _P, _P]),
}

RNG_FILL = ctypes.CFUNCTYPE(None, ctypes.c_void_p, ctypes.POINTER(ctypes.c_uint8), ctypes.c_size_t)

_lib = None


class H2Error(RuntimeError):
    def __init__(self, status, where):
        self.status = status
        detail = ""
        try:
            msg = load().h2_strerror(status).decode()
            dev = load().h2_last_device_error().decode()
            detail = msg + (" [" + dev + "]" if dev and status == -3 else "")
        except Exception:
            pass
        super().__init__("%s failed: %s (%s)" % (where, STATUS_NAMES.get(status, status), detail))


def load():
    global _lib
    if _lib is None:
        if not os.path.exists(LIB_PATH):
            raise ImportError(
                "halo2_prover_amd: %s not found -- build it with `python __graft_entry__.py build` "
                "(hipcc --offload-arch=gfx950). There is no CPU fallback." % LIB_PATH)
        try:
            import torch
        except ImportError:
            pass
        lib = ctypes.CDLL(LIB_PATH)
        for name, (res, args) in list(SYMBOLS.items()) + list(SELFTEST_SYMBOLS.items()):
            fn = getattr(lib, name)
            fn.restype = res
            fn.argtypes = args
        _lib = lib
    return _lib


def check(status, where):
    if status != H2_OK:
        raise H2Error(status, where)
```

### include/h2hip_selftest.h

```cpp
#ifndef H2HIP_SELFTEST_H
#define H2HIP_SELFTEST_H
#include <stddef.h>
#include <stdint.h>
#ifdef __cplusplus
extern "C" {
#endif
int h2_selftest_field_op(int field, int op, const uint64_t a[4], const uint64_t b[4], uint64_t out[4]);
int h2_selftest_curve_op(int curve, int op, const uint64_t p[8], const uint64_t q[8], uint64_t out[8]);
int h2_selftest_field_op_device(int field, int op, const uint64_t* a, const uint64_t* b, uint64_t* out, size_t n);
int h2_selftest_curve_op_device(int curve, int op, const uint64_t* p, const uint64_t* q, uint64_t* out, size_t n);
int h2_selftest_digits(int curve, const uint64_t scalar[4], size_t n_for_geometry, uint32_t* out, uint32_t cap);
int h2_selftest_set_msm_max_entries(uint64_t limit);
int h2_selftest_msm_check(int curve, size_t n_bases, size_t n, size_t m, size_t col_stride, int guard, uint64_t out[8]);
int h2_selftest_msm_front(int curve, size_t n_bases, size_t n, size_t m, int pack, uint64_t out[12]);
int h2_selftest_msm_tiles(uint32_t tiles, uint32_t m);
int h2_selftest_msm_guard(int on);
int h2_selftest_msm_guard_report(uint64_t out[2], char* first, size_t cap);
int h2_selftest_msm_points_check(int curve, size_t n, size_t m, size_t col_stride, int guard, uint64_t out[8]);
int h2_selftest_set_msm_points_small_max(size_t n);
int h2_selftest_set_gfft_lanes(int lanes);
int h2_selftest_glv_split(int curve, const uint64_t k[4], uint32_t out[10]);
int h2_selftest_glv_constants(int curve, uint64_t lambda[4], uint64_t beta[4], uint32_t* glv_bits);
int h2_selftest_modmul_rate(int curve, int waves_per_simd, int iters, double* modmul_per_s);
uint64_t h2_selftest_sharded_commits(void);
int h2_selftest_set_shard_min_rows(size_t rows);
uint64_t h2_selftest_commit_launches(void);
int h2_selftest_set_prove_group(size_t proofs);
int h2_selftest_host(int what, const uint8_t* in, size_t in_len, uint8_t* out, size_t cap, size_t* out_len);
int h2_selftest_fe29_op(int field, int op, const int32_t in[36], int32_t out[9]);
int h2_selftest_fe29_op_device(int field, int op, const int32_t* in, int32_t* out, size_t n);
int h2_selftest_fe29_chain_device(int field, int op, const int32_t* in, int32_t* out_cpp, int32_t* out_chain, size_t n);
int h2_selftest_expr_run(const uint8_t* dag, size_t dag_len, const uint64_t* cols, const uint32_t* log_len, uint32_t ncols,
                         uint32_t log_en, uint32_t step, uint64_t* out, uint32_t stats[6]);
int h2_selftest_arena_stats(uint64_t out[4]);
uint64_t h2_selftest_pairing_checks(void);

#ifdef __cplusplus
}
#endif
#endif
```

Measured before the change: 191.4 billion.

## Skip arena events until cross-stream sharing and carry MSM zeroing extent

Arena leases drawn from an ArenaSet no longer record a HIP event on every release. Events are recorded only after a cross-stream takeover is first seen, at which point the code does one device-wide synchronize and switches the set to eager event recording. Separately, the MSM path keeps the larger zeroed extent from a previous run so the rowcol kernel re-zeroes the whole region it may have dirtied. The aim is to cut per-launch hipEventRecord overhead, at the cost of a heavier one-time hipDeviceSynchronize on the first takeover.

Result: no change. 193.1 billion, median of 6 (+0.9%).

```diff
diff --git a/halo2_prover_amd/csrc/h2_capi.hip b/halo2_prover_amd/csrc/h2_capi.hip
--- a/halo2_prover_amd/csrc/h2_capi.hip
+++ b/halo2_prover_amd/csrc/h2_capi.hip
@@ -61,6 +61,9 @@
 }
 
 ArenaLease::ArenaLease(Arena& arena, size_t want, hipStream_t stream) : a(arena), s(stream) { rc = acquire(want); }
+ArenaLease::ArenaLease(ArenaSet& slots, size_t want, hipStream_t stream) : a(slots.of(stream)), s(stream), set(&slots) {
+  rc = acquire(want);
+}
 int ArenaLease::acquire(size_t want) {
   clean_bytes = a.bytes < want ? 0 : a.clean_bytes;
   a.clean_bytes = 0;
@@ -80,15 +83,34 @@
   if (!a.ev) H2_TRY(hipEventCreateWithFlags(&a.ev, hipEventDisableTiming));
   if (a.used && a.last != s) {
     g_counts.arena_waits++;
-    H2_TRY(hipStreamWaitEvent(s, a.ev, 0));
-  }
-  return H2_OK;
+    if (a.recorded) {
+      H2_TRY(hipStreamWaitEvent(s, a.ev, 0));
+    } else {
+      g_counts.takeover_syncs++;
+      H2_TRY(hipDeviceSynchronize());
+      a.used = false;
+      if (set) {
+        for (Arena& o : set->slot) o.used = false;
+        set->eager = true;
+      }
+    }
+  }
+  return H2_OK;
+}
+hipError_t ArenaLease::mark_used() {
+  const bool record = !set || set->eager;
+  if (record) {
+    if (hipError_t e = hipEventRecord(a.ev, s); e != hipSuccess) return e;
+    g_counts.arena_events++;
+  }
+  a.recorded = record;
+  a.last = s;
+  a.used = true;
+  return hipSuccess;
 }
 int ArenaLease::release() {
   released = true;
-  H2_TRY(hipEventRecord(a.ev, s));
-  a.last = s;
-  a.used = true;
+  H2_TRY(mark_used());
   return H2_OK;
 }
 int ArenaLease::wait() {
@@ -98,12 +120,7 @@
 }
 ArenaLease::~ArenaLease() noexcept {
   if (rc != H2_OK || released) return;
-  if (hipEventRecord(a.ev, s) == hipSuccess) {
-    a.last = s;
-    a.used = true;
-  } else {
-    (void)hipGetLastError();
-  }
+  if (mark_used() != hipSuccess) (void)hipGetLastError();
 }
 static void arena_free(Arena& a) {
   if (a.p) (void)hipFree(a.p);
@@ -141,7 +158,7 @@
     if (scan_ws.rc != H2_OK) return fail(scan_ws.rc);
     uint32_t* d_bad = (uint32_t*)scan_ws.a.p;
     uint32_t bad = 0;
-    ArenaLease table_ws(src.msm_ws.of(src.stream), be.table_bytes / 64 * MSM_TABLE_SCRATCH, src.stream);
+    ArenaLease table_ws(src.msm_ws, be.table_bytes / 64 * MSM_TABLE_SCRATCH, src.stream);
     if (table_ws.rc != H2_OK) return fail(table_ws.rc);
     hipError_t e = hipMemsetAsync(d_bad, 0, 4, src.stream);
     if (e == hipSuccess) e = ops->table_build(d_affine, be.table[si], table_ws.a.p, (uint32_t)n, g, d_bad, src.stream);
@@ -214,7 +231,7 @@
 static int msm_run_group(DevCtx& c, hipStream_t stream, const MsmGroupPlan& plan, const char* route, const char* label, size_t m,
                          const char* guard_what, Launch&& launch, Finish&& finish) {
   const MsmWorkspace& ws = plan.ws;
-  ArenaLease lease(c.msm_ws.of(stream), ws.total, stream);
+  ArenaLease lease(c.msm_ws, ws.total, stream);
   if (lease.rc != H2_OK) return lease.rc;
   Arena& A = lease.a;
   if (const char* broken = plan.broken ? plan.broken : ws.total <= A.bytes ? nullptr : "ws.total <= arena_bytes") {
@@ -224,12 +241,14 @@
   const bool guard = g_knobs.msm_guard;
   if (guard) H2_TRY(hipMemsetAsync(A.p, MSM_GUARD_BYTE, ws.total, stream));
   const bool zeroed = !guard && lease.clean_bytes >= ws.zero_bytes && A.clean_off == ws.off_misc;
-  if (int rc = launched(launch((char*)A.p, zeroed), label); rc != H2_OK) return rc;
+  const size_t zero_extent = msm_zero_extent(ws, zeroed ? lease.clean_bytes : 0);
+  if (!zeroed) g_counts.msm_memsets++;
+  if (int rc = launched(launch((char*)A.p, zeroed, zero_extent), label); rc != H2_OK) return rc;
   if (guard) {
     if (int rc = msm_guard_inspect(ws, (char*)A.p, stream, m, guard_what); rc != H2_OK) return rc;
   } else {
     A.clean_off = ws.off_misc;
-    A.clean_bytes = ws.zero_bytes;
+    A.clean_bytes = zero_extent;
   }
   if (int rc = finish((char*)A.p); rc != H2_OK) return rc;
   return lease.release();
@@ -271,11 +290,11 @@
     void* dst = (char*)d_out + j0 * out_sz;
     int rc = msm_run_group(
         c, stream, plan, "msm", "msm_launch", mm, ws.sort2 ? " two-level sort" : ws.staged ? " staged scatter" : " direct scatter",
-        [&](char* ws_base, bool zeroed) {
+        [&](char* ws_base, bool zeroed, size_t zero_extent) {
           const auto [ev0, ev1] = msm_prof_events(c, n, mm);
           hipError_t e = ops->msm_launch(table, per_column ? col_tables : nullptr, (uint32_t)be.n,
                                          (const char*)d_scalars + j0 * col_stride * 32, n, col_stride, mm, be.geom, ws_base, ws, stream,
-                                         ev0, ev1, (c.tail_wanted && !ev1) ? c.tail_event : nullptr, affine_out ? nullptr : dst, zeroed);
+                                         ev0, ev1, (c.tail_wanted && !ev1) ? c.tail_event : nullptr, affine_out ? nullptr : dst, zeroed, zero_extent);
           c.tail_recorded = c.tail_wanted;
           c.tail_wait = ev1 ? ev1 : c.tail_event;
           return e;
@@ -296,7 +315,7 @@
     const size_t blocks = (n + 15) / 16, work = MSM_SMALL_MAX * (blocks * (XYZZ29_WORDS * 4) + 4);
     for (size_t j0 = 0; j0 < m; j0 += MSM_SMALL_MAX) {
       const uint32_t count = (uint32_t)std::min<size_t>(MSM_SMALL_MAX, m - j0);
-      ArenaLease lease(c.msm_ws.of(stream), work, stream);
+      ArenaLease lease(c.msm_ws, work, stream);
       if (lease.rc != H2_OK) return lease.rc;
       const void* pts[MSM_SMALL_MAX];
       const void* sc[MSM_SMALL_MAX];
@@ -319,9 +338,9 @@
     if (mm == 0) return H2_EINVAL;
     int rc = msm_run_group(
         c, stream, plan, "msm points", "msm_points_launch", mm, " points front",
-        [&](char* ws_base, bool zeroed) {
+        [&](char* ws_base, bool zeroed, size_t zero_extent) {
           return ops->msm_points_launch(d_points, (const char*)d_scalars + j0 * col_stride * 32, n, col_stride, mm, g, ws_base, plan.ws,
-                                        stream, (char*)d_out + j0 * 96, zeroed);
+                                        stream, (char*)d_out + j0 * 96, zeroed, zero_extent);
         },
         [](char*) { return (int)H2_OK; });
     if (rc != H2_OK) return rc;
@@ -374,7 +393,7 @@
     if (int rc = get_twiddles(c, ops, omega, log_n, table_scale, &tw); rc != H2_OK) return rc;
   std::optional<ArenaLease> A;
   if (ntt_make_plan(log_n).npass > 1) {
-    A.emplace(c.ntt_ws.of(stream), m * ((size_t)32 << log_n), stream);
+    A.emplace(c.ntt_ws, m * ((size_t)32 << log_n), stream);
     if (A->rc != H2_OK) return A->rc;
   }
   if (int rc = launched(launch(tw, A ? A->a.p : nullptr), what); rc != H2_OK) return rc;
@@ -1368,7 +1387,7 @@
   for (size_t j0 = 0; j0 < m; j0 += group) {
     const size_t mm = std::min(group, m - j0);
     const LookupWorkspace ws = lookup_workspace(u, mm);
-    ArenaLease A(k.c->msm_ws.of(k.stream), ws.total, k.stream);
+    ArenaLease A(k.c->msm_ws, ws.total, k.stream);
     if (A.rc != H2_OK) return A.rc;
     if (const char* broken = lookup_check(ws, u, mm, col_stride, A.a.bytes)) {
       g_h2.last_error = std::string("lookup launch geometry: ") + broken;
@@ -1697,7 +1716,7 @@
   if (!curve_ok((int)curve) || !d_points_jac || !omega || log_n > 26) return H2_EINVAL;
   if (log_n == 0) return H2_OK;
   const CurveOps* ops = ops_of((int)curve);
-  ArenaLease A(k.c->msm_ws.of(k.stream), ops->group_fft_scratch(log_n), k.stream);
+  ArenaLease A(k.c->msm_ws, ops->group_fft_scratch(log_n), k.stream);
   if (A.rc != H2_OK) return A.rc;
   if (int rc = launched(ops->group_fft(d_points_jac, d_points_jac, A.a.p, omega, log_n, g_knobs.gfft_lanes, k.stream), "group fft kernels"); rc != H2_OK) return rc;
   return A.release();
@@ -1729,7 +1748,7 @@
   if ((in & 15) || (out & 15)) return H2_EINVAL;
   if (in != out && in < out + bytes && out < in + bytes) return H2_EINVAL;
   const CurveOps* ops = ops_of((int)curve);
-  ArenaLease A(k.c->msm_ws.of(k.stream), ops->group_fft_scratch(log_n), k.stream);
+  ArenaLease A(k.c->msm_ws, ops->group_fft_scratch(log_n), k.stream);
   if (A.rc != H2_OK) return A.rc;
   if (int rc = launched(ops->g_to_lagrange(d_g_affine, d_out_affine, A.a.p, omega_inv, scale, log_n, g_knobs.gfft_lanes, k.stream),
                         "g_to_lagrange kernels");
diff --git a/halo2_prover_amd/csrc/h2_curve_impl.hip b/halo2_prover_amd/csrc/h2_curve_impl.hip
--- a/halo2_prover_amd/csrc/h2_curve_impl.hip
+++ b/halo2_prover_amd/csrc/h2_curve_impl.hip
@@ -43,13 +43,13 @@
 }
 hipError_t msm_launch_(const void* d_table, const void* const* per_column, uint32_t n_bases, const void* d_scalars, size_t n, size_t col_stride, size_t m,
                        const MsmGeom& g, char* ws_base, const MsmWorkspace& ws, hipStream_t s, hipEvent_t ev_start,
-                       hipEvent_t ev_stop, hipEvent_t ev_tail, void* d_out_jac, bool zeroed) {
+                       hipEvent_t ev_stop, hipEvent_t ev_tail, void* d_out_jac, bool zeroed, size_t zero_extent) {
   return msm_launch<CV>((const U128*)d_table, (const U128* const*)per_column, n_bases, (const U128*)d_scalars, n, col_stride, m, g, ws_base, ws, s, ev_start,
-                        ev_stop, ev_tail, (U128*)d_out_jac, zeroed);
+                        ev_stop, ev_tail, (U128*)d_out_jac, zeroed, zero_extent);
 }
 hipError_t msm_points_launch_(const void* d_points, const void* d_scalars, size_t n, size_t col_stride, size_t m, const MsmGeom& g,
-                              char* ws_base, const MsmWorkspace& ws, hipStream_t s, void* d_out_jac, bool zeroed) {
-  return msm_points_launch<CV>((const U128*)d_points, (const U128*)d_scalars, n, col_stride, m, g, ws_base, ws, s, (U128*)d_out_jac, zeroed);
+                              char* ws_base, const MsmWorkspace& ws, hipStream_t s, void* d_out_jac, bool zeroed, size_t zero_extent) {
+  return msm_points_launch<CV>((const U128*)d_points, (const U128*)d_scalars, n, col_stride, m, g, ws_base, ws, s, (U128*)d_out_jac, zeroed, zero_extent);
 }
 hipError_t srs_powers(void* d_out_affine, const uint64_t s_mont[4], uint32_t n, hipStream_t s) {
   Fe<FS> sv;
diff --git a/halo2_prover_amd/csrc/h2_curve_ops.hpp b/halo2_prover_amd/csrc/h2_curve_ops.hpp
--- a/halo2_prover_amd/csrc/h2_curve_ops.hpp
+++ b/halo2_prover_amd/csrc/h2_curve_ops.hpp
@@ -36,10 +36,11 @@
                            const MsmGeom& g, char* ws_base, const MsmWorkspace& ws, hipStream_t s,
                            hipEvent_t ev_start, hipEvent_t ev_stop, hipEvent_t ev_tail,
                            void* d_out_jac ,
-                           bool zeroed );
+                           bool zeroed ,
+                           size_t zero_extent );
   hipError_t (*msm_points_launch)(const void* d_points_affine, const void* d_scalars, size_t n, size_t col_stride, size_t m,
                                   const MsmGeom& g, char* ws_base, const MsmWorkspace& ws, hipStream_t s, void* d_out_jac,
-                                  bool zeroed);
+                                  bool zeroed, size_t zero_extent);
   hipError_t (*srs_powers)(void* d_out_affine, const uint64_t s_mont[4], uint32_t n, hipStream_t s);
   hipError_t (*fixed_base_mul)(void* d_out_affine, const void* d_scalars, uint32_t n, hipStream_t s);
   hipError_t (*msm_small)(const void* const* d_points_affine, const void* const* d_scalars, const uint32_t* m, uint32_t count,
diff --git a/halo2_prover_amd/csrc/h2_internal.hpp b/halo2_prover_amd/csrc/h2_internal.hpp
--- a/halo2_prover_amd/csrc/h2_internal.hpp
+++ b/halo2_prover_amd/csrc/h2_internal.hpp
@@ -19,6 +19,7 @@
   hipEvent_t ev = nullptr;
   hipStream_t last = nullptr;
   bool used = false;
+  bool recorded = false;
   size_t clean_off = 0, clean_bytes = 0;
 };
 
@@ -29,6 +30,7 @@
   bool owned[H2_ARENA_SLOTS] = {};
   uint64_t used_at[H2_ARENA_SLOTS] = {};
   uint64_t clock = 0, takeovers = 0;
+  bool eager = false;
   Arena& of(hipStream_t s) {
     int pick = -1;
     for (int i = 0; i < H2_ARENA_SLOTS && pick < 0; i++)
@@ -118,6 +120,7 @@
   uint64_t guard_launches = 0, guard_violations = 0;
   std::string guard_first;
   uint64_t arena_growths = 0, arena_waits = 0;
+  uint64_t arena_events = 0, takeover_syncs = 0, msm_memsets = 0;
 };
 extern TestKnobs g_knobs;
 extern TestCounters g_counts;
@@ -147,9 +150,11 @@
 struct ArenaLease {
   Arena& a;
   hipStream_t s;
+  ArenaSet* set = nullptr;
   size_t clean_bytes = 0;
   int rc;
   ArenaLease(Arena& arena, size_t want, hipStream_t stream);
+  ArenaLease(ArenaSet& slots, size_t want, hipStream_t stream);
   ArenaLease(const ArenaLease&) = delete;
   ~ArenaLease() noexcept;
   int release();
@@ -157,6 +162,7 @@
  private:
   bool released = false;
   int acquire(size_t want);
+  hipError_t mark_used();
 };
 
 int msm_device_run(DevCtx& c, int curve, const BasesEntry& be, const void* d_scalars, size_t first_base, size_t n,
diff --git a/halo2_prover_amd/csrc/h2_msm.hpp b/halo2_prover_amd/csrc/h2_msm.hpp
--- a/halo2_prover_amd/csrc/h2_msm.hpp
+++ b/halo2_prover_amd/csrc/h2_msm.hpp
@@ -1294,6 +1294,14 @@
 }
 #undef MSM_REQUIRE
 
+inline size_t msm_zero_extent(const MsmWorkspace& ws, size_t carry) {
+  if (ws.guard || carry <= ws.zero_bytes) return ws.zero_bytes;
+  const size_t end = ws.off_misc + carry;
+  const bool holds = carry % 16 == 0 && carry / 16 < (1ull << 32) && end <= ws.off_xsum && end <= ws.off_rc && end <= ws.off_part &&
+                     end <= ws.off_done && end <= ws.off_tree2 && end <= ws.total;
+  return holds ? carry : ws.zero_bytes;
+}
+
 static __global__ void __launch_bounds__(256)
 msm_guard_check_kernel(const uint8_t* __restrict__ arena, MsmWorkspace ws, uint32_t* __restrict__ bad ) {
   const uint32_t r = blockIdx.x;
@@ -1351,7 +1359,8 @@
 template <class CV>
 inline hipError_t msm_launch_back(const U128* table, const U128** d_tables, uint32_t log_b, size_t m, const MsmGeom& g,
                                   char* ws_base, const MsmWorkspace& ws, const MsmKeysArgs& keys_args, bool keys_merged,
-                                  hipStream_t stream, hipEvent_t ev_start, hipEvent_t ev_stop, hipEvent_t ev_tail, U128* d_out_jac) {
+                                  hipStream_t stream, hipEvent_t ev_start, hipEvent_t ev_stop, hipEvent_t ev_tail, U128* d_out_jac,
+                                  size_t zero_extent ) {
   uint32_t* offsets = (uint32_t*)(ws_base + ws.off_offsets);
   uint32_t* sref = (uint32_t*)(ws_base + ws.off_ref);
   uint32_t* chunk_first = (uint32_t*)(ws_base + ws.off_key);
@@ -1386,7 +1395,7 @@
   uint32_t* part = (uint32_t*)(ws_base + ws.off_part);
   uint32_t* done = (uint32_t*)(ws_base + ws.off_done);
   hipLaunchKernelGGL(msm_rowcol_kernel<CV>, dim3(ws.rc, (unsigned)m), dim3(64 * msm_rowcol_waves(g.c - 1, ws.lb, m)), 0, stream,
-                     xsum, rc, done, g.c - 1, ws.lb, (U128*)misc, (uint32_t)(ws.zero_bytes / 16));
+                     xsum, rc, done, g.c - 1, ws.lb, (U128*)misc, (uint32_t)(zero_extent / 16));
   hipLaunchKernelGGL(msm_final_kernel<CV>, dim3(msm_final_blocks(g.c - 1, ws.lb), (unsigned)m), dim3(64), 0, stream, rc, part,
                      done, tree2, d_out_jac, g.c - 1, ws.lb);
   return hipGetLastError();
@@ -1398,7 +1407,8 @@
                              size_t m, const MsmGeom& g, char* ws_base, const MsmWorkspace& ws, hipStream_t stream,
                              hipEvent_t ev_start = nullptr, hipEvent_t ev_stop = nullptr, hipEvent_t ev_tail = nullptr,
                              U128* d_out_jac = nullptr ,
-                             bool zeroed = false ) {
+                             bool zeroed = false ,
+                             size_t zero_extent = 0 ) {
   uint32_t* gcounts = (uint32_t*)(ws_base + ws.off_gcounts);
   uint32_t* offsets = (uint32_t*)(ws_base + ws.off_offsets);
   uint32_t* tile_base = (uint32_t*)(ws_base + ws.off_tile_base);
@@ -1458,7 +1468,7 @@
                          gcounts, tile_base, sref, (uint32_t)n, col_stride, n_bases, ws.tile, tiles, (uint32_t)m, g);
   }
   return msm_launch_back<CV>(table, d_tables, log_b, m, g, ws_base, ws, keys_args, keys_merged, stream, ev_start, ev_stop, ev_tail,
-                             d_out_jac);
+                             d_out_jac, zero_extent ? zero_extent : ws.zero_bytes);
 }
 
 }
diff --git a/halo2_prover_amd/csrc/h2_msm_points.hpp b/halo2_prover_amd/csrc/h2_msm_points.hpp
--- a/halo2_prover_amd/csrc/h2_msm_points.hpp
+++ b/halo2_prover_amd/csrc/h2_msm_points.hpp
@@ -199,7 +199,7 @@
 template <class CV>
 inline hipError_t msm_points_launch(const U128* d_points, const U128* d_scalars, size_t n, size_t col_stride, size_t m,
                                     const MsmGeom& g, char* ws_base, const MsmWorkspace& ws, hipStream_t stream, U128* d_out_jac,
-                                    bool zeroed) {
+                                    bool zeroed, size_t zero_extent ) {
   uint32_t* gcounts = (uint32_t*)(ws_base + ws.off_gcounts);
   uint32_t* offsets = (uint32_t*)(ws_base + ws.off_offsets);
   uint32_t* tile_base = (uint32_t*)(ws_base + ws.off_tile_base);
@@ -219,7 +219,7 @@
                      ws.tile, tiles, (uint32_t)m, g);
   const MsmGeom v = msm_points_virtual(g);
   if ((e = msm_launch_back<CV>(packed, nullptr, 0, m * g.W, v, ws_base, ws, msm_keys_args(ws_base, ws), false, stream, nullptr,
-                               nullptr, nullptr, nullptr)) != hipSuccess)
+                               nullptr, nullptr, nullptr, zero_extent ? zero_extent : ws.zero_bytes)) != hipSuccess)
     return e;
   hipLaunchKernelGGL(msm_points_combine_kernel<CV>, dim3((unsigned)((m + 15) / 16)), dim3(64), 0, stream,
                      (const uint32_t*)(ws_base + ws.off_tree2), d_out_jac, (uint32_t)m, g);
diff --git a/halo2_prover_amd/csrc/h2_selftest.hip b/halo2_prover_amd/csrc/h2_selftest.hip
--- a/halo2_prover_amd/csrc/h2_selftest.hip
+++ b/halo2_prover_amd/csrc/h2_selftest.hip
@@ -271,6 +271,38 @@
   out[3] = c->ntt_ws.takeovers;
   return H2_OK;
 }
+extern "C" int h2_selftest_arena_events(uint64_t out[3]) {
+  std::lock_guard<std::recursive_mutex> lk(g_h2_mu);
+  if (!out) return H2_EINVAL;
+  out[0] = g_counts.arena_events;
+  out[1] = g_counts.takeover_syncs;
+  out[2] = g_counts.msm_memsets;
+  return H2_OK;
+}
+extern "C" int h2_selftest_msm_zero_extent(int curve, size_t n_bases, size_t n, size_t m, size_t carry, size_t* extent) {
+  std::lock_guard<std::recursive_mutex> lk(g_h2_mu);
+  const CurveOps* ops = ops_of(curve);
+  if (!ops || !extent || n == 0 || m == 0 || n > n_bases || n_bases >= (1ull << 31)) return H2_EINVAL;
+  const MsmGeom g = msm_geometry(n_bases, ops->scalar_bits);
+  const MsmGroupPlan plan = msm_plan_group(g, n_bases, n, m, n, false, true);
+  if (plan.cols < m) return H2_EINVAL;
+  if (plan.broken) {
+    g_h2.last_error = std::string("msm launch geometry: ") + plan.broken;
+    return H2_EINVAL;
+  }
+  *extent = msm_zero_extent(plan.ws, carry >= plan.ws.zero_bytes ? carry : 0);
+  return H2_OK;
+}
+extern "C" int h2_selftest_msm_zero_layout(int curve, size_t n_bases, size_t n, size_t m, uint64_t out[4]) {
+  std::lock_guard<std::recursive_mutex> lk(g_h2_mu);
+  const CurveOps* ops = ops_of(curve);
+  if (!ops || !out || n == 0 || m == 0 || n > n_bases || n_bases >= (1ull << 31)) return H2_EINVAL;
+  const MsmGroupPlan plan = msm_plan_group(msm_geometry(n_bases, ops->scalar_bits), n_bases, n, m, n, false, true);
+  if (plan.cols < m || plan.broken) return H2_EINVAL;
+  const MsmWorkspace& ws = plan.ws;
+  out[0] = ws.zero_bytes; out[1] = ws.off_offsets - ws.off_misc; out[2] = ws.off_xsum - ws.off_misc; out[3] = ws.total - ws.off_misc;
+  return H2_OK;
+}
 extern "C" int h2_selftest_msm_tiles(uint32_t tiles, uint32_t m) {
   if (tiles == 0 || m == 0 || (uint64_t)tiles * m > (1u << 24)) return H2_EINVAL;
   const uint32_t grid = msm_tile_grid(tiles, m);
diff --git a/halo2_prover_amd/lib.py b/halo2_prover_amd/lib.py
--- a/halo2_prover_amd/lib.py
+++ b/halo2_prover_amd/lib.py
@@ -135,6 +135,9 @@
     "h2_selftest_msm_guard": (_I, [_I]),
     "h2_selftest_msm_guard_report": (_I, [_P, _P, _Z]),
     "h2_selftest_arena_stats": (_I, [_P]),
+    "h2_selftest_arena_events": (_I, [_P]),
+    "h2_selftest_msm_zero_extent": (_I, [_I, _Z, _Z, _Z, _Z, ctypes.POINTER(_Z)]),
+    "h2_selftest_msm_zero_layout": (_I, [_I, _Z, _Z, _Z, _P]),
     "h2_selftest_fe29_op": (_I, [_I, _I, _P, _P]),
     "h2_selftest_fe29_op_device": (_I, [_I, _I, _P, _P, _Z]),
     "h2_selftest_fe29_chain_device": (_I, [_I, _I, _P, _P, _P, _Z]),
diff --git a/include/h2hip_selftest.h b/include/h2hip_selftest.h
--- a/include/h2hip_selftest.h
+++ b/include/h2hip_selftest.h
@@ -33,6 +33,9 @@
 int h2_selftest_expr_run(const uint8_t* dag, size_t dag_len, const uint64_t* cols, const uint32_t* log_len, uint32_t ncols,
                          uint32_t log_en, uint32_t step, uint64_t* out, uint32_t stats[6]);
 int h2_selftest_arena_stats(uint64_t out[4]);
+int h2_selftest_arena_events(uint64_t out[3]);
+int h2_selftest_msm_zero_extent(int curve, size_t n_bases, size_t n, size_t m, size_t carry, size_t* extent);
+int h2_selftest_msm_zero_layout(int curve, size_t n_bases, size_t n, size_t m, uint64_t out[4]);
 uint64_t h2_selftest_pairing_checks(void);
 
 #ifdef __cplusplus
```
